# IntuitionMachines/volta

Hardware: AMD Instinct MI355X
Metric: image-text pairs/sec, ctrl_vilbert_base pretrain step (higher is better)
Workload: dtype bf16

## Files before the change

include/volta_hip.h:

```cpp
#ifndef VOLTA_HIP_H
#define VOLTA_HIP_H
#include <stddef.h>
#include <stdint.h>

#ifdef __cplusplus
extern "C" {
#endif

typedef void* vk_stream_t;

int vk_version(void);
const char* vk_device_arch(void);
const char* vk_last_error(void);

typedef struct vk_dropout {
    const uint64_t* seed;
    uint32_t site;
    uint32_t threshold;
    float scale;
} vk_dropout;

int vk_set_seed(uint64_t* seed_dev, uint64_t seed, vk_stream_t s);

int vk_cast_f32_bf16(const float* src, void* dst, int64_t n, vk_stream_t s);
// ... 262 lines not shown
    const void* target;
    const int64_t* mask;
    void* work;
    float* out;
    int32_t* row_argmax;
    int32_t kind, groups, n, ld;
} vk_task_loss_args;
int64_t vk_task_loss_work_bytes(int groups);
int vk_task_loss_fwd(const vk_task_loss_args* a, vk_stream_t s);
int vk_task_loss_bwd(const vk_task_loss_args* a, const float* gscale, void* dlogits, vk_stream_t s);

int vk_mask_prep(const int64_t* mask, float* out, int n, vk_stream_t s);

#define VK_CHUNK_SKIP 255
int vk_grad_norm_workspace_floats(void);
int vk_grad_norm_clip(const float* g, int64_t n, float pre_scale, float max_norm, float* partial, float* out, vk_stream_t s);
int vk_grad_norm_clip_masked(const float* g, int64_t n, const uint8_t* chunk_class, float pre_scale, float max_norm, float* partial, float* out, vk_stream_t s);
int vk_grad_sqnorm_chunks(const float* g, int64_t chunk0, int64_t nchunks, const uint8_t* chunk_class, float* sums, vk_stream_t s);
int vk_grad_norm_from_chunks(float* sums, int64_t total_chunks, float pre_scale, float max_norm, float* out, vk_stream_t s);
typedef struct vk_adamw_args {
    float* p;
    const float* g;
    float* m;
    float* v;
    void* shadow;
    const uint8_t* chunk_class;
    const float* clip;
    int64_t n;
    float cls_lr_mult[8];
    float cls_wd[8];
    float lr, beta1, beta2, eps, step_mult, grad_scale;
} vk_adamw_args;
int vk_adamw_step(const vk_adamw_args* a, vk_stream_t s);
int vk_adamw_step_on(const vk_adamw_args* a, int ncus, vk_stream_t s);
typedef struct vk_adamw_tensor {
    float* p;
    const float* g;
    float* m;
    float* v;
    int64_t numel;
    int32_t cls;
    int32_t reserved_;
} vk_adamw_tensor;
int vk_adamw_step_list(const vk_adamw_args* a, const vk_adamw_tensor* list, int n, int64_t max_numel, vk_stream_t s);
int vk_grad_sqnorm_list(const vk_adamw_tensor* list, int n, int64_t max_numel, float* work, float* sums, vk_stream_t s);
int vk_grad_sqnorm_list_work_floats(void);
#define VK_RADAM_CLASSES 64
typedef struct vk_radam_args {
    float* p;
    const float* g;
    float* m;
    float* v;
    void* shadow;
    const uint8_t* chunk_class;
    const float* clip;
    int64_t n;
    float cls_decay[VK_RADAM_CLASSES];
    float cls_step[VK_RADAM_CLASSES];
    int32_t cls_rect[VK_RADAM_CLASSES];
    float beta1, beta2;
    float one_minus_beta1, one_minus_beta2;
    float eps, grad_scale;
} vk_radam_args;
int vk_radam_step(const vk_radam_args* a, vk_stream_t s);
int vk_radam_step_list(const vk_radam_args* a, const vk_adamw_tensor* list, int n, int64_t max_numel, vk_stream_t s);
int vk_axpy_f32(float* y, const float* x, float alpha, int64_t n, vk_stream_t s);
// ... 314 lines not shown
```

volta_amd/_lib.py:

```python
import ctypes as C
import os

import torch

_HERE = os.path.dirname(os.path.abspath(__file__))
LIB_PATH = os.path.join(_HERE, "libvolta_hip_%s.so" % os.environ["VK_LIB"] if os.environ.get("VK_LIB") else "libvolta_hip.so")
GEMM_PERSISTENT, GEMM_ONE_TILE_PER_WG, GEMM_SOFT_START = 0x1000, 0x2000, 0x4000


class VoltaHipError(RuntimeError):
    pass


if not os.path.exists(LIB_PATH):
    raise ImportError(
        "volta_amd: %s not found. The HIP kernels are the product; there is no fallback path. "
        "Build with `make -C volta_amd/csrc` (hipcc --offload-arch=gfx950)." % LIB_PATH)

lib = C.CDLL(LIB_PATH)

c_p = C.c_void_p
i32 = C.c_int32
CHUNK_SKIP = 255

# ... 286 lines not shown
_sig("vk_text_end_rows", C.c_int, c_p, C.c_int, C.c_int, c_p, c_p, c_p)
_sig("vk_vlbert_obj_ids", C.c_int, c_p, c_p, C.c_int, C.c_int, c_p)
_sig("vk_lmdb_open", C.c_int, C.c_char_p, C.POINTER(c_p))
_sig("vk_lmdb_close", None, c_p)
_sig("vk_lmdb_entries", C.c_int64, c_p)
_sig("vk_lmdb_first", C.c_int, c_p)
_sig("vk_lmdb_next", C.c_int, c_p, C.POINTER(c_p), C.POINTER(C.c_size_t), C.POINTER(c_p), C.POINTER(C.c_size_t))
_sig("vk_lmdb_get", C.c_int, c_p, C.c_char_p, C.c_size_t, C.POINTER(c_p), C.POINTER(C.c_size_t))
_sig("vk_concap_record_decode", C.c_int, c_p, C.c_size_t, C.POINTER(ConcapRecord))
_sig("vk_concap_records_decode", C.c_int, C.POINTER(c_p), C.POINTER(C.c_size_t), C.POINTER(ConcapRecord), C.c_int, C.c_int, C.POINTER(C.c_int))
_sig("vk_wordpiece_open", C.c_int, C.c_char_p, C.c_int, C.POINTER(c_p))
_sig("vk_wordpiece_close", None, c_p)
_sig("vk_wordpiece_vocab_size", C.c_int, c_p)
_sig("vk_wordpiece_token_id", C.c_int, c_p, C.c_char_p)
_sig("vk_wordpiece_encode", C.c_int, c_p, C.c_char_p, C.c_size_t, c_p, C.c_int)
_sig("vk_wordpiece_encode_batch", C.c_int, c_p, C.POINTER(C.c_char_p), C.POINTER(C.c_size_t), C.c_int, c_p, C.c_int, c_p, C.c_int)
_sig("vk_b64_decode", C.c_int, C.c_char_p, C.c_size_t, c_p, C.c_size_t, C.POINTER(C.c_size_t))
_sig("vk_task_batch", C.c_int, C.POINTER(TaskBatchArgs), c_p)
_sig("vk_task_images_stage", C.c_int, C.POINTER(TaskImage), C.c_int, C.c_int, C.POINTER(C.c_int))
_sig("vk_vlbert_positions", C.c_int, c_p, C.c_int, C.c_int, C.c_int, c_p, c_p, c_p)
_sig("vk_vis_loss_fwd", C.c_int, C.POINTER(VisLossArgs), c_p)
_sig("vk_vis_loss_bwd", C.c_int, C.POINTER(VisLossArgs), c_p, C.c_int, c_p, c_p)
_sig("vk_task_loss_work_bytes", C.c_int64, C.c_int)
_sig("vk_task_loss_fwd", C.c_int, C.POINTER(TaskLossArgs), c_p)
_sig("vk_task_loss_bwd", C.c_int, C.POINTER(TaskLossArgs), c_p, c_p, c_p)
_sig("vk_nce_negatives", C.c_int, Dropout, C.c_int, C.c_int, c_p, c_p)
_sig("vk_pool_mul_bwd", C.c_int, c_p, C.c_int, c_p, c_p, c_p, c_p, C.c_int, C.c_int, Dropout, c_p)
_sig("vk_mask_prep", C.c_int, c_p, c_p, C.c_int, c_p)
_sig("vk_mul_bf16", C.c_int, c_p, c_p, c_p, C.c_int64, c_p, C.c_int, c_p)
_sig("vk_grad_norm_workspace_floats", C.c_int)
_sig("vk_grad_norm_clip", C.c_int, c_p, C.c_int64, C.c_float, C.c_float, c_p, c_p, c_p)
_sig("vk_adamw_step", C.c_int, C.POINTER(AdamwArgs), c_p)
_sig("vk_adamw_step_on", C.c_int, C.POINTER(AdamwArgs), C.c_int, c_p)
_sig("vk_grad_norm_clip_masked", C.c_int, c_p, C.c_int64, c_p, C.c_float, C.c_float, c_p, c_p, c_p)
_sig("vk_adamw_step_list", C.c_int, C.POINTER(AdamwArgs), c_p, C.c_int, C.c_int64, c_p)
_sig("vk_grad_sqnorm_list", C.c_int, c_p, C.c_int, C.c_int64, c_p, c_p, c_p)
_sig("vk_grad_sqnorm_list_work_floats", C.c_int)
_sig("vk_grad_seed", C.c_int, C.POINTER(GradSeedArgs), c_p)
_sig("vk_pair_gather", C.c_int, C.POINTER(PairGatherArgs), c_p)
_sig("vk_retrieval_ranks", C.c_int, C.POINTER(RetrievalRanksArgs), c_p)
_sig("vk_retrieval_ranks_shard_rows", C.c_int, C.POINTER(RetrievalRanksShardArgs), c_p)
_sig("vk_retrieval_ranks_shard_cols", C.c_int, C.POINTER(RetrievalRanksShardArgs), c_p)
_sig("vk_retrieval_ranks_finish", C.c_int, C.POINTER(RetrievalRanksShardArgs), c_p)
_sig("vk_image_means", C.c_int, C.POINTER(ImageMeansArgs), c_p)
_sig("vk_knn_pool_work_bytes", C.c_int64, C.c_int, C.c_int, C.c_int, C.c_int)
_sig("vk_knn_pool", C.c_int, C.POINTER(KnnPoolArgs), c_p)
_sig("vk_radam_step", C.c_int, C.POINTER(RadamArgs), c_p)
_sig("vk_radam_step_list", C.c_int, C.POINTER(RadamArgs), c_p, C.c_int, C.c_int64, c_p)
_sig("vk_grad_sqnorm_chunks", C.c_int, c_p, C.c_int64, C.c_int64, c_p, c_p, c_p)
_sig("vk_grad_norm_from_chunks", C.c_int, c_p, C.c_int64, C.c_float, C.c_float, c_p, c_p)
_sig("vk_axpy_f32", C.c_int, c_p, c_p, C.c_float, C.c_int64, c_p)
_sig("vk_sum_slabs_f32", C.c_int, c_p, c_p, C.c_int64, C.c_int, C.c_int64, c_p)
_sig("vk_sum_slabs_bf16", C.c_int, c_p, c_p, C.c_int64, C.c_int, C.c_int64, c_p, C.c_int, c_p)
_sig("vk_memset_async", C.c_int, c_p, C.c_int, C.c_int64, c_p)
_sig("vk_hold_cus", C.c_int, C.c_int, C.c_int, C.c_int, c_p)
_sig("vk_gate_wait", C.c_int, c_p, c_p, C.c_int, c_p, c_p)
_sig("vk_bump_u64", C.c_int, c_p, c_p)
_sig("vk_store_u64", C.c_int, c_p, C.c_uint64, c_p)
_sig("vk_gate_value", C.c_int, c_p, C.c_uint64, C.c_int, c_p, c_p)
_sig("vk_comm_standin", C.c_int, c_p, c_p, C.c_int64, C.c_int, C.c_int, c_p, c_p)
_sig("vk_gemm_reserve_cus", C.c_int, C.c_int)
_sig("vk_side_tail", C.c_int, C.POINTER(TailJob), C.c_int, c_p)
_sig("vk_lora_fwd", C.c_int, C.POINTER(LoraProblem), C.c_int, c_p)
_sig("vk_lora_bwd", C.c_int, C.POINTER(LoraBwdProblem), C.c_int, c_p, c_p)
_sig("vk_lora_bwd_work_bytes", C.c_int64, C.POINTER(LoraBwdProblem), C.c_int)
_sig("vk_lora_proj_fwd", C.c_int, C.POINTER(LoraProjProblem), C.c_int, c_p)
_sig("vk_lora_proj_bwd", C.c_int, C.POINTER(LoraProjBwdProblem), C.c_int, c_p, c_p)
_sig("vk_lora_proj_bwd_work_bytes", C.c_int64, C.POINTER(LoraProjBwdProblem), C.c_int)
_sig("vk_lora_fwd_drop", C.c_int, C.POINTER(LoraProblem), C.POINTER(Dropout), C.c_int, c_p)
_sig("vk_lora_bwd_drop", C.c_int, C.POINTER(LoraBwdProblem), C.POINTER(Dropout), C.c_int, c_p, c_p)
_sig("vk_lora_proj_fwd_drop", C.c_int, C.POINTER(LoraProjProblem), C.POINTER(Dropout), C.c_int, c_p)
_sig("vk_lora_proj_bwd_drop", C.c_int, C.POINTER(LoraProjBwdProblem), C.POINTER(Dropout), C.c_int, c_p, c_p)
_sig("vk_run_ops", C.c_int, C.POINTER(Op), C.c_int, c_p)
_sig("vk_run_ops_timed", C.c_int, C.POINTER(Op), C.c_int, c_p, C.POINTER(C.c_float))
_sig("vk_ln_bwd_finalize", C.c_int, C.POINTER(LnBwdArgs), c_p)
_sig("vk_ln_fwd_pair", C.c_int, C.POINTER(LnArgs), C.POINTER(LnArgs), c_p)
_sig("vk_ln_bwd_pair", C.c_int, C.POINTER(LnBwdArgs), C.POINTER(LnBwdArgs), c_p)
_sig("vk_concap_batch", C.c_int, C.POINTER(ConcapArgs), c_p)
_sig("vk_side_join", C.c_int, c_p)
_sig("vk_side_join_from", C.c_int, c_p, c_p)
_sig("vk_side_enable", None, C.c_int)
_sig("vk_side_stream", c_p, c_p)

EXPORTS = ["vk_version", "vk_device_arch", "vk_last_error", "vk_set_seed", "vk_cast_f32_bf16", "vk_gemm_grouped", "vk_gemm_grouped_ex", "vk_gemm_geometry", "vk_gemm_chain", "vk_gemm_split_workspace_bytes", "vk_gemm_fp8_grouped", "vk_quant_rows_fp8", "vk_cast_bf16_fp8",
           "vk_ln_fwd", "vk_ln_fwd_pair", "vk_ln_bwd_partial_rows", "vk_ln_bwd", "vk_ln_bwd_pair", "vk_ln_bwd_finalize", "vk_gated_attn_fwd", "vk_gated_attn_bwd", "vk_gated_attn_lds_bytes",
           "vk_embed_sum_fwd", "vk_embed_sum_bwd", "vk_embed_bwd_workspace_bytes", "vk_rows32", "vk_loc_linear_fwd", "vk_loc_linear_bwd",
           "vk_add_dropout", "vk_colsum_bf16", "vk_vlbert_prep_fwd", "vk_vlbert_maskgrad", "vk_rowgroup_sum_bf16",
           "vk_relu_bwd_bf16", "vk_copy_async", "vk_select_rows", "vk_gather_rows", "vk_scatter_rows_add", "vk_xent_fwd",
           "vk_xent_bwd", "vk_kl_fwd", "vk_kl_bwd", "vk_loss_finalize", "vk_pool_mul_fwd", "vk_pool_mul_bwd",
           "vk_pool_fuse_fwd", "vk_pool_fuse_bwd", "vk_text_end_rows", "vk_vlbert_obj_ids", "vk_vlbert_positions", "vk_vis_loss_fwd", "vk_vis_loss_bwd", "vk_nce_negatives", "vk_task_loss_work_bytes", "vk_task_loss_fwd", "vk_task_loss_bwd",
           "vk_mask_prep", "vk_mul_bf16", "vk_grad_norm_workspace_floats", "vk_grad_norm_clip", "vk_grad_norm_clip_masked", "vk_grad_sqnorm_chunks", "vk_grad_norm_from_chunks", "vk_adamw_step", "vk_adamw_step_on", "vk_adamw_step_list", "vk_grad_sqnorm_list", "vk_grad_sqnorm_list_work_floats", "vk_grad_seed", "vk_pair_gather", "vk_radam_step", "vk_radam_step_list",
           "vk_axpy_f32", "vk_sum_slabs_f32", "vk_sum_slabs_bf16", "vk_memset_async", "vk_hold_cus", "vk_gate_wait", "vk_bump_u64", "vk_store_u64", "vk_gate_value", "vk_comm_standin", "vk_gemm_reserve_cus", "vk_side_tail", "vk_run_ops", "vk_run_ops_timed", "vk_side_join", "vk_side_join_from", "vk_side_stream", "vk_side_enable", "vk_concap_batch",
           "vk_lmdb_open", "vk_lmdb_close", "vk_lmdb_entries", "vk_lmdb_first", "vk_lmdb_next", "vk_lmdb_get", "vk_concap_record_decode", "vk_concap_records_decode", "vk_b64_decode",
           "vk_wordpiece_open", "vk_wordpiece_close", "vk_wordpiece_vocab_size", "vk_wordpiece_token_id", "vk_wordpiece_encode", "vk_wordpiece_encode_batch",
           "vk_lora_fwd", "vk_lora_bwd", "vk_lora_bwd_work_bytes", "vk_lora_proj_fwd", "vk_lora_proj_bwd", "vk_lora_proj_bwd_work_bytes",
           "vk_lora_fwd_drop", "vk_lora_bwd_drop", "vk_lora_proj_fwd_drop", "vk_lora_proj_bwd_drop",
           "vk_task_batch", "vk_task_images_stage", "vk_retrieval_ranks", "vk_retrieval_ranks_shard_rows", "vk_retrieval_ranks_shard_cols", "vk_retrieval_ranks_finish", "vk_image_means", "vk_knn_pool_work_bytes", "vk_knn_pool"]


def check(rc):
    if rc != 0:
        raise VoltaHipError(lib.vk_last_error().decode())


def stream_ptr():
    return C.c_void_p(torch.cuda.current_stream().cuda_stream)


def ptr(t):
    return C.c_void_p(t.data_ptr()) if t is not None else None
```

volta_amd/csrc/attention.hip:

```cpp
#include "common.h"
#include "../../include/volta_hip.h"
#include "util.h"

namespace vk {



template <int DHT>
__device__ __forceinline__ uint32_t img_off(int row, int col) {
    return (uint32_t)(row * (2 * DHT) + ((((col >> 4) ^ ((row >> 1) & 3)) << 5) | ((col & 15) << 1)));
}
template <int DHT>
__device__ __forceinline__ bf16x8 img_row_frag(uint32_t img, int row0, int ks, int lane) {
    const int row = row0 + (lane & 15);
    return *(const bf16x8 VK_LDS*)(uintptr_t)(img + img_off<DHT>(row, ks * 32 + (lane >> 4) * 8));
}
template <int DHT>
__device__ __forceinline__ bf16x8 img_tr_frag(uint32_t img, int rbase, int d0, int lane) {
    const int g = lane >> 4, q = (lane & 15) >> 2, p = lane & 3;
    const int r0 = rbase + 4 * g + q, r1 = r0 + 16;
    bf16x4 lo = lds_read_tr16(img + img_off<DHT>(r0, d0 + 4 * p));
    bf16x4 hi = lds_read_tr16(img + img_off<DHT>(r1, d0 + 4 * p));
    bf16x8 r;
    r[0] = lo[0]; r[1] = lo[1]; r[2] = lo[2]; r[3] = lo[3];
// ... 440 lines not shown
static int fill(AttnK& k, const vk_attn_args* a, const vk_attn_bwd_args* bw) {
    for (int m = 0; m < 2; ++m) {
        k.q[m] = (const uint16_t*)a->q[m]; k.k[m] = (const uint16_t*)a->k[m]; k.v[m] = (const uint16_t*)a->v[m];
        k.ld[m] = a->ld[m]; k.L[m] = a->L[m]; k.mask[m] = a->mask[m];
        k.ctx[m] = (uint16_t*)a->ctx[m]; k.ldo[m] = a->ldo[m]; k.lse[m] = a->lse[m];
        for (int n = 0; n < 2; ++n) { k.gate[m][n] = a->gate[m][n]; k.drop[m][n] = a->drop[m][n]; }
        k.dctx[m] = bw ? (const uint16_t*)bw->dctx[m] : nullptr;
        k.dq[m] = bw ? (uint16_t*)bw->dq[m] : nullptr; k.dk[m] = bw ? (uint16_t*)bw->dk[m] : nullptr;
        k.dv[m] = bw ? (uint16_t*)bw->dv[m] : nullptr; k.ldg[m] = bw ? bw->ldg[m] : 0;
    }
    k.B = a->B; k.nh = a->nh; k.scale = a->scale;
    for (int m = 0; m < 2; ++m) {
        const bool qa = a->gate[m][0] || a->gate[m][1], ka = a->gate[0][m] || a->gate[1][m];
        if (!qa && !ka) continue;
        if (a->L[m] <= 0) return set_error("vk_gated_attn: modality %d is gated on but has length %d", m, a->L[m]);
        if (a->L[m] > (m == 0 ? 64 : 128)) return set_error("vk_gated_attn: lengths (%d, %d) exceed the (64, 128) tile budget", a->L[0], a->L[1]);
        if ((a->ld[m] & 7) || (a->ldo[m] & 7)) return set_error("vk_gated_attn: row strides must be multiples of 8");
        if (ka && (!a->k[m] || !a->v[m] || !a->mask[m])) return set_error("vk_gated_attn: K/V/mask of modality %d missing", m);
        if (qa && (!a->q[m] || !a->ctx[m] || !a->lse[m])) return set_error("vk_gated_attn: Q/ctx/lse of modality %d missing", m);
        if (bw && qa && (!bw->dctx[m] || !bw->dq[m])) return set_error("vk_gated_attn_bwd: dctx/dq of modality %d missing", m);
        if (bw && ka && (!bw->dk[m] || !bw->dv[m])) return set_error("vk_gated_attn_bwd: dk/dv of modality %d missing", m);
    }
    return 0;
}

VK_ATTN_TUNABLE g_attn_fwd_waves = 4;
VK_ATTN_TUNABLE g_attn_fwd_occ = 4;
template <int TP, int RP, int DHT>
static int launch_fwd(const AttnK& k, int nq_tiles, hipStream_t s) {
    const int lds = 3 * (TP + RP) * 2 * DHT + (TP + RP) * 4 + 16;
    int waves = nq_tiles < 4 ? 4 : (nq_tiles > 8 ? 8 : nq_tiles);
    if (g_attn_fwd_waves >= 4 && g_attn_fwd_waves < waves && 4 * lds <= 160 * 1024) waves = g_attn_fwd_waves;
    if (DHT == 64 && g_attn_fwd_occ == 5) {
        hipLaunchKernelGGL((attn_fwd_kernel<TP, RP, 5, DHT>), dim3(k.B * k.nh), dim3(64 * waves), lds, s, k);
    } else {
        auto kern = attn_fwd_kernel<TP, RP, (DHT == 64 ? 4 : 3), DHT>;
        static const hipError_t attr = hipFuncSetAttribute((const void*)kern, hipFuncAttributeMaxDynamicSharedMemorySize, lds); (void)attr;
        hipLaunchKernelGGL(kern, dim3(k.B * k.nh), dim3(64 * waves), lds, s, k);
    }
    return check_launch("vk_gated_attn_fwd");
}
VK_ATTN_TUNABLE g_attn_bwd_waves = 4;
VK_ATTN_TUNABLE g_attn_bwd_occ = 3;

template <int TP, int RP, int DHT>
static int launch_bwd(const AttnK& k, int ntasks, hipStream_t s) {
    const int lds = 4 * (TP + RP) * 2 * DHT + 3 * (TP + RP) * 4 + 16;
    if (DHT == 64 && g_attn_bwd_occ == 3 && 3 * lds <= 160 * 1024) {
        auto kern = attn_bwd_kernel<TP, RP, 3, DHT>;
        static const hipError_t attr = hipFuncSetAttribute((const void*)kern, hipFuncAttributeMaxDynamicSharedMemorySize, lds); (void)attr;
        int waves = g_attn_bwd_waves < 4 ? 4 : (ntasks > g_attn_bwd_waves ? g_attn_bwd_waves : (ntasks < 4 ? 4 : ntasks));
        hipLaunchKernelGGL(kern, dim3(k.B * k.nh), dim3(64 * waves), lds, s, k);
    } else {
        auto kern = attn_bwd_kernel<TP, RP, 2, DHT>;
        static const hipError_t attr = hipFuncSetAttribute((const void*)kern, hipFuncAttributeMaxDynamicSharedMemorySize, lds); (void)attr;
        int waves = g_attn_bwd_waves < 4 ? 4 : (ntasks > g_attn_bwd_waves ? g_attn_bwd_waves : (ntasks < 4 ? 4 : ntasks));
        if (2 * lds > 160 * 1024) waves = ntasks >= 8 ? 8 : (ntasks < 4 ? 4 : ntasks);
        hipLaunchKernelGGL(kern, dim3(k.B * k.nh), dim3(64 * waves), lds, s, k);
    }
    return check_launch("vk_gated_attn_bwd");
}

static bool bwd_fits(int TP, int RP, int dht) { return 4 * (TP + RP) * 2 * dht + 3 * (TP + RP) * 4 + 16 <= 160 * 1024; }

}

namespace vk { int attn_generic(const vk_attn_args* a, const vk_attn_bwd_args* bw, vk_stream_t stream); }

#ifdef VK_STUDY
static int g_attn_force_generic = 0;
extern "C" void vk_attn_set_force_generic(int v) { g_attn_force_generic = v; }
#else
static constexpr int g_attn_force_generic = 0;
#endif
static bool attn_mfma_ok(const vk_attn_args* a) {
    if (a->probs[0][0] || a->probs[0][1] || a->probs[1][0] || a->probs[1][1]) return false;
    for (int m = 0; m < 2; ++m) {
        const bool on = a->gate[m][0] || a->gate[m][1] || a->gate[0][m] || a->gate[1][m];
        if (on && a->L[m] > (m == 0 ? 64 : 128)) return false;
    }
    if (a->dh == 0 || a->dh == 64) return true;
    if (a->dh != 128 || g_attn_force_generic) return false;
    const int TP = a->L[0] > 32 ? 64 : 32, RP = a->L[1] > 64 ? 128 : 64;
    return vk::bwd_fits(TP, RP, 128);
}

namespace vk { size_t attn_generic_lds(const vk_attn_args* a, bool bwd); }

extern "C" size_t vk_gated_attn_lds_bytes(const vk_attn_args* a, int backward) {
    if (!a || attn_mfma_ok(a)) return 0;
    return vk::attn_generic_lds(a, backward != 0);
// ... 51 lines not shown
```

volta_amd/csrc/attention_generic.hip:

```cpp
#include "common.h"
#include "../../include/volta_hip.h"
#include "util.h"

namespace vk {

struct AttnG {
    const uint16_t* q[2]; const uint16_t* k[2]; const uint16_t* v[2];
    int32_t ld[2], L[2];
    const float* mask[2];
    uint16_t* ctx[2]; int32_t ldo[2];
    float* lse[2];
    int32_t B, nh;
    int32_t gate[2][2];
    vk_dropout drop[2][2];
    float scale;
    const uint16_t* dctx[2];
    uint16_t* dq[2]; uint16_t* dk[2]; uint16_t* dv[2];
    int32_t ldg[2];
    float* probs[2][2];
};

constexpr int GW = 4;
constexpr int GMAXNS = 8;

// ... 227 lines not shown
                    const uint32_t wq = *(const uint32_t*)(imgA[mq] + q * RS + 4 * lane), wg = *(const uint32_t*)(imgB[mq] + q * RS + 4 * lane);
                    const float ds = pb0[j], pd = pb1[j];
                    k0 += ds * bf2f(wq & 0xFFFF); k1 += ds * bf2f(wq >> 16);
                    v0 += pd * bf2f(wg & 0xFFFF); v1 += pd * bf2f(wg >> 16);
                }
                *(uint32_t*)(a.dk[mk] + ((size_t)b * Lk + k) * a.ldg[mk] + h * D + 2 * lane) = pack2bf(k0, k1);
                *(uint32_t*)(a.dv[mk] + ((size_t)b * Lk + k) * a.ldg[mk] + h * D + 2 * lane) = pack2bf(v0, v1);
            }
        }
    }
}

static size_t g_lds_bytes(const AttnG& k, int D, int NS, bool bwd) {
    const size_t RS = (size_t)D * 2 + 16;
    size_t n = 0;
    if (bwd) {
        const size_t Lsum = (size_t)k.L[0] + (size_t)k.L[1];
        n = 2 * Lsum * RS + 2 * ((Lsum * 4 + 15) & ~(size_t)15);
    } else {
        for (int m = 0; m < 2; ++m)
            if (k.gate[0][m] || k.gate[1][m]) n += 2 * (size_t)k.L[m] * RS;
    }
    n += (size_t)GW * D * 4 * (bwd ? 2 : 1) + (size_t)GW * NS * 64 * 4 * (bwd ? 2 : 1);
    return (n + 15) & ~(size_t)15;
}

template <int D, int NS>
static int g_launch_ns(const AttnG& k, bool bwd, hipStream_t s) {
    const size_t lds = g_lds_bytes(k, D, NS, bwd);
    if (lds > 160 * 1024) return set_error("vk_gated_attn: head size %d with lengths (%d, %d) needs %zu bytes of LDS (> 160 KiB)", D, k.L[0], k.L[1], lds);
    if (bwd) {
        auto kern = attn_generic_bwd_kernel<D, NS>;
        if (hipFuncSetAttribute((const void*)kern, hipFuncAttributeMaxDynamicSharedMemorySize, (int)lds) != hipSuccess) return set_error("vk_gated_attn_bwd: cannot reserve %zu bytes of LDS", lds);
        hipLaunchKernelGGL(kern, dim3(k.B * k.nh), dim3(64 * GW), lds, s, k);
        return check_launch("vk_gated_attn_bwd (generic kernel)");
    }
    auto kern = attn_generic_fwd_kernel<D, NS>;
    if (hipFuncSetAttribute((const void*)kern, hipFuncAttributeMaxDynamicSharedMemorySize, (int)lds) != hipSuccess) return set_error("vk_gated_attn_fwd: cannot reserve %zu bytes of LDS", lds);
    hipLaunchKernelGGL(kern, dim3(k.B * k.nh), dim3(64 * GW), lds, s, k);
    return check_launch("vk_gated_attn_fwd (generic kernel)");
}

template <int D>
static int g_launch(const AttnG& k, bool bwd, hipStream_t s) {
    int need = 0;
    for (int m = 0; m < 2; ++m) {
        const int nq = (k.gate[m][0] ? k.L[0] : 0) + (k.gate[m][1] ? k.L[1] : 0), nk = (k.gate[0][m] ? k.L[0] : 0) + (k.gate[1][m] ? k.L[1] : 0);
        need = need > nq ? need : nq;
        need = need > nk ? need : nk;
    }
    if (need > GMAXNS * 64) return set_error("vk_gated_attn: %d keys per query row (at most %d on the generic kernels)", need, GMAXNS * 64);
    if (need <= 192) return g_launch_ns<D, 3>(k, bwd, s);
    if (need <= 320) return g_launch_ns<D, 5>(k, bwd, s);
    return g_launch_ns<D, 8>(k, bwd, s);
}

size_t attn_generic_lds(const vk_attn_args* a, bool bwd) {
    AttnG k;
    for (int m = 0; m < 2; ++m) {
        const bool qa = a->gate[m][0] || a->gate[m][1], ka = a->gate[0][m] || a->gate[1][m];
        k.L[m] = (qa || ka) ? a->L[m] : 0;
        for (int j = 0; j < 2; ++j) k.gate[m][j] = a->gate[m][j];
    }
    int need = 0;
    for (int m = 0; m < 2; ++m) {
        const int nq = (k.gate[m][0] ? k.L[0] : 0) + (k.gate[m][1] ? k.L[1] : 0), nk = (k.gate[0][m] ? k.L[0] : 0) + (k.gate[1][m] ? k.L[1] : 0);
        need = need > nq ? need : nq;
        need = need > nk ? need : nk;
    }
    const int NS = need <= 192 ? 3 : need <= 320 ? 5 : 8;
    return g_lds_bytes(k, a->dh ? a->dh : 64, NS, bwd);
}
// ... 37 lines not shown
```

volta_amd/csrc/backbone.hip:

```cpp
#include "common.h"
#include "../../include/volta_hip.h"
#include "util.h"

namespace vk {

__global__ __launch_bounds__(256) void grad_seed_kernel(const vk_grad_seed_args a) {
    const int64_t per_row = a.H / 8, total = (int64_t)a.B * a.L * per_row;
    for (int64_t i = (int64_t)blockIdx.x * 256 + threadIdx.x; i < total; i += (int64_t)gridDim.x * 256) {
        const int64_t r = i / per_row;
        const int h = (int)(i - r * per_row) * 8;
        const int64_t b = r / a.L, l = r - b * a.L;
        float x[8];
        if (a.src) {
            const float* s = a.src + b * a.stride_b + l * a.stride_l + h;
            const f32x4 lo = *(const f32x4*)s, hi = *(const f32x4*)(s + 4);
#pragma unroll
            for (int k = 0; k < 4; ++k) { x[k] = lo[k]; x[k + 4] = hi[k]; }
        } else {
#pragma unroll
            for (int k = 0; k < 8; ++k) x[k] = 0.f;
        }
        if (a.y) {
            const u32x4 yv = *(const u32x4*)((const uint16_t*)a.y + r * a.ldy + h);
#pragma unroll
            for (int k = 0; k < 4; ++k) {
                if (!(bf2f((uint16_t)(yv[k] & 0xFFFFu)) > 0.f)) x[2 * k] = 0.f;
                if (!(bf2f((uint16_t)(yv[k] >> 16)) > 0.f)) x[2 * k + 1] = 0.f;
            }
        }
        uint16_t* d = (uint16_t*)a.dst + (a.row0 + r) * a.ld + h;
        if (a.accumulate) {
            const u32x4 dv = *(const u32x4*)d;
#pragma unroll
            for (int k = 0; k < 4; ++k) {
                x[2 * k] += bf2f((uint16_t)(dv[k] & 0xFFFFu));
                x[2 * k + 1] += bf2f((uint16_t)(dv[k] >> 16));
            }
        }
        *(u32x4*)d = u32x4{pack2bf(x[0], x[1]), pack2bf(x[2], x[3]), pack2bf(x[4], x[5]), pack2bf(x[6], x[7])};
    }
}

}

using namespace vk;

extern "C" int vk_grad_seed(const vk_grad_seed_args* a, vk_stream_t s) {
    if (a->B <= 0 || a->L <= 0 || a->H <= 0) return set_error("vk_grad_seed: empty shape %d x %d x %d", a->B, a->L, a->H);
    if (a->H % 8 || a->ld % 8 || a->row0 < 0 || a->ld < a->H || (a->y && (a->ldy % 8 || a->ldy < a->H)))
        return set_error("vk_grad_seed: H, ld and ldy must be multiples of 8 (H %d, ld %d, ldy %d)", a->H, a->ld, a->ldy);
    if (!a->dst || ((uintptr_t)a->dst & 15) || ((uintptr_t)a->y & 15)) return set_error("vk_grad_seed: dst and y need 16-byte alignment");
    if (!a->src && a->accumulate) return 0;
    if (a->src && (((uintptr_t)a->src & 15) || (a->stride_b & 3) || (a->stride_l & 3)))
        return set_error("vk_grad_seed: src needs 16-byte alignment and strides that are multiples of 4 (copy it contiguous)");
    const int64_t total = (int64_t)a->B * a->L * (a->H / 8);
    int64_t blocks = (total + 255) / 256;
    if (blocks > 2048) blocks = 2048;
    hipLaunchKernelGGL(grad_seed_kernel, dim3((unsigned)blocks), dim3(256), 0, (hipStream_t)s, *a);
    return check_launch("vk_grad_seed");
}
```

volta_amd/csrc/capi.cpp:

```cpp
#include "util.h"
#include "../../include/volta_hip.h"

namespace vk {
static thread_local char g_err[512] = {0};
char* error_buffer() { return g_err; }
int set_error(const char* fmt, ...) {
    va_list ap;
    va_start(ap, fmt);
    vsnprintf(g_err, sizeof(g_err), fmt, ap);
    va_end(ap);
    return -1;
}
int check_launch(const char* what) {
    hipError_t e = hipGetLastError();
    if (e != hipSuccess) return set_error("%s: %s", what, hipGetErrorString(e));
    return 0;
}
}

extern "C" int vk_version(void) { return 1; }
extern "C" const char* vk_device_arch(void) { return "gfx950"; }
extern "C" const char* vk_last_error(void) { return vk::error_buffer(); }
```

volta_amd/csrc/embed.hip:

```cpp
#include "common.h"
#include "../../include/volta_hip.h"
#include "util.h"
#include <climits>

namespace vk {

__device__ __forceinline__ void ld4(const uint16_t* p, float (&v)[4]) {
    u32x2 r = *(const u32x2*)p;
    v[0] = bf2f(r[0] & 0xFFFF); v[1] = bf2f(r[0] >> 16); v[2] = bf2f(r[1] & 0xFFFF); v[3] = bf2f(r[1] >> 16);
}
__device__ __forceinline__ void st4(uint16_t* p, const float (&v)[4]) {
    *(u32x2*)p = u32x2{pack2bf(v[0], v[1]), pack2bf(v[2], v[3])};
}

__device__ __forceinline__ int64_t clampi(int64_t v, int n) { return v < 0 ? 0 : (v >= n ? n - 1 : v); }

__global__ __launch_bounds__(256) void embed_sum_fwd_kernel(vk_embed_args a) {
    const int lane = threadIdx.x & 63, row = blockIdx.x * 4 + (threadIdx.x >> 6);
    if (row >= a.M) return;
    const int64_t id = clampi(a.ids[row], a.V);
    const int64_t ty = a.type_ids ? clampi(a.type_ids[row], a.n_types) : 0;
    const int64_t ps = clampi(a.pos_ids ? a.pos_ids[row] : (row % a.T), a.P);
    const float* w = a.word + (size_t)id * a.H;
    const float* p = a.pos + (size_t)ps * a.H;
// ... 521 lines not shown
    const int b = blockIdx.x, c = blockIdx.y * 256 + threadIdx.x * 4;
    if (c >= H) return;
    float s[4] = {0.f, 0.f, 0.f, 0.f};
    for (int t = 0; t < T; ++t) {
        float v[4];
        ld4(in + ((size_t)b * T + t) * H + c, v);
#pragma unroll
        for (int r = 0; r < 4; ++r) s[r] += v[r];
    }
    st4(out + (size_t)b * H + c, s);
}

__global__ void relu_bwd_kernel(const uint16_t* dy, const uint16_t* y, uint16_t* out, size_t n8) {
    for (size_t i = (size_t)blockIdx.x * blockDim.x + threadIdx.x; i < n8; i += (size_t)gridDim.x * blockDim.x) {
        const u32x4 g = *(const u32x4*)(dy + i * 8), v = *(const u32x4*)(y + i * 8);
        u32x4 o;
#pragma unroll
        for (int k = 0; k < 4; ++k) {
            const uint32_t lo = (bf2f(v[k] & 0xFFFF) > 0.f) ? (g[k] & 0xFFFFu) : 0u, hi = (bf2f(v[k] >> 16) > 0.f) ? (g[k] & 0xFFFF0000u) : 0u;
            o[k] = lo | hi;
        }
        *(u32x4*)(out + i * 8) = o;
    }
}

}

using namespace vk;

extern "C" int vk_vlbert_prep_fwd(const float* loc, int nloc, const float* feat, const float* mask_emb, void* out, int32_t* zero_flag,
                                  int M, int F, int dim, vk_dropout drop, vk_stream_t s) {
    if (F % 4 || (8 * dim) % 4 || nloc < 4) return set_error("vk_vlbert_prep_fwd: F and 8*dim must be multiples of 4, nloc >= 4");
    if (M <= 0) return 0;
    hipLaunchKernelGGL(vlbert_prep_kernel, dim3((M + 3) / 4), dim3(256), 0, (hipStream_t)s, loc, nloc, feat, mask_emb, (uint16_t*)out, zero_flag, M, F, dim, drop);
    return check_launch("vk_vlbert_prep_fwd");
}

extern "C" int vk_vlbert_maskgrad(const void* dx, int ldx, int col0, const int32_t* zero_flag, float* partial, float* out, int M, int F,
                                  vk_dropout drop, vk_stream_t s) {
    if (F % 4 || F > 2048 || col0 % 4) return set_error("vk_vlbert_maskgrad: F must be a multiple of 4, <= 2048");
    if (M <= 0) return 0;
    const int nblk = (M + 31) / 32, nch = (F + 255) / 256;
    hipStream_t st = (hipStream_t)s;
    if (nch <= 4) hipLaunchKernelGGL(vlbert_maskgrad_kernel<4>, dim3(nblk), dim3(256), 0, st, (const uint16_t*)dx, ldx, col0, zero_flag, partial, M, F, drop);
    else hipLaunchKernelGGL(vlbert_maskgrad_kernel<8>, dim3(nblk), dim3(256), 0, st, (const uint16_t*)dx, ldx, col0, zero_flag, partial, M, F, drop);
    hipLaunchKernelGGL(colsum_finalize_kernel, dim3((F + 63) / 64), dim3(1024), 0, st, partial, nblk, F, out, 0);
    return check_launch("vk_vlbert_maskgrad");
}

extern "C" int vk_rowgroup_sum_bf16(const void* in, void* out, int B, int T, int H, vk_stream_t s) {
    if (H % 4) return set_error("vk_rowgroup_sum_bf16: H %% 4 != 0");
    if (B <= 0) return 0;
    hipLaunchKernelGGL(rowgroup_sum_kernel, dim3(B, (H + 255) / 256), dim3(64), 0, (hipStream_t)s, (const uint16_t*)in, (uint16_t*)out, T, H);
    return check_launch("vk_rowgroup_sum_bf16");
}

extern "C" int vk_relu_bwd_bf16(const void* dy, const void* y, void* out, int64_t n, vk_stream_t s) {
    if (n % 8) return set_error("vk_relu_bwd_bf16: n %% 8 != 0");
    if (n <= 0) return 0;
    int64_t blocks = (n / 8 + 255) / 256;
    if (blocks > 4096) blocks = 4096;
    hipLaunchKernelGGL(relu_bwd_kernel, dim3((unsigned)blocks), dim3(256), 0, (hipStream_t)s, (const uint16_t*)dy, (const uint16_t*)y, (uint16_t*)out, (size_t)(n / 8));
    return check_launch("vk_relu_bwd_bf16");
}

extern "C" int vk_copy_async(void* dst, const void* src, int64_t bytes, vk_stream_t s) {
    if (bytes <= 0) return 0;
    hipError_t e = hipMemcpyAsync(dst, src, (size_t)bytes, hipMemcpyDeviceToDevice, (hipStream_t)s);
    if (e != hipSuccess) return set_error("vk_copy_async: %s", hipGetErrorString(e));
    return 0;
}

extern "C" int vk_embed_sum_fwd(const vk_embed_args* a, vk_stream_t s) {
    if (a->H % 4) return set_error("vk_embed_sum_fwd: H %% 4 != 0");
    if (a->M <= 0) return 0;
    hipLaunchKernelGGL(embed_sum_fwd_kernel, dim3((a->M + 3) / 4), dim3(256), 0, (hipStream_t)s, *a);
    return check_launch("vk_embed_sum_fwd");
}

static size_t ws_align(size_t b) { return (b + 255) & ~(size_t)255; }

static size_t embed_ws_layout(int M, int H, int V, int P, int has_pos, char* base, EmbWs* w) {
    const size_t S = (size_t)((M + 31) / 32) * 32;
    size_t off = 0;
    auto take = [&](size_t bytes) { char* q = base ? base + off : nullptr; off += ws_align(bytes); return q; };
    EmbWs x;
    x.Pw = (float*)take(S * H * 4);
    x.Pp = has_pos ? (float*)take(S * H * 4) : nullptr;
    x.Q = (float*)take(S / 32 * 4 * H * 4);
    x.kw = (int*)take(S * 4);
    x.kp = has_pos ? (int*)take(S * 4) : nullptr;
    x.ow = (int*)take((size_t)V * 4);
    x.op = has_pos ? (int*)take((size_t)P * 4) : nullptr;
    if (w) *w = x;
    return off;
}

extern "C" int64_t vk_embed_bwd_workspace_bytes(int M, int H, int V, int P, int has_pos) {
    return M <= 0 ? 0 : (int64_t)embed_ws_layout(M, H, V, P, has_pos, nullptr, nullptr);
}

extern "C" int vk_embed_sum_bwd(const vk_embed_bwd_args* a, vk_stream_t s) {
    if (a->H % 4 || a->H > 1024) return set_error("vk_embed_sum_bwd: H must be a multiple of 4, <= 1024");
    if (a->n_types > 4) return set_error("vk_embed_sum_bwd: at most 4 token types");
    if (a->M <= 0) return 0;
    if (a->T <= 0 || a->M % a->T) return set_error("vk_embed_sum_bwd: M must be a multiple of T (rows are b * T + t)");
    if (!a->work) return set_error("vk_embed_sum_bwd: no workspace (vk_embed_bwd_workspace_bytes)");
    const int has_pos = a->pos_ids && a->dpos;
    EmbWs w;
    embed_ws_layout(a->M, a->H, a->V, a->P, has_pos, (char*)a->work, &w);
    const int nch = (a->H + 255) / 256, S = (a->M + 31) / 32 * 32;
    hipStream_t st = (hipStream_t)s;
    hipLaunchKernelGGL(fill_i32_kernel, dim3((a->V + 255) / 256), dim3(256), 0, st, w.ow, INT_MAX, a->V);
    if (has_pos) hipLaunchKernelGGL(fill_i32_kernel, dim3((a->P + 255) / 256), dim3(256), 0, st, w.op, INT_MAX, a->P);
    dim3 grid(S / 32), block(256);
    switch (nch) {
        case 1: hipLaunchKernelGGL(embed_scatter_kernel<1>, grid, block, 0, st, *a, w); break;
        case 2: hipLaunchKernelGGL(embed_scatter_kernel<2>, grid, block, 0, st, *a, w); break;
        case 3: hipLaunchKernelGGL(embed_scatter_kernel<3>, grid, block, 0, st, *a, w); break;
        default: hipLaunchKernelGGL(embed_scatter_kernel<4>, grid, block, 0, st, *a, w); break;
    }
    dim3 grid2(S + (a->dtype ? (a->H + 63) / 64 : 0), has_pos ? 2 : 1);
    switch (nch) {
        case 1: hipLaunchKernelGGL(embed_combine_kernel<1>, grid2, block, 0, st, *a, w, S); break;
        case 2: hipLaunchKernelGGL(embed_combine_kernel<2>, grid2, block, 0, st, *a, w, S); break;
        case 3: hipLaunchKernelGGL(embed_combine_kernel<3>, grid2, block, 0, st, *a, w, S); break;
        default: hipLaunchKernelGGL(embed_combine_kernel<4>, grid2, block, 0, st, *a, w, S); break;
    }
    if (!a->pos_ids && a->dpos) {
        hipLaunchKernelGGL(embed_pos_reduce_kernel, dim3(a->T, (a->H + 255) / 256), dim3(64), 0, st, (const uint16_t*)a->dz, a->dpos,
                           a->M / a->T, a->T, a->H);
    }
    return check_launch("vk_embed_sum_bwd");
}

extern "C" int vk_loc_linear_fwd(const float* loc, const float* W, const float* bias, void* out, int M, int H, int nloc, vk_stream_t s) {
    if (nloc > 8 || H % 4) return set_error("vk_loc_linear_fwd: nloc <= 8, H %% 4 == 0 required");
    if (M <= 0) return 0;
    if (H > 1024) return set_error("vk_loc_linear_fwd: H <= 1024 required");
    const dim3 grid((M + 4 * LOC_ROWS - 1) / (4 * LOC_ROWS)), block(256);
    hipStream_t st = (hipStream_t)s;
    switch ((H + 255) / 256) {
        case 1: hipLaunchKernelGGL(loc_linear_fwd_kernel<1>, grid, block, 0, st, loc, W, bias, (uint16_t*)out, M, H, nloc); break;
        case 2: hipLaunchKernelGGL(loc_linear_fwd_kernel<2>, grid, block, 0, st, loc, W, bias, (uint16_t*)out, M, H, nloc); break;
        case 3: hipLaunchKernelGGL(loc_linear_fwd_kernel<3>, grid, block, 0, st, loc, W, bias, (uint16_t*)out, M, H, nloc); break;
        default: hipLaunchKernelGGL(loc_linear_fwd_kernel<4>, grid, block, 0, st, loc, W, bias, (uint16_t*)out, M, H, nloc); break;
    }
    return check_launch("vk_loc_linear_fwd");
}

extern "C" int vk_rows32(int M) { return (M + 31) / 32; }

extern "C" int vk_loc_linear_bwd(const void* dz, const float* loc, float* partial, float* dW, float* db, int M, int H, int nloc, vk_stream_t s) {
    if (nloc > 8 || H % 4 || H > 1024) return set_error("vk_loc_linear_bwd: nloc <= 8, H %% 4 == 0, H <= 1024 required");
    if (M <= 0) return 0;
    const int nblk = (M + 31) / 32, nch = (H + 255) / 256;
    hipStream_t st = (hipStream_t)s;
    switch (nch) {
        case 1: hipLaunchKernelGGL(loc_linear_bwd_kernel<1>, dim3(nblk), dim3(256), 0, st, (const uint16_t*)dz, loc, partial, M, H, nloc); break;
        case 2: hipLaunchKernelGGL(loc_linear_bwd_kernel<2>, dim3(nblk), dim3(256), 0, st, (const uint16_t*)dz, loc, partial, M, H, nloc); break;
        case 3: hipLaunchKernelGGL(loc_linear_bwd_kernel<3>, dim3(nblk), dim3(256), 0, st, (const uint16_t*)dz, loc, partial, M, H, nloc); break;
        default: hipLaunchKernelGGL(loc_linear_bwd_kernel<4>, dim3(nblk), dim3(256), 0, st, (const uint16_t*)dz, loc, partial, M, H, nloc); break;
    }
    hipLaunchKernelGGL(loc_linear_bwd_finalize_kernel, dim3((9 * H + 63) / 64), dim3(1024), 0, st, partial, nblk, H, nloc, dW, db);
    return check_launch("vk_loc_linear_bwd");
}

extern "C" int vk_add_dropout(const void* a, const void* b, void* y, int M, int H, float scale, vk_dropout drop, int backward, vk_stream_t s) {
    if (H % 4) return set_error("vk_add_dropout: H %% 4 != 0");
    if (M <= 0) return 0;
    hipLaunchKernelGGL(add_dropout_kernel, dim3((M + 3) / 4), dim3(256), 0, (hipStream_t)s, (const uint16_t*)a, (const uint16_t*)b,
                       (uint16_t*)y, M, H, scale, drop, backward);
    return check_launch("vk_add_dropout");
}

extern "C" int vk_colsum_bf16(const void* src, float* partial, float* out, int M, int H, int accumulate, vk_stream_t s) {
    if (H % 4 || H > 1024) return set_error("vk_colsum_bf16: H must be a multiple of 4, <= 1024");
    if (M <= 0) return 0;
    const int nblk = (M + 31) / 32, nch = (H + 255) / 256;
    hipStream_t st = (hipStream_t)s;
    switch (nch) {
        case 1: hipLaunchKernelGGL(colsum_kernel<1>, dim3(nblk), dim3(256), 0, st, (const uint16_t*)src, partial, M, H); break;
        case 2: hipLaunchKernelGGL(colsum_kernel<2>, dim3(nblk), dim3(256), 0, st, (const uint16_t*)src, partial, M, H); break;
        case 3: hipLaunchKernelGGL(colsum_kernel<3>, dim3(nblk), dim3(256), 0, st, (const uint16_t*)src, partial, M, H); break;
        default: hipLaunchKernelGGL(colsum_kernel<4>, dim3(nblk), dim3(256), 0, st, (const uint16_t*)src, partial, M, H); break;
    }
    hipLaunchKernelGGL(colsum_finalize_kernel, dim3((H + 63) / 64), dim3(1024), 0, st, partial, nblk, H, out, accumulate);
    return check_launch("vk_colsum_bf16");
}
```

volta_amd/csrc/executor.cpp:

```cpp
#include "util.h"
#include <vector>
#include "../../include/volta_hip.h"

static int run_one(const vk_op& o, int i, vk_stream_t s);

#include <cstdlib>
#include <mutex>
#include <unordered_map>
namespace {
constexpr int N_SIDE_EVENTS = 16;
struct Side {
    hipStream_t stream = nullptr;
    hipEvent_t fork = nullptr, join = nullptr;
    hipEvent_t done[N_SIDE_EVENTS] = {};
    bool recorded[N_SIDE_EVENTS] = {};
    bool ok = false;
};
std::mutex g_side_mutex;
std::unordered_map<void*, Side*> g_sides;
int g_side_enabled = 1;

Side* side_lookup(vk_stream_t caller) {
    std::lock_guard<std::mutex> lock(g_side_mutex);
    auto it = g_sides.find((void*)caller);
// ... 15 lines not shown
        if (e != hipSuccess) { vk::set_error("side stream: hipStreamCreate failed"); return nullptr; }
    }
    if (hipEventCreateWithFlags(&g.fork, hipEventDisableTiming) != hipSuccess || hipEventCreateWithFlags(&g.join, hipEventDisableTiming) != hipSuccess) {
        vk::set_error("side stream: hipEventCreate failed");
        return nullptr;
    }
    for (int i = 0; i < N_SIDE_EVENTS; ++i)
        if (hipEventCreateWithFlags(&g.done[i], hipEventDisableTiming) != hipSuccess) { vk::set_error("side stream: hipEventCreate failed"); return nullptr; }
    g.ok = true;
    return sp;
}
}

extern "C" void vk_side_enable(int on) { g_side_enabled = on; }

extern "C" int vk_side_join_from(vk_stream_t owner, vk_stream_t waiter) {
    Side* g = side_lookup(owner);
    if (!g || !g->ok) return 0;
    if (hipEventRecord(g->join, g->stream) != hipSuccess) return vk::set_error("vk_side_join: hipEventRecord failed");
    if (hipStreamWaitEvent((hipStream_t)waiter, g->join, 0) != hipSuccess) return vk::set_error("vk_side_join: hipStreamWaitEvent failed");
    return 0;
}

extern "C" int vk_side_join(vk_stream_t s) { return vk_side_join_from(s, s); }

extern "C" vk_stream_t vk_side_stream(vk_stream_t owner) {
    Side* g = side_for(owner);
    return g ? (vk_stream_t)g->stream : nullptr;
}

extern "C" int vk_run_ops(const vk_op* ops, int n, vk_stream_t s) {
    vk_stream_t cur = s;
    Side* g = nullptr;
    for (int i = 0; i < n; ++i) {
        const vk_op& o = ops[i];
        if (o.kind >= VK_OP_SIDE_BEGIN && o.kind <= VK_OP_JOIN) {
            if (!g_side_enabled) continue;
            if (!g && !(g = side_for(s))) return -1;
            hipError_t e = hipSuccess;
            switch (o.kind) {
                case VK_OP_SIDE_BEGIN:
                    if (o.i0 != 1) {
                        e = hipEventRecord(g->fork, (hipStream_t)s);
                        if (e == hipSuccess) e = hipStreamWaitEvent(g->stream, g->fork, 0);
                    }
                    cur = (vk_stream_t)g->stream;
                    break;
                case VK_OP_SIDE_END:
                    if (o.i0 < 0 || o.i0 >= N_SIDE_EVENTS) return vk::set_error("vk_run_ops: side event %d out of range", o.i0);
                    e = hipEventRecord(g->done[o.i0], g->stream);
                    g->recorded[o.i0] = true;
                    cur = s;
                    break;
                case VK_OP_WAIT_SIDE:
                    if (o.i0 < 0 || o.i0 >= N_SIDE_EVENTS) return vk::set_error("vk_run_ops: side event %d out of range", o.i0);
                    if (g->recorded[o.i0]) e = hipStreamWaitEvent((hipStream_t)s, g->done[o.i0], 0);
                    break;
                default:
                    if (vk_side_join(s) != 0) return -1;
            }
            if (e != hipSuccess) return vk::set_error("vk_run_ops: side-stream control op %d failed at index %d: %s", o.kind, i, hipGetErrorString(e));
            continue;
        }
        if (o.kind == VK_OP_GENERIC && o.a && ((const vk_generic_args*)o.a)->fn == VK_FN_GATE && cur == s) continue;
        int rc = run_one(o, i, cur);
        if (rc != 0) return rc;
    }
    if (cur != s) return vk::set_error("vk_run_ops: op list ends inside a side-stream block");
    return 0;
}

extern "C" int vk_run_ops_timed(const vk_op* ops, int n, vk_stream_t s, float* ms) {
    static thread_local std::vector<hipEvent_t> ev;
    while ((int)ev.size() < n + 1) {
        hipEvent_t e;
        if (hipEventCreate(&e) != hipSuccess) return vk::set_error("vk_run_ops_timed: hipEventCreate failed");
        ev.push_back(e);
    }
    hipStream_t st = (hipStream_t)s;
    (void)hipEventRecord(ev[0], st);
    for (int i = 0; i < n; ++i) {
        const bool gate = ops[i].kind == VK_OP_GENERIC && ops[i].a && ((const vk_generic_args*)ops[i].a)->fn == VK_FN_GATE;
        if (!(ops[i].kind >= VK_OP_SIDE_BEGIN && ops[i].kind <= VK_OP_JOIN) && !gate) {
            int rc = run_one(ops[i], i, s);
            if (rc != 0) return rc;
        }
        (void)hipEventRecord(ev[i + 1], st);
    }
    if (hipStreamSynchronize(st) != hipSuccess) return vk::set_error("vk_run_ops_timed: stream sync failed");
    for (int i = 0; i < n; ++i) {
        float t = 0.f;
        (void)hipEventElapsedTime(&t, ev[i], ev[i + 1]);
        ms[i] += t;
    }
    return 0;
}

static int run_one(const vk_op& o, int i, vk_stream_t s) {
// ... 78 lines not shown
```

volta_amd/csrc/fp8.hip:

```cpp
#include "gemm_common.h"

namespace vk {

typedef __attribute__((ext_vector_type(8))) int i32x8;
constexpr float FP8_MAX = 448.0f;

struct KProb8 { KProb b; const float* sa; const float* sb; };
struct KGroup8 { int32_t nprob; int32_t plain_order; KProb8 p[VK_GEMM_FP8_MAX_GROUP]; };

template <typename SRC>
__global__ __launch_bounds__(256) void quant_rows_fp8_kernel(const SRC* __restrict__ src, int64_t ld, uint8_t* __restrict__ dst, int64_t ldq, float* __restrict__ scale,
                                                             int M, int K, const int32_t* dyn) {
    const int lane = threadIdx.x & 63, row = blockIdx.x * 4 + (threadIdx.x >> 6);
    const int Mr = dyn ? min(*dyn, M) : M;
    if (row >= Mr) return;
    const SRC* x = src + (size_t)row * ld;
    constexpr int MAXCH = 8;
    float v[MAXCH][8];
    float amax = 0.f;
#pragma unroll
    for (int j = 0; j < MAXCH; ++j) {
        const int c = (j * 64 + lane) * 8;
#pragma unroll
        for (int r = 0; r < 8; ++r) v[j][r] = 0.f;
// ... 115 lines not shown
        }
    }
    {
        const int gq = lane >> 4, lr = lane & 15;
        const __amdgpu_buffer_rsrc_t ra = make_rsrc(Q.sa, Q.sa ? (uint32_t)M * 4u : 0u), rb = make_rsrc(Q.sb, Q.sb ? (uint32_t)P.N * 4u : 0u);
        f32x4 sb4[4];
#pragma unroll
        for (int j = 0; j < 4; ++j) {
            sb4[j] = __builtin_bit_cast(f32x4, __builtin_amdgcn_raw_buffer_load_b128(rb, (uint32_t)(n0 + wn * 64 + j * 16 + gq * 4) * 4u, 0, 0));
            if (!Q.sb) sb4[j] = f32x4{1.f, 1.f, 1.f, 1.f};
        }
#pragma unroll
        for (int i = 0; i < TI; ++i) {
            float sa = __builtin_bit_cast(float, __builtin_amdgcn_raw_buffer_load_b32(ra, (uint32_t)(m0 + wm * 64 * TM + i * 16 + lr) * 4u, 0, 0));
            if (!Q.sa) sa = 1.f;
#pragma unroll
            for (int j = 0; j < 4; ++j)
#pragma unroll
                for (int r = 0; r < 4; ++r) acc[i][j][r] *= sa * sb4[j][r];
        }
    }
    f32x4 accb[TI];
    __builtin_amdgcn_s_barrier();
    gemm_epilogue<false, EPI, TI, 4>(P, acc, accb, false, m0 + wm * 64 * TM, n0 + wn * 64, M, lane, lds0 + (uint32_t)wave * 16384u);
}

template <int WM, int WN, int TM>
static int launch8(int epi, const KGroup8& g, int total, hipStream_t s) {
    constexpr int LDS = 2 * (64 * TM * WM + 64 * WN) * 128;
#define VK_CASE(E)                                                                                        \
    case E: {                                                                                             \
        auto k = gemm_fp8_kernel<E, WM, WN, TM>;                                                          \
        static const hipError_t attr = hipFuncSetAttribute((const void*)k, hipFuncAttributeMaxDynamicSharedMemorySize, LDS); (void)attr; \
        hipLaunchKernelGGL(k, dim3(total), dim3(64 * WM * WN), LDS, s, g);                                \
        break;                                                                                            \
    }
    switch (epi) {
        VK_CASE(VK_EPI_BF16) VK_CASE(VK_EPI_GELU) VK_CASE(VK_EPI_F32) VK_CASE(VK_EPI_RELU)
        default: return set_error("vk_gemm_fp8_grouped: epilogue %d is not available on the fp8 path", epi);
    }
#undef VK_CASE
    return check_launch("vk_gemm_fp8_grouped");
}

}

using namespace vk;

extern "C" int vk_gemm_fp8_grouped(int epilogue, const vk_gemm_fp8_problem* probs, int nprob, int geometry, vk_stream_t stream) {
    if (nprob < 1 || nprob > VK_GEMM_FP8_MAX_GROUP) return set_error("vk_gemm_fp8_grouped: nprob %d out of range", nprob);
    const bool f32out = epilogue == VK_EPI_F32;
    bool any_dyn = false;
    for (int i = 0; i < nprob; ++i) {
        const vk_gemm_problem& q = probs[i].p;
        if (q.M < 0 || q.N <= 0 || q.K < 0) return set_error("vk_gemm_fp8_grouped: bad shape %d %d %d", q.M, q.N, q.K);
        if ((q.lda & 15) || (q.ldb & 15)) return set_error("vk_gemm_fp8_grouped: lda/ldb must be multiples of 16 bytes (got %d %d)", q.lda, q.ldb);
        if (((uintptr_t)q.A & 15) || ((uintptr_t)q.B & 15) || ((uintptr_t)q.C & 15)) return set_error("vk_gemm_fp8_grouped: operands must be 16-byte aligned");
        if (!f32out && (q.ldc & 3)) return set_error("vk_gemm_fp8_grouped: ldc must be a multiple of 4");
        if ((q.K % 128) != 0 && q.lda < ((q.K + 127) / 128) * 128) return set_error("vk_gemm_fp8_grouped: K=%d needs lda padded to a multiple of 128", q.K);
        if (q.bias_grad || q.R) return set_error("vk_gemm_fp8_grouped: forward epilogues only");
        if (epilogue == VK_EPI_GELU && !q.C2) return set_error("vk_gemm_fp8_grouped: C2 missing");
        if (probs[i].c8 && (epilogue != VK_EPI_GELU || (probs[i].ldc8 & 3) || ((uintptr_t)probs[i].c8 & 3))) return set_error("vk_gemm_fp8_grouped: c8 is a GELU-epilogue output with a 4-byte aligned leading dimension");
        if ((uint64_t)q.M * q.lda >= 0x7FFFFFF0ull || (uint64_t)q.N * q.ldb >= 0x7FFFFFF0ull) return set_error("vk_gemm_fp8_grouped: operands must stay below 2 GiB");
        any_dyn |= q.dyn != nullptr;
    }
    int t256 = 0;
    for (int i = 0; i < nprob; ++i) t256 += ((probs[i].p.M + 255) / 256) * ((probs[i].p.N + 255) / 256);
    int edge = geometry ? geometry : (t256 >= 160 ? 256 : 128);
    if (edge != 128 && edge != 256) return set_error("vk_gemm_fp8_grouped: geometry %d (128 or 256)", geometry);
    KGroup8 g{};
    g.nprob = nprob;
    g.plain_order = any_dyn ? 1 : 0;
    int total = 0;
    for (int i = 0; i < nprob; ++i) {
        const vk_gemm_problem& q = probs[i].p;
        KProb& k = g.p[i].b;
        k.A = (const char*)q.A; k.B = (const char*)q.B; k.C = (char*)q.C; k.C2 = (char*)q.C2; k.bias = q.bias;
        k.R = nullptr; k.bias_grad = nullptr; k.dyn = q.dyn;
        k.M = q.M; k.N = q.N; k.K = q.K; k.lda = q.lda; k.ldb = q.ldb; k.ldc = q.ldc; k.ldr = 0; k.n_store = q.n_store;
        const int ncols = (f32out && q.n_store > q.N) ? q.n_store : q.N;
        k.tiles_n = (ncols + edge - 1) / edge;
        k.tile_start = total;
        total += ((q.M + edge - 1) / edge) * k.tiles_n;
        k.C8 = (char*)probs[i].c8; k.c8_mul = probs[i].c8_mul; k.ldc8 = probs[i].ldc8;
        g.p[i].sa = probs[i].scale_a; g.p[i].sb = probs[i].scale_b;
    }
    if (total == 0) return 0;
    hipStream_t s = (hipStream_t)stream;
    return edge == 256 ? launch8<2, 4, 2>(epilogue, g, total, s) : launch8<2, 2, 1>(epilogue, g, total, s);
}

extern "C" int vk_quant_rows_fp8(const void* src, int src_is_f32, int64_t ld, void* dst, int64_t ldq, float* scale, int M, int K, const int32_t* dyn, vk_stream_t stream) {
    if (M <= 0) return 0;
    if (K <= 0 || K > 4096 || (K & 7) || (ld & 7) || (ldq & 7)) return set_error("vk_quant_rows_fp8: K=%d (multiple of 8, <= 4096), ld / ldq multiples of 8", K);
    if (((uintptr_t)src & 15) || ((uintptr_t)dst & 7)) return set_error("vk_quant_rows_fp8: alignment");
    hipStream_t s = (hipStream_t)stream;
    if (src_is_f32) hipLaunchKernelGGL(quant_rows_fp8_kernel<float>, dim3((M + 3) / 4), dim3(256), 0, s, (const float*)src, ld, (uint8_t*)dst, ldq, scale, M, K, dyn);
    else hipLaunchKernelGGL(quant_rows_fp8_kernel<uint16_t>, dim3((M + 3) / 4), dim3(256), 0, s, (const uint16_t*)src, ld, (uint8_t*)dst, ldq, scale, M, K, dyn);
    return check_launch("vk_quant_rows_fp8");
}

extern "C" int vk_cast_bf16_fp8(const void* src, void* dst, int64_t n, float mul, vk_stream_t stream) {
    if (n <= 0) return 0;
    if ((n & 7) || ((uintptr_t)src & 15) || ((uintptr_t)dst & 7)) return set_error("vk_cast_bf16_fp8: n %% 8 == 0 and aligned buffers required");
    int64_t blocks = (n / 8 + 255) / 256;
    if (blocks > 8192) blocks = 8192;
    hipLaunchKernelGGL(cast_bf16_fp8_kernel, dim3((unsigned)blocks), dim3(256), 0, (hipStream_t)stream, (const uint16_t*)src, (uint8_t*)dst, (size_t)n, mul);
    return check_launch("vk_cast_bf16_fp8");
}
```

volta_amd/csrc/gemm.hip:

```cpp
#include "gemm_common.h"
#include <cstdlib>

namespace vk {

template <int WM, int WN, int TM = 1> struct Geo {
    static constexpr int THREADS = 64 * WM * WN, BM = 64 * TM * WM, BN = 64 * WN;
    static constexpr int A_BYTES = BM * BK * 2, B_BYTES = BN * BK * 2, STAGE = A_BYTES + B_BYTES;
};

template <bool T, int EXT, int THREADS>
__device__ __forceinline__ void stage_tile(__amdgpu_buffer_rsrc_t rs, uint32_t lds_tile, int ld, int row0, int col0, int tid) {
    constexpr int NP = EXT * 8 / THREADS;
    constexpr int CPR = T ? EXT / 8 : 8;
    const int wave = tid >> 6;
#pragma unroll
    for (int i = 0; i < NP; ++i) {
        const int lin = i * THREADS + tid;
        const int r = lin / CPR, cp = lin % CPR;
        const int cl = T ? (cp ^ tswz(r)) : (cp ^ (r & 7));
        const uint32_t voff = ((uint32_t)(row0 + r) * (uint32_t)ld + (uint32_t)(col0 + cl * 8)) * 2u;
        const uint32_t dst = lds_tile + (i * THREADS + wave * 64) * 16;
        __builtin_amdgcn_raw_ptr_buffer_load_lds(rs, (VK_LDS void*)(uintptr_t)dst, 16, voff, 0, 0, 0);
    }
}
// ... 121 lines not shown
#undef VK_LSTORE
    } else {
        auto stage = [&](int buf, int kt) {
            const uint32_t ta = lds0 + buf * G::STAGE, tb = ta + G::A_BYTES;
            if (AT) stage_tile<true, BM, THREADS>(rsA, ta, P.lda, kt * BK, m0, tid);
            else    stage_tile<false, BM, THREADS>(rsA, ta, P.lda, m0, kt * BK, tid);
            if (BT) stage_tile<true, BN, THREADS>(rsB, tb, P.ldb, kt * BK, n0, tid);
            else    stage_tile<false, BN, THREADS>(rsB, tb, P.ldb, n0, kt * BK, tid);
        };
        if (nk > 0) stage(0, 0);
        const bool late = (g.stagger & 0xFF) && (WM * WN > 4) && ((__builtin_amdgcn_readfirstlane(wave) >> 2) & 1);
        for (int kt = 0; kt < nk; ++kt) {
            asm volatile("s_waitcnt vmcnt(0)" ::: "memory");
            __builtin_amdgcn_s_barrier();
            if (!late && kt + 1 < nk) stage((kt + 1) & 1, kt + 1);
            compute_ks(kt & 1, 0);
            if (late && kt + 1 < nk) stage((kt + 1) & 1, kt + 1);
            compute_ks(kt & 1, 1);
        }
    }

    gemm_epilogue<AT, EPI, TI, 4>(P, acc, accb, do_bias_grad, m0 + wm * 64 * TM, n0 + wn * 64, M, lane);
    retire_mark(g);
}

template <bool AT, bool BT, int WM, int WN, bool REGSTAGE, int TM = 1>
static int launch_cfg(int epi, const KGroup& g, int total, hipStream_t s) {
    using G = Geo<WM, WN, TM>;
    constexpr int LDS = 2 * G::STAGE;
#define VK_CASE(E)                                                                                        \
    case E: {                                                                                             \
        auto k = gemm_kernel<AT, BT, E, WM, WN, REGSTAGE, TM>;                                                \
        static const hipError_t attr = hipFuncSetAttribute((const void*)k, hipFuncAttributeMaxDynamicSharedMemorySize, LDS); (void)attr;  \
        hipLaunchKernelGGL(k, dim3(total), dim3(G::THREADS), LDS, s, g);                                  \
        break;                                                                                            \
    }
    switch (epi) {
        VK_CASE(VK_EPI_BF16) VK_CASE(VK_EPI_GELU) VK_CASE(VK_EPI_MULR) VK_CASE(VK_EPI_ADDR) VK_CASE(VK_EPI_F32) VK_CASE(VK_EPI_RELU) VK_CASE(VK_EPI_F32_ACC)
        default: return set_error("vk_gemm_grouped: unknown epilogue %d", epi);
    }
#undef VK_CASE
    return check_launch("vk_gemm_grouped");
}

#ifdef VK_STUDY
#define VK_TUNABLE static int
#else
#define VK_TUNABLE static constexpr int
#endif
VK_TUNABLE g_stagger = 1;
VK_TUNABLE g_min_tiles256_tn = 50;
VK_TUNABLE g_min_tiles256 = 160;
VK_TUNABLE g_debug = 0;
VK_TUNABLE g_regstage_override = -1;
VK_TUNABLE g_persistent = 1;
#ifdef VK_STUDY
static int g_tile_override = 0;
#endif

static int total_tiles(const vk_gemm_problem* probs, int nprob, int epilogue, int bm, int bn) {
    int total = 0;
    for (int i = 0; i < nprob; ++i) {
        const vk_gemm_problem& q = probs[i];
        const bool f32 = epilogue == VK_EPI_F32 || epilogue == VK_EPI_F32_ACC;
        const int ncols = (f32 && q.n_store > q.N) ? q.n_store : q.N;
        total += ((q.M + bm - 1) / bm) * ((ncols + bn - 1) / bn);
    }
// ... 228 lines not shown
```

volta_amd/csrc/gemm256.hip:

```cpp
#include "gemm_common.h"
#include <hip/hip_ext.h>
#include <type_traits>
#include <atomic>

namespace vk {

constexpr uint32_t HT = 16384;
constexpr uint32_t OOB = 0x80000000u;

template <bool T, bool IS_A>
__device__ __forceinline__ void stage_offsets(uint32_t (&off)[2], int ld, int ext0, int tid) {
#pragma unroll
    for (int i = 0; i < 2; ++i) {
        const int lin = i * 512 + tid;
        if (!T) {
            const int hr = lin >> 3, cp = lin & 7;
            const int row = IS_A ? ((hr >> 6) * 128 + (hr & 63)) : ((hr >> 5) * 64 + (hr & 31));
            off[i] = ((uint32_t)(ext0 + row) * (uint32_t)ld + (uint32_t)((cp ^ (hr & 7)) * 8)) * 2u;
        } else {
            const int kr = lin >> 4, cp = lin & 15;
            const int c = cp ^ tswz(kr);
            const int col = IS_A ? ((c >> 3) * 128 + (c & 7) * 8) : ((c >> 2) * 64 + (c & 3) * 8);
            off[i] = ((uint32_t)kr * (uint32_t)ld + (uint32_t)(ext0 + col)) * 2u;
        }
// ... 472 lines not shown
}

#ifdef VK_STUDY
static unsigned long long* g_stamps = nullptr;
#else
static constexpr unsigned long long* g_stamps = nullptr;
#endif

static std::atomic<int> g_reserved_cus{0};

static int persistent_grid(int total) {
    const int ncu = NUM_CU - g_reserved_cus.load(std::memory_order_relaxed);
    if (total <= ncu) return total;
    const int rounds = (total + ncu - 1) / ncu;
    const int even = ((total + rounds - 1) / rounds + 7) & ~7;
    return even < ncu ? even : ncu;
}

template <bool AT, bool BT, int KSPLIT>
static int launch_layout(int epi, const KGroup& g, int total, hipStream_t s, bool persistent, bool soft) {
    const int flags = soft ? hipExtAnyOrderLaunch : 0;
    constexpr int LDS = (KSPLIT ? 10 : 8) * HT;
#ifdef VK_STUDY
#define VK_KERNEL_OF(E) (KSPLIT == 2 ? gemm256k_kernel<AT, BT, E, 2> : KSPLIT == 3 ? gemm256k_kernel<AT, BT, E, 3> : KSPLIT == 4 ? gemm256k_kernel<AT, BT, E, 4> : gemm256_kernel<AT, BT, E>)
#else
#define VK_KERNEL_OF(E) (KSPLIT == 2 ? gemm256k_kernel<AT, BT, E, 2> : KSPLIT == 3 ? gemm256k_kernel<AT, BT, E, 3> : gemm256k_kernel<AT, BT, E, 4>)
#endif
#define VK_CASE(E)                                                                                        \
    case E: {                                                                                             \
        if constexpr (!(AT && BT) && (KSPLIT == 3 || KSPLIT == 4)) {                                      \
            if (persistent) {                                                                             \
                auto kp = gemm256p_kernel<AT, BT, E, KSPLIT>;                                             \
                static const hipError_t attr_p = hipFuncSetAttribute((const void*)kp, hipFuncAttributeMaxDynamicSharedMemorySize, LDS); (void)attr_p; \
                hipExtLaunchKernelGGL(kp, dim3(persistent_grid(total)), dim3(512), LDS, s, nullptr, nullptr, flags, g, total, g_stamps); \
                break;                                                                                    \
            }                                                                                             \
        }                                                                                                 \
        auto k = VK_KERNEL_OF(E);                                                                         \
        static const hipError_t attr = hipFuncSetAttribute((const void*)k, hipFuncAttributeMaxDynamicSharedMemorySize, LDS); (void)attr;  \
        hipExtLaunchKernelGGL(k, dim3(total), dim3(512), LDS, s, nullptr, nullptr, flags, g);             \
        break;                                                                                            \
    }
    switch (epi) {
        VK_CASE(VK_EPI_BF16) VK_CASE(VK_EPI_GELU) VK_CASE(VK_EPI_MULR) VK_CASE(VK_EPI_ADDR) VK_CASE(VK_EPI_F32) VK_CASE(VK_EPI_RELU) VK_CASE(VK_EPI_F32_ACC)
        default: return set_error("vk_gemm_grouped: unknown epilogue %d", epi);
    }
#undef VK_CASE
#undef VK_KERNEL_OF
    return check_launch("vk_gemm_grouped");
}

int launch_gemm256_chain(int layout, int epi_p, int epi_c, const KGroup& g, int nprod, int ncons, hipStream_t s) {
    constexpr int LDS = 10 * HT;
    const int ncu = (NUM_CU - g_reserved_cus.load(std::memory_order_relaxed)) & ~7;
#define VK_CHAIN_CASE(BT_, P_, C_)                                                                                  \
    if (layout == ((BT_) ? VK_NN : VK_NT) && epi_p == (P_) && epi_c == (C_)) {                                        \
        auto k = gemm256c_kernel<BT_, P_, C_>;                                                                        \
        static const hipError_t attr = hipFuncSetAttribute((const void*)k, hipFuncAttributeMaxDynamicSharedMemorySize, LDS); (void)attr; \
        hipLaunchKernelGGL(k, dim3(ncu), dim3(512), LDS, s, g, nprod, ncons, g_stamps);                               \
        return check_launch("vk_gemm_chain");                                                                         \
    }
    VK_CHAIN_CASE(false, VK_EPI_GELU, VK_EPI_BF16)
    VK_CHAIN_CASE(true, VK_EPI_MULR, VK_EPI_ADDR)
#undef VK_CHAIN_CASE
    return set_error("vk_gemm_chain: layout %d with epilogues %d -> %d is not built (NT: GELU -> BF16, NN: MULR -> ADDR)", layout, epi_p, epi_c);
}

template <int KSPLIT>
static int launch_variant(int layout, int epilogue, const KGroup& g, int total, hipStream_t s, bool persistent, bool soft) {
    if (layout == VK_NT) return launch_layout<false, false, KSPLIT>(epilogue, g, total, s, persistent, soft);
    if (layout == VK_NN) return launch_layout<false, true, KSPLIT>(epilogue, g, total, s, persistent, soft);
    if (layout == VK_TN) return launch_layout<true, true, KSPLIT>(epilogue, g, total, s, false, false);
    return set_error("vk_gemm_grouped: unknown layout %d", layout);
}

int launch_gemm256(int layout, int epilogue, const KGroup& g, int total, hipStream_t s, int variant, bool persistent, bool soft) {
    if (variant == 2) return launch_variant<2>(layout, epilogue, g, total, s, false, soft);
    if (variant == 3) return launch_variant<3>(layout, epilogue, g, total, s, persistent, soft);
    if (variant == 4) return launch_variant<4>(layout, epilogue, g, total, s, persistent, soft);
#ifdef VK_STUDY
    return launch_variant<0>(layout, epilogue, g, total, s, false, false);
#else
    return set_error("vk_gemm_grouped: geometry variant %d is not part of this build", variant);
#endif
}

}

extern "C" int vk_gemm_reserve_cus(int n) {
    const int prev = vk::g_reserved_cus.load(std::memory_order_relaxed);
    if (n >= 0) vk::g_reserved_cus.store(n > 128 ? 128 : (n + 7) & ~7, std::memory_order_relaxed);
    return prev;
// ... 8 lines not shown
```

volta_amd/csrc/gemm4w.hip:

```cpp
#include "gemm_common.h"

namespace vk {

constexpr uint32_t W4_OOB = 0x80000000u;

__device__ __forceinline__ int kswz4(int r) { return (-(r >> 2)) & 3; }

template <bool T, int EXT, int NMAX>
__device__ __forceinline__ void strip_offsets4(uint32_t (&off)[NMAX], int ld, int ext0, int tid) {
    static_assert(EXT / 64 <= NMAX, "offset array too small");
#pragma unroll
    for (int i = 0; i < EXT / 64; ++i) {
        const int lin = i * 256 + tid;
        if (!T) {
            const int r = lin >> 2, cp = lin & 3;
            off[i] = ((uint32_t)(ext0 + r) * (uint32_t)ld + (uint32_t)((cp ^ kswz4(r)) * 8)) * 2u;
        } else {
            constexpr int CPR = EXT / 8;
            const int kr = lin / CPR, cp = lin % CPR;
            const int c = cp ^ tswz(kr);
            off[i] = ((uint32_t)kr * (uint32_t)ld + (uint32_t)(ext0 + c * 8)) * 2u;
        }
    }
}
// ... 102 lines not shown
        asm volatile("s_waitcnt lgkmcnt(0)" ::: "memory");
        __builtin_amdgcn_sched_barrier(0);
        __builtin_amdgcn_s_setprio(1);
#pragma unroll
        for (int i = 0; i < TI; ++i)
#pragma unroll
            for (int j = 0; j < 4; ++j)
                acc[i][j] = __builtin_amdgcn_mfma_f32_16x16x32_bf16(b[j], a[i], acc[i][j], 0, 0, 0);
        if (BG && do_bias_grad) {
#pragma unroll
            for (int i = 0; i < TI; ++i) accb[i] = __builtin_amdgcn_mfma_f32_16x16x32_bf16(ones, a[i], accb[i], 0, 0, 0);
        }
        __builtin_amdgcn_s_setprio(0);
        W4_BARRIER();
        rd = rd == RING - 1 ? 0 : rd + 1;
        wrs = wrs == RING - 1 ? 0 : wrs + 1;
    }
    asm volatile("s_waitcnt vmcnt(0)" ::: "memory");
    W4_BARRIER();

#undef W4_WAIT_STAGE
    gemm_epilogue<AT, EPI, TI, 4>(P, acc, accb, do_bias_grad, m0 + wr * (BM / 2), n0 + wc * 64, M, lane, lds0 + (uint32_t)wave * 16384u);
    retire_mark(g);
}

template <bool AT, bool BT, int TI, int RING>
static int launch_layout4(int epi, const KGroup& g, int total, hipStream_t s) {
    constexpr int LDS = RING * (32 * TI * 64 + 8192);
    static_assert(LDS >= 4 * 16384, "the epilogue stages 16 KiB per wave in the ring");
#define VK_CASE(E)                                                                                        \
    case E: {                                                                                             \
        auto k = gemm4w_kernel<AT, BT, E, TI, RING>;                                                      \
        static const hipError_t attr = hipFuncSetAttribute((const void*)k, hipFuncAttributeMaxDynamicSharedMemorySize, LDS); (void)attr; \
        hipLaunchKernelGGL(k, dim3(total), dim3(256), LDS, s, g);                                         \
        break;                                                                                            \
    }
    switch (epi) {
        VK_CASE(VK_EPI_BF16) VK_CASE(VK_EPI_GELU) VK_CASE(VK_EPI_MULR) VK_CASE(VK_EPI_ADDR) VK_CASE(VK_EPI_F32) VK_CASE(VK_EPI_RELU) VK_CASE(VK_EPI_F32_ACC)
        default: return set_error("vk_gemm_grouped: unknown epilogue %d", epi);
    }
#undef VK_CASE
    return check_launch("vk_gemm_grouped");
}

int launch_gemm4w(int layout, int epilogue, const KGroup& g, int total, hipStream_t s, int bm) {
    if (bm == 128) {
        if (layout == VK_NT) return launch_layout4<false, false, 4, 6>(epilogue, g, total, s);
        if (layout == VK_NN) return launch_layout4<false, true, 4, 6>(epilogue, g, total, s);
        if (layout == VK_TN) return launch_layout4<true, true, 4, 6>(epilogue, g, total, s);
    } else {
        if (layout == VK_NT) return launch_layout4<false, false, 8, 3>(epilogue, g, total, s);
        if (layout == VK_NN) return launch_layout4<false, true, 8, 3>(epilogue, g, total, s);
        if (layout == VK_TN) return launch_layout4<true, true, 8, 3>(epilogue, g, total, s);
    }
    return set_error("vk_gemm_grouped: unknown layout %d", layout);
}

}
```

volta_amd/csrc/heads.hip:

```cpp
#include "common.h"
#include "../../include/volta_hip.h"
#include "util.h"

namespace vk {

__global__ __launch_bounds__(1024) void select_rows_kernel(const int64_t* labels, int N, int mode, int inner, int outer, int off,
                                                           int32_t* rows, int32_t* pos, int32_t* count) {
    __shared__ int wave_tot[16];
    __shared__ int base_s;
    const int tid = threadIdx.x, lane = tid & 63, wave = tid >> 6;
    if (tid == 0) base_s = 0;
    __syncthreads();
    for (int start = 0; start < N; start += 1024) {
        const int i = start + tid;
        bool f = false;
        if (i < N) { const int64_t l = labels[i]; f = mode ? (l == 1) : (l != -1); }
        const unsigned long long bal = __ballot(f);
        const int before = __popcll(bal & ((1ull << lane) - 1ull));
        if (lane == 0) wave_tot[wave] = __popcll(bal);
        __syncthreads();
        int wbase = base_s;
        for (int w = 0; w < wave; ++w) wbase += wave_tot[w];
        if (f) {
            const int j = wbase + before;
// ... 160 lines not shown
        const u32x4 w = philox4((uint32_t)(c >> 2), (uint32_t)row, dc.site, 0u, (uint32_t)seed, (uint32_t)(seed >> 32));
        keep = (w[c & 3] >= dc.threshold) ? dc.scale : 0.f;
    }
    out[i] = f2bf(bf2f(pt[i]) * bf2f(pv[i]) * keep);
}
__global__ __launch_bounds__(256) void pool_mul_bwd_kernel(const uint16_t* dp, int ldp, const uint16_t* pt, const uint16_t* pv, uint16_t* dyt, uint16_t* dyv,
                                                           int B, int P, vk_dropout dc) {
    const int i = blockIdx.x * 256 + threadIdx.x;
    if (i >= B * P) return;
    const int row = i / P, c = i - row * P;
    float keep = 1.f;
    if (dc.threshold) {
        const uint64_t seed = *dc.seed;
        const u32x4 w = philox4((uint32_t)(c >> 2), (uint32_t)row, dc.site, 0u, (uint32_t)seed, (uint32_t)(seed >> 32));
        keep = (w[c & 3] >= dc.threshold) ? dc.scale : 0.f;
    }
    const float g = bf2f(dp[(size_t)row * ldp + c]) * keep, a = bf2f(pt[i]), b = bf2f(pv[i]);
    dyt[i] = f2bf(a > 0.f ? g * b : 0.f);
    dyv[i] = f2bf(b > 0.f ? g * a : 0.f);
}

__global__ void mask_prep_kernel(const int64_t* m, float* out, int n) {
    const int i = blockIdx.x * 256 + threadIdx.x;
    if (i < n) out[i] = (1.0f - (float)m[i]) * -10000.0f;
}

}

using namespace vk;

extern "C" int vk_select_rows(const int64_t* labels, int N, int mode, int inner, int outer, int off, int32_t* rows, int32_t* pos,
                              int32_t* count, vk_stream_t s) {
    if (N < 0 || inner <= 0) return set_error("vk_select_rows: bad arguments");
    hipLaunchKernelGGL(select_rows_kernel, dim3(1), dim3(1024), 0, (hipStream_t)s, labels, N, mode, inner, outer, off, rows, pos, count);
    return check_launch("vk_select_rows");
}
extern "C" int vk_gather_rows(const void* src, const int32_t* rows, const int32_t* count, void* dst, int H, int max_rows, vk_stream_t s) {
    if (H % 8) return set_error("vk_gather_rows: H %% 8 != 0");
    if (max_rows <= 0) return 0;
    hipLaunchKernelGGL(gather_rows_kernel, dim3((max_rows + 3) / 4), dim3(256), 0, (hipStream_t)s, (const uint16_t*)src, rows, count, (uint16_t*)dst, H, max_rows);
    return check_launch("vk_gather_rows");
}
extern "C" int vk_scatter_rows_add(const void* src, const int32_t* rows, const int32_t* count, void* dst, int H, int max_rows, vk_stream_t s) {
    if (H % 4) return set_error("vk_scatter_rows_add: H %% 4 != 0");
    if (max_rows <= 0) return 0;
    hipLaunchKernelGGL(scatter_rows_add_kernel, dim3((max_rows + 3) / 4), dim3(256), 0, (hipStream_t)s, (const uint16_t*)src, rows, count, (uint16_t*)dst, H, max_rows);
    return check_launch("vk_scatter_rows_add");
}
extern "C" int vk_xent_fwd(const vk_xent_args* a, vk_stream_t s) {
    if (a->max_rows <= 0) return 0;
    hipLaunchKernelGGL(xent_fwd_kernel, dim3(a->max_rows), dim3(256), 0, (hipStream_t)s, *a);
    return check_launch("vk_xent_fwd");
}
extern "C" int vk_xent_bwd(const vk_xent_args* a, void* dlogits, int ldd, const float* gscale, vk_stream_t s) {
    if (a->max_rows <= 0) return 0;
    if (ldd < a->V) return set_error("vk_xent_bwd: ldd < V");
    hipLaunchKernelGGL(xent_bwd_kernel, dim3(a->max_rows), dim3(256), 0, (hipStream_t)s, *a, (uint16_t*)dlogits, ldd, gscale);
    return check_launch("vk_xent_bwd");
}
extern "C" int vk_kl_fwd(const vk_kl_args* a, vk_stream_t s) {
    if (a->max_rows <= 0) return 0;
    hipLaunchKernelGGL(kl_fwd_kernel, dim3(a->max_rows), dim3(256), 0, (hipStream_t)s, *a);
    return check_launch("vk_kl_fwd");
}
extern "C" int vk_kl_bwd(const vk_kl_args* a, void* dlogits, int ldd, const float* gscale, vk_stream_t s) {
    if (a->max_rows <= 0) return 0;
    if (ldd < a->V) return set_error("vk_kl_bwd: ldd < V");
    hipLaunchKernelGGL(kl_bwd_kernel, dim3(a->max_rows), dim3(256), 0, (hipStream_t)s, *a, (uint16_t*)dlogits, ldd, gscale);
    return check_launch("vk_kl_bwd");
}
extern "C" int vk_loss_finalize(const float* sums, const int32_t* n_t, const int32_t* n_v, int B, float kl_weight, float* losses, vk_stream_t s) {
    hipLaunchKernelGGL(loss_finalize_kernel, dim3(1), dim3(64), 0, (hipStream_t)s, sums, n_t, n_v, B, kl_weight, losses);
    return check_launch("vk_loss_finalize");
}
extern "C" int vk_pool_mul_fwd(const void* pt, const void* pv, void* out, int B, int P, vk_dropout drop, vk_stream_t s) {
    hipLaunchKernelGGL(pool_mul_fwd_kernel, dim3((B * P + 255) / 256), dim3(256), 0, (hipStream_t)s, (const uint16_t*)pt, (const uint16_t*)pv, (uint16_t*)out, B, P, drop);
    return check_launch("vk_pool_mul_fwd");
}
extern "C" int vk_pool_mul_bwd(const void* dp, int ldp, const void* pt, const void* pv, void* dyt, void* dyv, int B, int P, vk_dropout drop, vk_stream_t s) {
    hipLaunchKernelGGL(pool_mul_bwd_kernel, dim3((B * P + 255) / 256), dim3(256), 0, (hipStream_t)s, (const uint16_t*)dp, ldp, (const uint16_t*)pt,
                       (const uint16_t*)pv, (uint16_t*)dyt, (uint16_t*)dyv, B, P, drop);
    return check_launch("vk_pool_mul_bwd");
}
extern "C" int vk_mask_prep(const int64_t* mask, float* out, int n, vk_stream_t s) {
    if (n <= 0) return 0;
    hipLaunchKernelGGL(mask_prep_kernel, dim3((n + 255) / 256), dim3(256), 0, (hipStream_t)s, mask, out, n);
    return check_launch("vk_mask_prep");
}
```

volta_amd/csrc/layernorm.hip:

```cpp
#include "common.h"
#include "../../include/volta_hip.h"
#include "util.h"

namespace vk {

constexpr float LN_EPS = 1e-12f;
constexpr int LN_THREADS = 256;
constexpr int LN_BWD_ROWS = 16;

__device__ __forceinline__ uint32_t drop_row(const vk_drop_rows (&seg)[2], int split, int row, uint32_t& site) {
    const int si = row >= split ? 1 : 0;
    const int r = si ? row - split : row;
    site = seg[si].site;
    if (seg[si].div <= 0) return (uint32_t)r;
    return (uint32_t)((r / seg[si].div) * seg[si].mul + (r % seg[si].div) + seg[si].off);
}

__device__ __forceinline__ void load4(const uint16_t* p, float (&v)[4]) {
    u32x2 r = *(const u32x2*)p;
    v[0] = bf2f(r[0] & 0xFFFF); v[1] = bf2f(r[0] >> 16); v[2] = bf2f(r[1] & 0xFFFF); v[3] = bf2f(r[1] >> 16);
}
__device__ __forceinline__ void store4(uint16_t* p, const float (&v)[4]) {
    *(u32x2*)p = u32x2{pack2bf(v[0], v[1]), pack2bf(v[2], v[3])};
}
// ... 290 lines not shown
        for (int b = ty; b < nblk; b += 16) s += partial[(size_t)b * 2 * H + i];
    red[ty][tx] = s;
    __syncthreads();
    if (ty == 0 && i < 2 * H) {
#pragma unroll
        for (int k = 1; k < 16; ++k) s += red[k][tx];
        float* o = i < H ? dgamma + i : dbeta + (i - H);
        *o = accumulate ? *o + s : s;
    }
}

}

static int ln_check(int H, int maxH, const char* who) {
    if (H % 4 || H > maxH || H <= 0) return vk::set_error("%s: H=%d must be a multiple of 4, <= %d", who, H, maxH);
    return 0;
}

extern "C" int vk_ln_fwd_pair(const vk_ln_args* a, const vk_ln_args* b, vk_stream_t stream) {
    using namespace vk;
    if (ln_check(a->H, 2048, "vk_ln_fwd")) return -1;
    if (b && (b->H != a->H || a->dyn || b->dyn)) return set_error("vk_ln_fwd_pair: both jobs need the same H and static row counts");
    const int nb0 = a->M > 0 ? (a->M + 3) / 4 : 0, nb1 = (b && b->M > 0) ? (b->M + 3) / 4 : 0;
    if (nb0 + nb1 == 0) return 0;
    const int nch = (a->H + 255) / 256;
    dim3 grid(nb0 + nb1), block(LN_THREADS);
    hipStream_t s = (hipStream_t)stream;
    JobPair<vk_ln_args> jp;
    jp.job[0] = *a;
    jp.job[1] = b ? *b : *a;
    jp.nb0 = nb0;
    jp.stagger = jp.stagger_mod = 0;
    switch (nch) {
        case 1: hipLaunchKernelGGL(ln_fwd_kernel<1>, grid, block, 0, s, jp); break;
        case 2: hipLaunchKernelGGL(ln_fwd_kernel<2>, grid, block, 0, s, jp); break;
        case 3: hipLaunchKernelGGL(ln_fwd_kernel<3>, grid, block, 0, s, jp); break;
        case 4: hipLaunchKernelGGL(ln_fwd_kernel<4>, grid, block, 0, s, jp); break;
        default: hipLaunchKernelGGL(ln_fwd_kernel<8>, grid, block, 0, s, jp); break;
    }
    return check_launch("vk_ln_fwd");
}

extern "C" int vk_ln_fwd(const vk_ln_args* a, vk_stream_t stream) { return vk_ln_fwd_pair(a, nullptr, stream); }

extern "C" int vk_ln_bwd_partial_rows(int M) { return (M + vk::LN_BWD_ROWS - 1) / vk::LN_BWD_ROWS; }

#ifdef VK_STUDY
static unsigned long long* g_ln_stamps = nullptr;
static int g_ln_stagger = 0, g_ln_stagger_mod = 0;
extern "C" void vk_ln_set_stamp_buffer(unsigned long long* p) { g_ln_stamps = p; }
extern "C" void vk_ln_set_stagger(int ticks, int mod) { g_ln_stagger = ticks; g_ln_stagger_mod = mod; }
#else
static constexpr unsigned long long* g_ln_stamps = nullptr;
static constexpr int g_ln_stagger = 0, g_ln_stagger_mod = 0;
#endif

static void ln_finalize_launch(const vk_ln_bwd_args* a, hipStream_t s) {
    hipLaunchKernelGGL(vk::ln_bwd_finalize_kernel, dim3((2 * a->H + 63) / 64), dim3(1024), 0, s, a->partial, vk_ln_bwd_partial_rows(a->M), a->H,
                       a->dgamma, a->dbeta, a->accumulate & 1);
}

extern "C" int vk_ln_bwd_pair(const vk_ln_bwd_args* a, const vk_ln_bwd_args* b, vk_stream_t stream) {
    using namespace vk;
    if (ln_check(a->H, 2048, "vk_ln_bwd")) return -1;
    if (b && (b->H != a->H || a->dyn || b->dyn)) return set_error("vk_ln_bwd_pair: both jobs need the same H and static row counts");
    if (b && !a->partial != !b->partial) {
        if (vk_ln_bwd_pair(a, nullptr, stream)) return -1;
        return vk_ln_bwd_pair(b, nullptr, stream);
    }
    const bool params = a->partial != nullptr;
    if (!params && !a->dz && !a->dd && (!b || (!b->dz && !b->dd))) return 0;
    const int nb0 = a->M > 0 ? vk_ln_bwd_partial_rows(a->M) : 0, nb1 = (b && b->M > 0) ? vk_ln_bwd_partial_rows(b->M) : 0;
    const int nch = (a->H + 255) / 256;
    dim3 grid(nb0 + nb1), block(LN_THREADS);
    hipStream_t s = (hipStream_t)stream;
    JobPair<vk_ln_bwd_args> jp;
    jp.job[0] = *a;
    jp.job[1] = b ? *b : *a;
    jp.nb0 = nb0;
    jp.stagger = g_ln_stagger; jp.stagger_mod = g_ln_stagger_mod;
    if (nb0 + nb1 && params) switch (nch) {
        case 1: hipLaunchKernelGGL(ln_bwd_kernel<1>, grid, block, 0, s, jp, g_ln_stamps); break;
        case 2: hipLaunchKernelGGL(ln_bwd_kernel<2>, grid, block, 0, s, jp, g_ln_stamps); break;
        case 3: hipLaunchKernelGGL(ln_bwd_kernel<3>, grid, block, 0, s, jp, g_ln_stamps); break;
        case 4: hipLaunchKernelGGL(ln_bwd_kernel<4>, grid, block, 0, s, jp, g_ln_stamps); break;
        case 5: case 6: hipLaunchKernelGGL(ln_bwd_kernel<6>, grid, block, 0, s, jp, g_ln_stamps); break;
        default: hipLaunchKernelGGL(ln_bwd_kernel<8>, grid, block, 0, s, jp, g_ln_stamps); break;
    }
    if (nb0 + nb1 && !params) switch (nch) {
        case 1: hipLaunchKernelGGL(ln_bwd_dx_kernel<1>, grid, block, 0, s, jp, g_ln_stamps); break;
        case 2: hipLaunchKernelGGL(ln_bwd_dx_kernel<2>, grid, block, 0, s, jp, g_ln_stamps); break;
        case 3: hipLaunchKernelGGL(ln_bwd_dx_kernel<3>, grid, block, 0, s, jp, g_ln_stamps); break;
        case 4: hipLaunchKernelGGL(ln_bwd_dx_kernel<4>, grid, block, 0, s, jp, g_ln_stamps); break;
        case 5: case 6: hipLaunchKernelGGL(ln_bwd_dx_kernel<6>, grid, block, 0, s, jp, g_ln_stamps); break;
        default: hipLaunchKernelGGL(ln_bwd_dx_kernel<8>, grid, block, 0, s, jp, g_ln_stamps); break;
    }
    if (!params) return check_launch("vk_ln_bwd");
    if ((nb0 || !(a->accumulate & 1)) && !(a->accumulate & 2)) ln_finalize_launch(a, s);
    if (b && (nb1 || !(b->accumulate & 1)) && !(b->accumulate & 2)) ln_finalize_launch(b, s);
    return check_launch("vk_ln_bwd");
}

extern "C" int vk_ln_bwd(const vk_ln_bwd_args* a, vk_stream_t stream) { return vk_ln_bwd_pair(a, nullptr, stream); }

extern "C" int vk_ln_bwd_finalize(const vk_ln_bwd_args* a, vk_stream_t stream) {
    if (!a->partial) return vk::set_error("vk_ln_bwd_finalize: the job has no partial records (partial NULL: gamma and beta frozen)");
    if (a->M <= 0 && (a->accumulate & 1)) return 0;
    ln_finalize_launch(a, (hipStream_t)stream);
    return vk::check_launch("vk_ln_bwd_finalize");
}
```

volta_amd/csrc/misc.hip:

```cpp
#include "common.h"
#include "../../include/volta_hip.h"
#include "util.h"

namespace vk {

__global__ void set_seed_kernel(uint64_t* p, uint64_t v) { *p = v; }

__global__ void cast_f32_bf16_kernel(const float* __restrict__ src, uint16_t* __restrict__ dst, size_t n) {
    const size_t n8 = n >> 3;
    for (size_t i = (size_t)blockIdx.x * blockDim.x + threadIdx.x; i < n8; i += (size_t)gridDim.x * blockDim.x) {
        const f32x4 a = __builtin_nontemporal_load((const f32x4*)(src + i * 8)), b = __builtin_nontemporal_load((const f32x4*)(src + i * 8 + 4));
        *(u32x4*)(dst + i * 8) = u32x4{pack2bf(a[0], a[1]), pack2bf(a[2], a[3]), pack2bf(b[0], b[1]), pack2bf(b[2], b[3])};
    }
    if (blockIdx.x == 0 && threadIdx.x < (n & 7)) dst[n8 * 8 + threadIdx.x] = f2bf(src[n8 * 8 + threadIdx.x]);
}

__global__ void mul_bf16_kernel(const uint16_t* a, const uint16_t* b, uint16_t* out, size_t n, const int32_t* dyn_rows, int row_len) {
    if (dyn_rows) { const size_t lim = (size_t)(*dyn_rows) * row_len; if (lim < n) n = lim; }
    const size_t n8 = n >> 3;
    for (size_t i = (size_t)blockIdx.x * blockDim.x + threadIdx.x; i < n8; i += (size_t)gridDim.x * blockDim.x) {
        const u32x4 x = *(const u32x4*)(a + i * 8), y = *(const u32x4*)(b + i * 8);
        u32x4 o;
#pragma unroll
        for (int k = 0; k < 4; ++k) o[k] = pack2bf(bf2f(x[k] & 0xFFFF) * bf2f(y[k] & 0xFFFF), bf2f(x[k] >> 16) * bf2f(y[k] >> 16));
        *(u32x4*)(out + i * 8) = o;
    }
}

}

extern "C" int vk_mul_bf16(const void* a, const void* b, void* out, int64_t n, const int32_t* dyn_rows, int row_len, vk_stream_t s) {
    if (n <= 0) return 0;
    if (n % 8 || row_len % 8) return vk::set_error("vk_mul_bf16: n and row_len must be multiples of 8");
    if (((uintptr_t)a & 15) || ((uintptr_t)b & 15) || ((uintptr_t)out & 15)) return vk::set_error("vk_mul_bf16: 16-byte alignment required");
    int64_t blocks = (n / 8 + 255) / 256;
    if (blocks > 4096) blocks = 4096;
    hipLaunchKernelGGL(vk::mul_bf16_kernel, dim3((unsigned)blocks), dim3(256), 0, (hipStream_t)s, (const uint16_t*)a, (const uint16_t*)b,
                       (uint16_t*)out, (size_t)n, dyn_rows, row_len);
    return vk::check_launch("vk_mul_bf16");
}

extern "C" int vk_set_seed(uint64_t* seed_dev, uint64_t seed, vk_stream_t s) {
    hipLaunchKernelGGL(vk::set_seed_kernel, dim3(1), dim3(1), 0, (hipStream_t)s, seed_dev, seed);
    return vk::check_launch("vk_set_seed");
}

extern "C" int vk_cast_f32_bf16(const float* src, void* dst, int64_t n, vk_stream_t s) {
    if (n <= 0) return 0;
    if (((uintptr_t)src & 15) || ((uintptr_t)dst & 15)) return vk::set_error("vk_cast_f32_bf16: 16-byte alignment required");
    int64_t blocks = (n / 8 + 255) / 256;
    if (blocks > 4096) blocks = 4096;
    if (blocks < 1) blocks = 1;
    hipLaunchKernelGGL(vk::cast_f32_bf16_kernel, dim3((unsigned)blocks), dim3(256), 0, (hipStream_t)s, src, (uint16_t*)dst, (size_t)n);
    return vk::check_launch("vk_cast_f32_bf16");
}

namespace vk {
__global__ __launch_bounds__(512) void mfma_peak_kernel(const uint32_t* seed, float* out, int iters) {
    typedef __attribute__((ext_vector_type(8))) short v8;
    typedef __attribute__((ext_vector_type(4))) float v4;
    v8 a[4], b[4];
    const uint32_t s = seed[threadIdx.x & 63] + blockIdx.x;
#pragma unroll
    for (int i = 0; i < 4; ++i)
#pragma unroll
        for (int k = 0; k < 8; ++k) {
            a[i][k] = (short)(0x3C00 + ((s * (i * 8 + k + 1) * 2654435761u) >> 22));
            b[i][k] = (short)(0xBC00 + ((s * (i * 8 + k + 77) * 40503u) >> 22));
        }
    v4 acc[4][4];
#pragma unroll
    for (int i = 0; i < 4; ++i)
#pragma unroll
        for (int j = 0; j < 4; ++j) acc[i][j] = v4{0.f, 0.f, 0.f, 0.f};
    for (int it = 0; it < iters; ++it) {
#pragma unroll
        for (int i = 0; i < 4; ++i)
#pragma unroll
            for (int j = 0; j < 4; ++j) acc[i][j] = __builtin_amdgcn_mfma_f32_16x16x32_bf16(a[i], b[j], acc[i][j], 0, 0, 0);
    }
    float t = 0.f;
#pragma unroll
    for (int i = 0; i < 4; ++i)
#pragma unroll
        for (int j = 0; j < 4; ++j) t += acc[i][j][0] + acc[i][j][1] + acc[i][j][2] + acc[i][j][3];
    if (t == 12345.678f) out[0] = t;
}
}

extern "C" int vk_mfma_peak(const uint32_t* seed64, float* out, int iters, int blocks, vk_stream_t stream) {
    hipLaunchKernelGGL(vk::mfma_peak_kernel, dim3(blocks), dim3(512), 0, (hipStream_t)stream, seed64, out, iters);
    return vk::check_launch("vk_mfma_peak");
}

namespace vk {
__global__ void hold_cus_kernel(unsigned ticks) {
    extern __shared__ char smem[];
    if (threadIdx.x == 0) {
        smem[0] = 1;
        const unsigned long long t0 = __builtin_amdgcn_s_memrealtime();
        while (__builtin_amdgcn_s_memrealtime() - t0 < ticks) __builtin_amdgcn_s_sleep(16);
    }
}
}

extern "C" int vk_hold_cus(int nwg, int usec, int whole_cu, vk_stream_t stream) {
    if (nwg <= 0 || usec <= 0) return 0;
    if (nwg > 256 || usec > 100000) return vk::set_error("vk_hold_cus: at most 256 workgroups for at most 0.1 s (got %d, %d us)", nwg, usec);
    constexpr int LDS = 160 * 1024;
    static const hipError_t attr = hipFuncSetAttribute((const void*)vk::hold_cus_kernel, hipFuncAttributeMaxDynamicSharedMemorySize, LDS); (void)attr;
    hipLaunchKernelGGL(vk::hold_cus_kernel, dim3(nwg), dim3(64), whole_cu ? LDS : 64, (hipStream_t)stream, (unsigned)usec * 100u);
    return vk::check_launch("vk_hold_cus");
}

namespace vk {
__global__ __launch_bounds__(256) void comm_standin_kernel(const u32x4* __restrict__ src, u32x4* __restrict__ dst, size_t n16, unsigned min_ticks,
                                                           unsigned long long* stamps) {
    const unsigned long long t0 = __builtin_amdgcn_s_memrealtime();
    if (stamps && threadIdx.x == 0) atomicMin(stamps, t0);
    const size_t per = (n16 + gridDim.x - 1) / gridDim.x, lo = per * blockIdx.x, hi = lo + per < n16 ? lo + per : n16;
    for (size_t i = lo + threadIdx.x; i < hi; i += 256) __builtin_nontemporal_store(__builtin_nontemporal_load(src + i), dst + i);
    if (threadIdx.x == 0) {
        const unsigned long long first = stamps ? __hip_atomic_load(stamps, __ATOMIC_RELAXED, __HIP_MEMORY_SCOPE_AGENT) : t0;
        while (__builtin_amdgcn_s_memrealtime() - first < min_ticks) __builtin_amdgcn_s_sleep(32);
        if (stamps) atomicMax(stamps + 1, __builtin_amdgcn_s_memrealtime());
    }
}
}

extern "C" int vk_comm_standin(const void* src, void* dst, int64_t bytes, int nwg, int min_usec, uint64_t* stamps, vk_stream_t stream) {
    if (bytes <= 0 || nwg <= 0) return 0;
    if ((bytes & 15) || ((uintptr_t)src & 15) || ((uintptr_t)dst & 15)) return vk::set_error("vk_comm_standin: 16-byte granularity");
    if (nwg > 1024 || min_usec < 0 || min_usec > 100000) return vk::set_error("vk_comm_standin: at most 1024 workgroups, at most 0.1 s");
    hipLaunchKernelGGL(vk::comm_standin_kernel, dim3(nwg), dim3(256), 0, (hipStream_t)stream, (const vk::u32x4*)src, (vk::u32x4*)dst, (size_t)(bytes / 16),
                       (unsigned)min_usec * 100u, (unsigned long long*)stamps);
    return vk::check_launch("vk_comm_standin");
}

namespace vk {
__global__ void gate_wait_kernel(const unsigned long long* flag, const unsigned long long* stamp, unsigned timeout_ticks, int32_t* err) {
    if (threadIdx.x != 0) return;
    const unsigned long long want = __hip_atomic_load(stamp, __ATOMIC_RELAXED, __HIP_MEMORY_SCOPE_AGENT);
    const unsigned long long t0 = __builtin_amdgcn_s_memrealtime();
    while (__hip_atomic_load(flag, __ATOMIC_RELAXED, __HIP_MEMORY_SCOPE_AGENT) != want) {
        __builtin_amdgcn_s_sleep(16);
        if (__builtin_amdgcn_s_memrealtime() - t0 > timeout_ticks) {
            if (err) __hip_atomic_store(err, 2, __ATOMIC_RELAXED, __HIP_MEMORY_SCOPE_AGENT);
            break;
        }
    }
}
__global__ void bump_u64_kernel(unsigned long long* w) { *w += 1ull; }
__global__ void store_u64_kernel(unsigned long long* w, unsigned long long v) { __hip_atomic_store(w, v, __ATOMIC_RELAXED, __HIP_MEMORY_SCOPE_AGENT); }
__global__ void gate_value_kernel(const unsigned long long* flag, unsigned long long want, unsigned timeout_ticks, int32_t* err) {
    if (threadIdx.x != 0) return;
    const unsigned long long t0 = __builtin_amdgcn_s_memrealtime();
    while (__hip_atomic_load(flag, __ATOMIC_RELAXED, __HIP_MEMORY_SCOPE_AGENT) != want) {
        __builtin_amdgcn_s_sleep(16);
        if (__builtin_amdgcn_s_memrealtime() - t0 > timeout_ticks) {
            if (err) __hip_atomic_store(err, 2, __ATOMIC_RELAXED, __HIP_MEMORY_SCOPE_AGENT);
            break;
        }
    }
}
}

extern "C" int vk_store_u64(uint64_t* word, uint64_t value, vk_stream_t stream) {
    if (!word) return vk::set_error("vk_store_u64: NULL");
    hipLaunchKernelGGL(vk::store_u64_kernel, dim3(1), dim3(1), 0, (hipStream_t)stream, (unsigned long long*)word, (unsigned long long)value);
    return vk::check_launch("vk_store_u64");
}

extern "C" int vk_gate_value(const uint64_t* flag, uint64_t want, int timeout_us, int32_t* err, vk_stream_t stream) {
    if (!flag || timeout_us <= 0 || timeout_us > 10000000) return vk::set_error("vk_gate_value: flag and 0 < timeout_us <= 10000000");
    hipLaunchKernelGGL(vk::gate_value_kernel, dim3(1), dim3(64), 0, (hipStream_t)stream, (const unsigned long long*)flag, (unsigned long long)want,
                       (unsigned)(timeout_us > 40000000 ? 4000000000u : (unsigned)timeout_us * 100u), err);
    return vk::check_launch("vk_gate_value");
}

extern "C" int vk_gate_wait(const uint64_t* flag, const uint64_t* stamp, int timeout_us, int32_t* err, vk_stream_t stream) {
    if (!flag || !stamp || timeout_us <= 0 || timeout_us > 1000000) return vk::set_error("vk_gate_wait: flag, stamp and 0 < timeout_us <= 1000000");
    hipLaunchKernelGGL(vk::gate_wait_kernel, dim3(1), dim3(64), 0, (hipStream_t)stream, (const unsigned long long*)flag, (const unsigned long long*)stamp,
                       (unsigned)timeout_us * 100u, err);
    return vk::check_launch("vk_gate_wait");
}

extern "C" int vk_bump_u64(uint64_t* word, vk_stream_t stream) {
    if (!word) return vk::set_error("vk_bump_u64: NULL");
    hipLaunchKernelGGL(vk::bump_u64_kernel, dim3(1), dim3(1), 0, (hipStream_t)stream, (unsigned long long*)word);
    return vk::check_launch("vk_bump_u64");
}
```

volta_amd/csrc/optim.hip:

```cpp
#include "common.h"
#include "../../include/volta_hip.h"
#include "util.h"

namespace vk {

constexpr int NORM_BLOCKS = 1024;

__global__ __launch_bounds__(256) void sqnorm_partial_kernel(const float* g, size_t n4, float* partial, const uint8_t* chunk_class) {
    __shared__ float sh[4];
    float s = 0.f;
    for (size_t i = (size_t)blockIdx.x * 256 + threadIdx.x; i < n4; i += (size_t)gridDim.x * 256) {
        if (chunk_class && chunk_class[i >> 8] == VK_CHUNK_SKIP) continue;
        const f32x4 v = *(const f32x4*)(g + i * 4);
        s += v[0] * v[0] + v[1] * v[1] + v[2] * v[2] + v[3] * v[3];
    }
    s = wave_sum(s);
    if ((threadIdx.x & 63) == 0) sh[threadIdx.x >> 6] = s;
    __syncthreads();
    if (threadIdx.x == 0) partial[blockIdx.x] = sh[0] + sh[1] + sh[2] + sh[3];
}
__global__ __launch_bounds__(256) void sqnorm_final_kernel(const float* partial, int nblk, float pre_scale, float max_norm, float* out) {
    __shared__ double sh[4];
    double s = 0.0;
    for (int i = threadIdx.x; i < nblk; i += 256) s += (double)partial[i];
// ... 263 lines not shown
            for (int k = 1; k < 16; ++k) s += red[k][tx];
            float* o = i < H ? J.dst + i : J.dst2 + (i - H);
            *o = J.accumulate ? *o + s : s;
        }
    }
}

}

using namespace vk;

extern "C" int vk_side_tail(const vk_tail_job* jobs, int njobs, vk_stream_t s) {
    if (njobs <= 0) return 0;
    if (njobs > VK_TAIL_MAX_JOBS) return set_error("vk_side_tail: %d jobs (max %d)", njobs, VK_TAIL_MAX_JOBS);
    TailJobs t;
    t.njobs = njobs;
    int total = 0;
    for (int i = 0; i < njobs; ++i) {
        t.j[i] = jobs[i];
        vk_tail_job& J = t.j[i];
        int nb;
        if (J.kind == 0) {
            if ((J.stride & 3) || ((uintptr_t)J.dst & 15) || ((uintptr_t)J.src & 15)) return set_error("vk_side_tail: slab job %d needs 16-byte alignment", i);
            nb = (int)((J.n / 4 + 255) / 256);
            if (nb < 1) nb = 1;
        } else if (J.kind == 1) {
            nb = (int)((2 * J.n + 15) / 16);
        } else return set_error("vk_side_tail: unknown job kind %d", J.kind);
        if (J.n <= 0 || J.count <= 0) nb = 0;
        J.block_start = total;
        total += nb;
    }
    if (total == 0) return 0;
    hipLaunchKernelGGL(side_tail_kernel, dim3((unsigned)total), dim3(256), 0, (hipStream_t)s, t);
    return check_launch("vk_side_tail");
}

extern "C" int vk_sum_slabs_bf16(void* dst, const float* src, int64_t slab_stride, int nslabs, int64_t n, const int32_t* dyn_rows, int row_len, vk_stream_t s) {
    if (n <= 0 || nslabs <= 0) return 0;
    if ((slab_stride & 3) || (n & 3) || (row_len & 3)) return set_error("vk_sum_slabs_bf16: lengths must be multiples of 4");
    if (((uintptr_t)src & 15) || ((uintptr_t)dst & 7)) return set_error("vk_sum_slabs_bf16: src needs 16-byte, dst 8-byte alignment");
    int64_t blocks = (n / 4 + 255) / 256;
    if (blocks > 2048) blocks = 2048;
    hipLaunchKernelGGL(sum_slabs_bf16_kernel, dim3((unsigned)blocks), dim3(256), 0, (hipStream_t)s, (uint16_t*)dst, src, (size_t)slab_stride, nslabs, (size_t)n, dyn_rows, row_len);
    return check_launch("vk_sum_slabs_bf16");
}

extern "C" int vk_sum_slabs_f32(float* dst, const float* src, int64_t slab_stride, int nslabs, int64_t n, vk_stream_t s) {
    if (n <= 0 || nslabs <= 0) return 0;
    if ((slab_stride & 3) || ((uintptr_t)dst & 15) || ((uintptr_t)src & 15)) return set_error("vk_sum_slabs_f32: 16-byte alignment required");
    int64_t blocks = (n / 4 + 255) / 256;
    if (blocks > 2048) blocks = 2048;
    if (blocks < 1) blocks = 1;
    hipLaunchKernelGGL(sum_slabs_kernel, dim3((unsigned)blocks), dim3(256), 0, (hipStream_t)s, dst, src, (size_t)slab_stride, nslabs, (size_t)n);
    return check_launch("vk_sum_slabs_f32");
}

extern "C" int vk_grad_norm_workspace_floats(void) { return NORM_BLOCKS; }

extern "C" int vk_grad_norm_clip_masked(const float* g, int64_t n, const uint8_t* chunk_class, float pre_scale, float max_norm, float* partial, float* out, vk_stream_t s) {
    if (n % 4 || ((uintptr_t)g & 15)) return set_error("vk_grad_norm_clip: n %% 4 == 0 and 16-byte alignment required");
    if (chunk_class && (n % 1024)) return set_error("vk_grad_norm_clip_masked: a chunk mask needs an arena of whole 1024-element chunks");
    hipStream_t st = (hipStream_t)s;
    hipLaunchKernelGGL(sqnorm_partial_kernel, dim3(NORM_BLOCKS), dim3(256), 0, st, g, (size_t)(n / 4), partial, chunk_class);
    hipLaunchKernelGGL(sqnorm_final_kernel, dim3(1), dim3(256), 0, st, partial, NORM_BLOCKS, pre_scale, max_norm, out);
    return check_launch("vk_grad_norm_clip");
}

extern "C" int vk_grad_sqnorm_chunks(const float* g, int64_t chunk0, int64_t nchunks, const uint8_t* chunk_class, float* sums, vk_stream_t s) {
    if (chunk0 < 0 || nchunks < 0 || ((uintptr_t)g & 15)) return set_error("vk_grad_sqnorm_chunks: bad range or alignment");
    if (nchunks == 0) return 0;
    hipLaunchKernelGGL(sqnorm_chunks_kernel, dim3((unsigned)((nchunks + 3) / 4)), dim3(256), 0, (hipStream_t)s, g, (size_t)chunk0, (size_t)nchunks, chunk_class, sums);
    return check_launch("vk_grad_sqnorm_chunks");
}

extern "C" int vk_grad_norm_from_chunks(float* sums, int64_t total_chunks, float pre_scale, float max_norm, float* out, vk_stream_t s) {
    if (total_chunks <= 0) return set_error("vk_grad_norm_from_chunks: no chunks");
    if (((uintptr_t)(sums + total_chunks)) & 7) return set_error("vk_grad_norm_from_chunks: total_chunks must be even (the group sums follow the chunk sums as doubles)");
    double* group = (double*)(sums + total_chunks);
    hipLaunchKernelGGL(sqnorm_groups_kernel, dim3(SQ_GROUPS), dim3(256), 0, (hipStream_t)s, sums, (size_t)total_chunks, group);
    hipLaunchKernelGGL(sqnorm_from_groups_kernel, dim3(1), dim3(64), 0, (hipStream_t)s, (const double*)group, pre_scale, max_norm, out);
    return check_launch("vk_grad_norm_from_chunks");
}

extern "C" int vk_grad_norm_clip(const float* g, int64_t n, float pre_scale, float max_norm, float* partial, float* out, vk_stream_t s) {
    return vk_grad_norm_clip_masked(g, n, nullptr, pre_scale, max_norm, partial, out, s);
}

extern "C" int vk_adamw_step(const vk_adamw_args* a, vk_stream_t s) {
    if (a->n % 1024) return set_error("vk_adamw_step: arena length must be a multiple of 1024 elements");
    if (a->n == 0) return 0;
    hipLaunchKernelGGL(adamw_kernel, dim3((unsigned)(a->n / 1024)), dim3(256), 0, (hipStream_t)s, *a);
    return check_launch("vk_adamw_step");
}

extern "C" int vk_adamw_step_on(const vk_adamw_args* a, int ncus, vk_stream_t s) {
    if (a->n % 1024) return set_error("vk_adamw_step_on: arena length must be a multiple of 1024 elements");
    if (ncus < 1 || ncus > 256) return set_error("vk_adamw_step_on: %d compute units", ncus);
    if (a->n == 0) return 0;
    constexpr int FOOTPRINT = 96 * 1024;
    static const hipError_t attr = hipFuncSetAttribute((const void*)adamw_narrow_kernel, hipFuncAttributeMaxDynamicSharedMemorySize, FOOTPRINT); (void)attr;
    hipLaunchKernelGGL(adamw_narrow_kernel, dim3((unsigned)ncus), dim3(512), FOOTPRINT, (hipStream_t)s, *a);
    return check_launch("vk_adamw_step_on");
}

static int list_blocks(int64_t max_numel, int cap) {
    int64_t b = (max_numel + 1023) / 1024;
    return (int)(b < 1 ? 1 : b > cap ? cap : b);
}

extern "C" int vk_adamw_step_list(const vk_adamw_args* a, const vk_adamw_tensor* list, int n, int64_t max_numel, vk_stream_t s) {
    if (n < 0 || n > 65535 || max_numel < 0) return set_error("vk_adamw_step_list: %d tensors, max numel %lld", n, (long long)max_numel);
    if (n == 0 || max_numel == 0) return 0;
    hipLaunchKernelGGL(adamw_list_kernel, dim3((unsigned)list_blocks(max_numel, 1024), (unsigned)n), dim3(256), 0, (hipStream_t)s, *a, list);
    return check_launch("vk_adamw_step_list");
}

extern "C" int vk_grad_sqnorm_list_work_floats(void) { return 2 * SQ_LIST_BLOCKS; }

extern "C" int vk_grad_sqnorm_list(const vk_adamw_tensor* list, int n, int64_t max_numel, float* work, float* sums, vk_stream_t s) {
    if (n < 0 || n > 65535 || max_numel < 0) return set_error("vk_grad_sqnorm_list: %d tensors, max numel %lld", n, (long long)max_numel);
    if (n == 0) return 0;
    if ((uintptr_t)work & 7) return set_error("vk_grad_sqnorm_list: work needs 8-byte alignment");
    hipLaunchKernelGGL(sqnorm_list_partial_kernel, dim3(SQ_LIST_BLOCKS, (unsigned)n), dim3(256), 0, (hipStream_t)s, list, (double*)work);
    hipLaunchKernelGGL(sqnorm_list_final_kernel, dim3((unsigned)n), dim3(64), 0, (hipStream_t)s, (const double*)work, sums);
    return check_launch("vk_grad_sqnorm_list");
// ... 17 lines not shown
```

volta_amd/csrc/pairs.hip:

```cpp
#include "common.h"
#include "../../include/volta_hip.h"
#include "util.h"

namespace vk {

__global__ __launch_bounds__(256) void pair_gather_kernel(const vk_pair_gather_args a) {
    const int p = blockIdx.x, k = blockIdx.y, t = threadIdx.x;
    const int side = a.side[k];
    int64_t item;
    if (a.cap_idx) item = side ? a.img_idx[p] : a.cap_idx[p];
    else item = side ? (int64_t)a.i0 + p % a.ni : (int64_t)a.c0 + p / a.ni;
    const bool ok = item >= 0 && item < a.n_items[side];
    const int64_t nb = a.bytes[k];
    const char* __restrict__ src = (const char*)a.src[k] + (ok ? item : 0) * nb;
    char* __restrict__ dst = (char*)a.dst[k] + (int64_t)p * nb;
    int64_t done = 0;
    if ((((uintptr_t)src | (uintptr_t)dst) & 15) == 0) {
        const u32x4* __restrict__ s4 = (const u32x4*)src;
        u32x4* __restrict__ d4 = (u32x4*)dst;
        const int64_t n16 = nb >> 4;
        const u32x4 z = {0u, 0u, 0u, 0u};
        int64_t j = t;
        for (; j + 3 * 256 < n16; j += 4 * 256) {
            const u32x4 v0 = ok ? s4[j] : z, v1 = ok ? s4[j + 256] : z, v2 = ok ? s4[j + 512] : z, v3 = ok ? s4[j + 768] : z;
// ... 2 lines not shown
            d4[j + 512] = v2;
            d4[j + 768] = v3;
        }
        for (; j < n16; j += 256) d4[j] = ok ? s4[j] : z;
        done = n16 << 2;
    }
    const uint32_t* __restrict__ s1 = (const uint32_t*)src;
    uint32_t* __restrict__ d1 = (uint32_t*)dst;
    for (int64_t j = done + t; j < (nb >> 2); j += 256) d1[j] = ok ? s1[j] : 0u;
}

}

using namespace vk;

extern "C" int vk_pair_gather(const vk_pair_gather_args* a, vk_stream_t s) {
    if (a->nseg < 1 || a->nseg > VK_PAIR_MAX_SEGS || a->npairs < 0) return set_error("vk_pair_gather: %d segments (1..%d), %d pairs", a->nseg, VK_PAIR_MAX_SEGS, a->npairs);
    if (!a->cap_idx != !a->img_idx) return set_error("vk_pair_gather: cap_idx and img_idx are given together or not at all");
    if (a->n_items[0] < 0 || a->n_items[1] < 0) return set_error("vk_pair_gather: negative item count");
    if (!a->cap_idx && a->npairs > 0) {
        if (a->nc <= 0 || a->ni <= 0 || (int64_t)a->nc * a->ni != a->npairs || a->c0 < 0 || a->i0 < 0 ||
            (int64_t)a->c0 + a->nc > a->n_items[0] || (int64_t)a->i0 + a->ni > a->n_items[1])
            return set_error("vk_pair_gather: cross product captions [%d, +%d) x images [%d, +%d) does not fit %d pairs of %lld x %lld items", a->c0, a->nc,
                             a->i0, a->ni, a->npairs, (long long)a->n_items[0], (long long)a->n_items[1]);
    }
    for (int k = 0; k < a->nseg; ++k) {
        if (!a->src[k] || !a->dst[k] || a->bytes[k] <= 0 || (a->bytes[k] & 3) || (a->side[k] != 0 && a->side[k] != 1) ||
            ((uintptr_t)a->src[k] & 3) || ((uintptr_t)a->dst[k] & 3))
            return set_error("vk_pair_gather: segment %d (bytes %lld, side %d): buffers 4-byte aligned, bytes a positive multiple of 4, side 0 | 1", k,
                             (long long)a->bytes[k], a->side[k]);
        if (a->n_items[a->side[k]] <= 0) return set_error("vk_pair_gather: segment %d reads side %d, which has no items", k, a->side[k]);
    }
    if (a->npairs == 0) return 0;
    hipLaunchKernelGGL(pair_gather_kernel, dim3((unsigned)a->npairs, (unsigned)a->nseg), dim3(256), 0, (hipStream_t)s, *a);
    return check_launch("vk_pair_gather");
}
```

volta_amd/csrc/util.h:

```cpp
#pragma once
#include <hip/hip_runtime.h>
#include <cstdarg>
#include <cstdio>

namespace vk {
char* error_buffer();
int set_error(const char* fmt, ...);
int check_launch(const char* what);
}
```

volta_amd/csrc/vislosses.hip:

```cpp
#include "common.h"
#include "../../include/volta_hip.h"
#include "util.h"

namespace vk {

__device__ __forceinline__ float vl_block_sum(float v, float* sh) {
    v = wave_sum(v);
    const int lane = threadIdx.x & 63, wave = threadIdx.x >> 6;
    __syncthreads();
    if (lane == 0) sh[wave] = v;
    __syncthreads();
    return sh[0] + sh[1] + sh[2] + sh[3];
}
__device__ __forceinline__ float vl_block_max(float v, float* sh) {
    v = wave_max(v);
    const int lane = threadIdx.x & 63, wave = threadIdx.x >> 6;
    __syncthreads();
    if (lane == 0) sh[wave] = v;
    __syncthreads();
    return fmaxf(fmaxf(sh[0], sh[1]), fmaxf(sh[2], sh[3]));
}

template <bool HUBER>
__global__ __launch_bounds__(256) void vis_reg_fwd_kernel(vk_vis_loss_args a) {
// ... 201 lines not shown
        for (int k = 0; k < K; ++k) opos[(size_t)b * K + k] = c + (k == K - 1);
    }
    for (int o = 32; o; o >>= 1) lo = min(lo, __shfl_xor(lo, o));
    if ((tid & 63) == 0) s_min[tid >> 6] = lo;
    __syncthreads();
    lo = s_min[0];
    for (int w = 1; w < 16; ++w) lo = min(lo, s_min[w]);
    for (int i = tid; i < B * T; i += 1024) {
        const int t = i % T;
        tpos[i] = t + (t >= lo ? K : 0);
    }
}

}

using namespace vk;

static int check_vis(const vk_vis_loss_args* a, const char* who) {
    if (a->kind != VK_VIS_MSE && a->kind != VK_VIS_NCE && a->kind != VK_VIS_XENT && a->kind != VK_VIS_HUBER) return set_error("%s: unknown kind %d", who, a->kind);
    if (!a->logits || !a->pos || !a->count || !a->loss_sum || a->ld < a->V) return set_error("%s: missing logits / pos / count / loss_sum, or ld < V", who);
    if (a->kind == VK_VIS_XENT && (!a->labels || !a->lse)) return set_error("%s: xent needs labels and lse", who);
    if ((a->kind == VK_VIS_MSE || a->kind == VK_VIS_HUBER || a->kind == VK_VIS_NCE) && !a->target) return set_error("%s: regression / nce need the feature matrix", who);
    if (a->kind == VK_VIS_NCE && (!a->neg_index || !a->aux || !a->lse || a->n_neg < 1 || a->n_neg + 1 > VK_NCE_MAX_SAMPLES || a->V % 4 || a->ld % 4))
        return set_error("%s: nce needs neg_index, aux, lse, 1 <= n_neg < %d and V, ld multiples of 4", who, VK_NCE_MAX_SAMPLES);
    return 0;
}

extern "C" int vk_vis_loss_fwd(const vk_vis_loss_args* a, vk_stream_t s) {
    if (check_vis(a, "vk_vis_loss_fwd")) return -1;
    if (a->max_rows <= 0) return 0;
    const dim3 grid(a->max_rows), block(256);
    hipStream_t st = (hipStream_t)s;
    switch (a->kind) {
        case VK_VIS_MSE: hipLaunchKernelGGL(vis_reg_fwd_kernel<false>, grid, block, 0, st, *a); break;
        case VK_VIS_HUBER: hipLaunchKernelGGL(vis_reg_fwd_kernel<true>, grid, block, 0, st, *a); break;
        case VK_VIS_XENT: hipLaunchKernelGGL(vis_xent_fwd_kernel, grid, block, 0, st, *a); break;
        default: hipLaunchKernelGGL(vis_nce_fwd_kernel, grid, block, 0, st, *a); break;
    }
    return check_launch("vk_vis_loss_fwd");
}

extern "C" int vk_vis_loss_bwd(const vk_vis_loss_args* a, void* dlogits, int ldd, const float* gscale, vk_stream_t s) {
    if (check_vis(a, "vk_vis_loss_bwd")) return -1;
    if (ldd < a->V) return set_error("vk_vis_loss_bwd: ldd < V");
    if (a->max_rows <= 0) return 0;
    const dim3 grid(a->max_rows), block(256);
    hipStream_t st = (hipStream_t)s;
    uint16_t* d = (uint16_t*)dlogits;
    switch (a->kind) {
        case VK_VIS_MSE: hipLaunchKernelGGL(vis_reg_bwd_kernel<false>, grid, block, 0, st, *a, d, ldd, gscale); break;
        case VK_VIS_HUBER: hipLaunchKernelGGL(vis_reg_bwd_kernel<true>, grid, block, 0, st, *a, d, ldd, gscale); break;
        case VK_VIS_XENT: hipLaunchKernelGGL(vis_xent_bwd_kernel, grid, block, 0, st, *a, d, ldd, gscale); break;
        default: hipLaunchKernelGGL(vis_nce_bwd_kernel, grid, block, 0, st, *a, d, ldd, gscale); break;
    }
    return check_launch("vk_vis_loss_bwd");
}

extern "C" int vk_nce_negatives(vk_dropout rng, int B, int R, int32_t* out, vk_stream_t s) {
    if (!rng.seed || B < 2 || R < 2) return set_error("vk_nce_negatives: needs a seed word, B >= 2 and R >= 2 (losses.py:50,59 draw from [0, B-1) and [0, R-1))");
    hipLaunchKernelGGL(nce_negatives_kernel, dim3(B * R), dim3(128), 0, (hipStream_t)s, rng, B, R, out);
    return check_launch("vk_nce_negatives");
}

extern "C" int vk_pool_fuse_fwd(const void* pt, const void* pv, void* out, int B, int P, int mode, vk_dropout drop, vk_stream_t s) {
    if (mode < VK_FUSE_MUL || mode > VK_FUSE_TEXT || (mode != VK_FUSE_TEXT && !pv)) return set_error("vk_pool_fuse_fwd: mode %d (mul 0 | sum 1 | text 2; pv required unless text)", mode);
    hipLaunchKernelGGL(pool_fuse_fwd_kernel, dim3((B * P + 255) / 256), dim3(256), 0, (hipStream_t)s, (const uint16_t*)pt, (const uint16_t*)pv, (uint16_t*)out, B, P, mode, drop);
    return check_launch("vk_pool_fuse_fwd");
}
extern "C" int vk_pool_fuse_bwd(const void* dp, int ldp, const void* pt, const void* pv, void* dyt, void* dyv, int B, int P, int mode, vk_dropout drop, vk_stream_t s) {
    if (mode < VK_FUSE_MUL || mode > VK_FUSE_TEXT || (mode != VK_FUSE_TEXT && (!pv || !dyv))) return set_error("vk_pool_fuse_bwd: mode %d (mul 0 | sum 1 | text 2; pv, dyv required unless text)", mode);
    hipLaunchKernelGGL(pool_fuse_bwd_kernel, dim3((B * P + 255) / 256), dim3(256), 0, (hipStream_t)s, (const uint16_t*)dp, ldp, (const uint16_t*)pt,
                       (const uint16_t*)pv, (uint16_t*)dyt, (uint16_t*)dyv, B, P, mode, drop);
    return check_launch("vk_pool_fuse_bwd");
}

extern "C" int vk_text_end_rows(const int64_t* ids, int B, int T, int32_t* rows, int32_t* count, vk_stream_t s) {
    if (B <= 0 || T <= 0) return set_error("vk_text_end_rows: bad arguments");
    hipLaunchKernelGGL(text_end_rows_kernel, dim3(B), dim3(64), 0, (hipStream_t)s, ids, B, T, rows, count);
    return check_launch("vk_text_end_rows");
}

extern "C" int vk_vlbert_obj_ids(const int32_t* zero_flag, int64_t* ids, int M, int K, vk_stream_t s) {
    if (M <= 0 || K <= 0) return set_error("vk_vlbert_obj_ids: bad arguments");
    hipLaunchKernelGGL(vlbert_obj_ids_kernel, dim3((M + 255) / 256), dim3(256), 0, (hipStream_t)s, zero_flag, ids, M, K);
    return check_launch("vk_vlbert_obj_ids");
}

extern "C" int vk_vlbert_positions(const int64_t* ids, int B, int T, int K, int64_t* tpos, int64_t* opos, vk_stream_t s) {
    if (B <= 0 || T <= 0 || K <= 0 || !ids || !tpos || !opos) return set_error("vk_vlbert_positions: bad arguments");
    hipLaunchKernelGGL(vlbert_positions_kernel, dim3(1), dim3(1024), 0, (hipStream_t)s, ids, B, T, K, tpos, opos);
    return check_launch("vk_vlbert_positions");
}
```

volta_amd/engine/arena.py:

```python
import math

import torch

from .. import _lib as L
from .._lib import check, ptr
from .plan import _round_up

CHUNK = 1024
NO_DECAY = ("bias", "LayerNorm.bias", "LayerNorm.weight")


class ParamArena:

    def __init__(self, model, device, prefix=""):
        named = [(prefix + n, p) for n, p in model.named_parameters()]
        byname = dict(named)
        slots, seen = [], set()
        for name, p in named:
            if name in seen:
                continue
            group = [name]
            for q in ("query", "v_query"):
                tag = ".attention_self.%s." % q
                if tag in name and name.rsplit(".", 1)[1] in ("weight", "bias"):
# ... 74 lines not shown
        if force or self.shadow_version != v:
            self.sync_optimizer()
            check(L.lib.vk_cast_f32_bf16(ptr(self.master), ptr(self.shadow), self.total, L.stream_ptr()))
            self.shadow_version = v
            self.weights_epoch += 1

    def mark_shadow_fresh(self):
        self.shadow_version = self.param_version()
        self.weights_epoch += 1

    def fp8_weight(self, w):
        key = w.data_ptr()
        if key not in self.fp8_sites:
            N, K = w.shape
            Kp = _round_up(K, 128)
            self.fp8_sites[key] = (w, torch.zeros(N, Kp, dtype=torch.uint8, device=self.device), torch.ones(N, dtype=torch.float32, device=self.device))
            self.fp8_epoch = -1
        return self.fp8_sites[key][1:]

    def refresh_fp8(self):
        if self.fp8_epoch == self.weights_epoch:
            return
        for w, q, sc in self.fp8_sites.values():
            N, K = w.shape
            check(L.lib.vk_quant_rows_fp8(ptr(w), 1, w.stride(0), ptr(q), q.stride(0), ptr(sc), N, K, None, L.stream_ptr()))
        self.fp8_epoch = self.weights_epoch

    def invalidate_shadow(self):
        self.shadow_version = -1

    def sync_optimizer(self):
        pend = self.opt_pending
        if pend:
            cur = torch.cuda.current_stream()
            for ev in pend[1]:
                cur.wait_event(ev)
            self.opt_pending = None
```

volta_amd/engine/builder.py:

```python
import ctypes as C
import os
import re

import torch

from .. import _lib as L
from .._lib import check, ptr
from ..modules import sublayer_schedule
from .arena import CHUNK
from .embeddings import EmbeddingBuilders
from .heads import HeadBuilders
from .plan import (EV_DECODER_WGRAD, EV_IMAGE_EMB_BWD, EV_IMAGE_EMB_FWD, EV_WGRAD_RING, NODROP, Plan, _addr, _mk_segs, _round_up, op, side_begin, side_end, wait_side)
from .sublayers import SublayerBuilders


def frozen_blocks(arena, heads="pretrain"):
    blocks = {}
    if heads == "pretrain":
        blocks["decoder"] = ["bert.embeddings.word_embeddings.weight"]
    for name in arena.params:
        m = re.match(r"bert\.(v_)?embeddings\.", name)
        if m:
            key = m.group(0)
        elif heads == "pretrain" and name == "cls.predictions.bias":
# ... 549 lines not shown
        key = tuple(bounds)
        cache = self._fwd_segments
        if key in cache:
            return cache[key]

        def need(prefixes):
            hi = max((arena.offset[nm] + int(torch.tensor(arena.shape[nm]).prod()) for nm in arena.params if nm.startswith(tuple(prefixes))), default=0)
            hi_chunk = -(-hi // CHUNK)
            return next((i + 1 for i, b in enumerate(bounds) if b >= hi_chunk), len(bounds))

        nemb = len(self.stage_prefix) - len(self.fwd_sub_start)
        cuts = [(need(self.stage_prefix[0] if nemb else ["bert.embeddings."]), 0)]
        for k, start in enumerate(self.fwd_sub_start):
            cuts.append((need(self.stage_prefix[nemb + k]), start))
        cuts.append((len(bounds), self.fwd_heads_start))
        segs, cur_need = [], 0
        for i, (nd, start) in enumerate(cuts):
            end = cuts[i + 1][1] if i + 1 < len(cuts) else len(self.fwd.ops)
            nd = max(nd, cur_need)
            if segs and nd == cur_need:
                segs[-1] = (nd, segs[-1][1], end)
            else:
                segs.append((nd, start, end))
            cur_need = nd
        cache[key] = segs
        return segs

    def run_forward(self):
        pend = self.arena.opt_pending
        if not pend:
            self.fwd.run()
            return
        bounds, events = pend
        cur = torch.cuda.current_stream()
        waited = 0
        for nd, start, end in self.fwd_segments(bounds):
            for i in range(waited, nd):
                cur.wait_event(events[i])
            waited = max(waited, nd)
            self.fwd.run(start, end)
        self.arena.opt_pending = None

    def bind_inputs(self, tensors):
        for name, sites in self.inputs.items():
            t = tensors[name]
            addr = t.data_ptr()
            for struct, field, index in sites:
                if index is None:
                    setattr(struct, field, addr)
                else:
                    getattr(struct, field)[index] = addr

    def prepare_step(self, seed):
        if self.train or self.nce_site is not None:
            check(L.lib.vk_set_seed(ptr(self.seed), C.c_uint64(seed & 0xFFFFFFFFFFFFFFFF), L.stream_ptr()))
```

volta_amd/optimization.py:

```python
import ctypes as C
import math

import numpy as np
import torch
import weakref

from torch.optim import Optimizer
from torch.optim.lr_scheduler import LambdaLR

from . import _lib as L


def _split_params(params, labels=None):
    labels = labels or ["parameter %d" % i for i in range(len(params))]
    owners, foreign = {}, []
    for p, lab in zip(params, labels):
        o = getattr(p, "_vk_owner", None)
        if o is not None:
            owners.setdefault(id(o), (o, lab))
        else:
            foreign.append((p, lab))
    if len(owners) > 1:
        (_, a), (_, b) = list(owners.values())[:2]
        raise RuntimeError("volta_amd optimizers take the parameters of at most one volta_amd model: %s and %s belong to different models" % (a, b))
# ... 198 lines not shown
        red = getattr(ddp, "reducer", None)
        if red is None or red.mode != "zero1" or not (red.sharded or red.replicated):
            return None
        return red

    def _step_zero1(self, a, arena, red):
        f = self._fused
        layout = tuple(red.sharded)
        prev = f.get("zero1_layout")
        if prev is not None and prev != layout:
            red.gather(f["m"], prev)
            red.gather(f["v"], prev)
        f["zero1_layout"] = layout
        base = (a.p, a.g, a.m, a.v, a.shadow, a.chunk_class)
        for lo, hi in red.owned():
            assert lo % 1024 == 0 and hi % 1024 == 0 and hi > lo, (lo, hi)
            a.p, a.g, a.m, a.v = base[0] + 4 * lo, base[1] + 4 * lo, base[2] + 4 * lo, base[3] + 4 * lo
            a.shadow, a.chunk_class = base[4] + 2 * lo, base[5] + lo // 1024
            a.n = hi - lo
            L.check(L.lib.vk_adamw_step(C.byref(a), L.stream_ptr()))
        f["model"]._ddp.gather_params(arena)

    def _step_pipelined(self, a, arena, clip):
        f = self._fused
        if "stream" not in f:
            n = max(1, min(self._overlap[1], arena.total // 1024))
            nchunks = arena.total // 1024
            from .streams import independent_stream, engine_streams
            ddp = getattr(f["model"], "_ddp", None)
            comm = getattr(getattr(ddp, "reducer", None), "stream", None)
            with torch.cuda.device(arena.device):
                f["stream"] = independent_stream(engine_streams(), device=arena.device, soft_avoid=[comm] if comm is not None else [])
            f["bounds"] = [nchunks * (i + 1) // n for i in range(n)]
            f["events"] = [torch.cuda.Event() for _ in range(n)]
        side, bounds, events = f["stream"], f["bounds"], f["events"]
        side.wait_stream(torch.cuda.current_stream())
        if clip is not None:
            clip.record_stream(side)
        base = (a.p, a.g, a.m, a.v, a.shadow, a.chunk_class)
        with torch.cuda.stream(side):
            sp = C.c_void_p(side.cuda_stream)
            lo = 0
            for hi, ev in zip(bounds, events):
                if hi > lo:
                    off = lo * 1024
                    a.p, a.g, a.m, a.v = base[0] + 4 * off, base[1] + 4 * off, base[2] + 4 * off, base[3] + 4 * off
                    a.shadow, a.chunk_class = base[4] + 2 * off, base[5] + lo
                    a.n = (hi - lo) * 1024
                    L.check(L.lib.vk_adamw_step(C.byref(a), sp))
                ev.record(side)
                lo = hi
        arena.opt_pending = (bounds, events)

    def synchronize(self):
        if self._fused is not None and self._fused["arena"] is not None:
            self._fused["arena"].sync_optimizer()

    def _spans(self):
        arena = self._fused["arena"]
        byptr = {p.data_ptr(): n for n, p in arena.params.items()} if arena is not None else {}
        fmap = {id(t["p"]): t for t in self._fused.get("foreign", ())}
        out = []
        for g in self.param_groups:
            for p in g["params"]:
                if id(p) in fmap:
                    out.append(fmap[id(p)])
                    continue
                n = byptr[p.data_ptr()]
                numel = 1
                for d in arena.shape[n]:
                    numel *= d
                out.append((arena.offset[n], numel, tuple(arena.shape[n])))
        return out

    def consolidate_state_dict(self):
        self.synchronize()
        if self._fused is None:
            return
        f = self._fused
        red = self._zero1_reducer()
        if red is not None and f.get("zero1_layout"):
            red.gather(f["m"], f["zero1_layout"])
            red.gather(f["v"], f["zero1_layout"])
        f["zero1_consolidated_at"] = f["step"]
# ... 515 lines not shown
```

Measured before the change: 15670.

## Record events via launch macro and batch pipelined AdamW ranges in C

Replaces hipLaunchKernelGGL with a VK_LAUNCH macro that can attach an armed event to a launch. The op executor uses it to skip separate hipEventRecord calls at side-stream fork and join points. The pipelined AdamW step now runs all chunk ranges and records their events in one C call, and stream waits use raw HIP events instead of torch Event objects. The aim is to cut Python and HIP API overhead per step, at the cost of extra launch-macro complexity and thread-local event state.

```diff
diff --git a/include/volta_hip.h b/include/volta_hip.h
--- a/include/volta_hip.h
+++ b/include/volta_hip.h
@@ -318,6 +318,9 @@
     float lr, beta1, beta2, eps, step_mult, grad_scale;
 } vk_adamw_args;
 int vk_adamw_step(const vk_adamw_args* a, vk_stream_t s);
+void* vk_event_create(void);
+int vk_stream_wait_event(vk_stream_t s, void* event);
+int vk_adamw_step_ranges(const vk_adamw_args* a, const int64_t* bounds, int n, void* const* events, vk_stream_t s);
 int vk_adamw_step_on(const vk_adamw_args* a, int ncus, vk_stream_t s);
 typedef struct vk_adamw_tensor {
     float* p;
diff --git a/volta_amd/_lib.py b/volta_amd/_lib.py
--- a/volta_amd/_lib.py
+++ b/volta_amd/_lib.py
@@ -342,6 +342,9 @@
 _sig("vk_grad_norm_clip", C.c_int, c_p, C.c_int64, C.c_float, C.c_float, c_p, c_p, c_p)
 _sig("vk_adamw_step", C.c_int, C.POINTER(AdamwArgs), c_p)
 _sig("vk_adamw_step_on", C.c_int, C.POINTER(AdamwArgs), C.c_int, c_p)
+_sig("vk_event_create", c_p)
+_sig("vk_stream_wait_event", C.c_int, c_p, c_p)
+_sig("vk_adamw_step_ranges", C.c_int, C.POINTER(AdamwArgs), C.POINTER(C.c_int64), C.c_int, C.POINTER(c_p), c_p)
 _sig("vk_grad_norm_clip_masked", C.c_int, c_p, C.c_int64, c_p, C.c_float, C.c_float, c_p, c_p, c_p)
 _sig("vk_adamw_step_list", C.c_int, C.POINTER(AdamwArgs), c_p, C.c_int, C.c_int64, c_p)
 _sig("vk_grad_sqnorm_list", C.c_int, c_p, C.c_int, C.c_int64, c_p, c_p, c_p)
@@ -399,7 +402,7 @@
            "vk_relu_bwd_bf16", "vk_copy_async", "vk_select_rows", "vk_gather_rows", "vk_scatter_rows_add", "vk_xent_fwd",
            "vk_xent_bwd", "vk_kl_fwd", "vk_kl_bwd", "vk_loss_finalize", "vk_pool_mul_fwd", "vk_pool_mul_bwd",
            "vk_pool_fuse_fwd", "vk_pool_fuse_bwd", "vk_text_end_rows", "vk_vlbert_obj_ids", "vk_vlbert_positions", "vk_vis_loss_fwd", "vk_vis_loss_bwd", "vk_nce_negatives", "vk_task_loss_work_bytes", "vk_task_loss_fwd", "vk_task_loss_bwd",
-           "vk_mask_prep", "vk_mul_bf16", "vk_grad_norm_workspace_floats", "vk_grad_norm_clip", "vk_grad_norm_clip_masked", "vk_grad_sqnorm_chunks", "vk_grad_norm_from_chunks", "vk_adamw_step", "vk_adamw_step_on", "vk_adamw_step_list", "vk_grad_sqnorm_list", "vk_grad_sqnorm_list_work_floats", "vk_grad_seed", "vk_pair_gather", "vk_radam_step", "vk_radam_step_list",
+           "vk_mask_prep", "vk_mul_bf16", "vk_grad_norm_workspace_floats", "vk_grad_norm_clip", "vk_grad_norm_clip_masked", "vk_grad_sqnorm_chunks", "vk_grad_norm_from_chunks", "vk_adamw_step", "vk_adamw_step_on", "vk_adamw_step_ranges", "vk_event_create", "vk_stream_wait_event", "vk_adamw_step_list", "vk_grad_sqnorm_list", "vk_grad_sqnorm_list_work_floats", "vk_grad_seed", "vk_pair_gather", "vk_radam_step", "vk_radam_step_list",
            "vk_axpy_f32", "vk_sum_slabs_f32", "vk_sum_slabs_bf16", "vk_memset_async", "vk_hold_cus", "vk_gate_wait", "vk_bump_u64", "vk_store_u64", "vk_gate_value", "vk_comm_standin", "vk_gemm_reserve_cus", "vk_side_tail", "vk_run_ops", "vk_run_ops_timed", "vk_side_join", "vk_side_join_from", "vk_side_stream", "vk_side_enable", "vk_concap_batch",
            "vk_lmdb_open", "vk_lmdb_close", "vk_lmdb_entries", "vk_lmdb_first", "vk_lmdb_next", "vk_lmdb_get", "vk_concap_record_decode", "vk_concap_records_decode", "vk_b64_decode",
            "vk_wordpiece_open", "vk_wordpiece_close", "vk_wordpiece_vocab_size", "vk_wordpiece_token_id", "vk_wordpiece_encode", "vk_wordpiece_encode_batch",
diff --git a/volta_amd/csrc/attention.hip b/volta_amd/csrc/attention.hip
--- a/volta_amd/csrc/attention.hip
+++ b/volta_amd/csrc/attention.hip
@@ -496,11 +496,11 @@
     int waves = nq_tiles < 4 ? 4 : (nq_tiles > 8 ? 8 : nq_tiles);
     if (g_attn_fwd_waves >= 4 && g_attn_fwd_waves < waves && 4 * lds <= 160 * 1024) waves = g_attn_fwd_waves;
     if (DHT == 64 && g_attn_fwd_occ == 5) {
-        hipLaunchKernelGGL((attn_fwd_kernel<TP, RP, 5, DHT>), dim3(k.B * k.nh), dim3(64 * waves), lds, s, k);
+        VK_LAUNCH((attn_fwd_kernel<TP, RP, 5, DHT>), dim3(k.B * k.nh), dim3(64 * waves), lds, s, k);
     } else {
         auto kern = attn_fwd_kernel<TP, RP, (DHT == 64 ? 4 : 3), DHT>;
         static const hipError_t attr = hipFuncSetAttribute((const void*)kern, hipFuncAttributeMaxDynamicSharedMemorySize, lds); (void)attr;
-        hipLaunchKernelGGL(kern, dim3(k.B * k.nh), dim3(64 * waves), lds, s, k);
+        VK_LAUNCH(kern, dim3(k.B * k.nh), dim3(64 * waves), lds, s, k);
     }
     return check_launch("vk_gated_attn_fwd");
 }
@@ -514,13 +514,13 @@
         auto kern = attn_bwd_kernel<TP, RP, 3, DHT>;
         static const hipError_t attr = hipFuncSetAttribute((const void*)kern, hipFuncAttributeMaxDynamicSharedMemorySize, lds); (void)attr;
         int waves = g_attn_bwd_waves < 4 ? 4 : (ntasks > g_attn_bwd_waves ? g_attn_bwd_waves : (ntasks < 4 ? 4 : ntasks));
-        hipLaunchKernelGGL(kern, dim3(k.B * k.nh), dim3(64 * waves), lds, s, k);
+        VK_LAUNCH(kern, dim3(k.B * k.nh), dim3(64 * waves), lds, s, k);
     } else {
         auto kern = attn_bwd_kernel<TP, RP, 2, DHT>;
         static const hipError_t attr = hipFuncSetAttribute((const void*)kern, hipFuncAttributeMaxDynamicSharedMemorySize, lds); (void)attr;
         int waves = g_attn_bwd_waves < 4 ? 4 : (ntasks > g_attn_bwd_waves ? g_attn_bwd_waves : (ntasks < 4 ? 4 : ntasks));
         if (2 * lds > 160 * 1024) waves = ntasks >= 8 ? 8 : (ntasks < 4 ? 4 : ntasks);
-        hipLaunchKernelGGL(kern, dim3(k.B * k.nh), dim3(64 * waves), lds, s, k);
+        VK_LAUNCH(kern, dim3(k.B * k.nh), dim3(64 * waves), lds, s, k);
     }
     return check_launch("vk_gated_attn_bwd");
 }
diff --git a/volta_amd/csrc/attention_generic.hip b/volta_amd/csrc/attention_generic.hip
--- a/volta_amd/csrc/attention_generic.hip
+++ b/volta_amd/csrc/attention_generic.hip
@@ -283,12 +283,12 @@
     if (bwd) {
         auto kern = attn_generic_bwd_kernel<D, NS>;
         if (hipFuncSetAttribute((const void*)kern, hipFuncAttributeMaxDynamicSharedMemorySize, (int)lds) != hipSuccess) return set_error("vk_gated_attn_bwd: cannot reserve %zu bytes of LDS", lds);
-        hipLaunchKernelGGL(kern, dim3(k.B * k.nh), dim3(64 * GW), lds, s, k);
+        VK_LAUNCH(kern, dim3(k.B * k.nh), dim3(64 * GW), lds, s, k);
         return check_launch("vk_gated_attn_bwd (generic kernel)");
     }
     auto kern = attn_generic_fwd_kernel<D, NS>;
     if (hipFuncSetAttribute((const void*)kern, hipFuncAttributeMaxDynamicSharedMemorySize, (int)lds) != hipSuccess) return set_error("vk_gated_attn_fwd: cannot reserve %zu bytes of LDS", lds);
-    hipLaunchKernelGGL(kern, dim3(k.B * k.nh), dim3(64 * GW), lds, s, k);
+    VK_LAUNCH(kern, dim3(k.B * k.nh), dim3(64 * GW), lds, s, k);
     return check_launch("vk_gated_attn_fwd (generic kernel)");
 }
 
diff --git a/volta_amd/csrc/backbone.hip b/volta_amd/csrc/backbone.hip
--- a/volta_amd/csrc/backbone.hip
+++ b/volta_amd/csrc/backbone.hip
@@ -56,6 +56,6 @@
     const int64_t total = (int64_t)a->B * a->L * (a->H / 8);
     int64_t blocks = (total + 255) / 256;
     if (blocks > 2048) blocks = 2048;
-    hipLaunchKernelGGL(grad_seed_kernel, dim3((unsigned)blocks), dim3(256), 0, (hipStream_t)s, *a);
+    VK_LAUNCH(grad_seed_kernel, dim3((unsigned)blocks), dim3(256), 0, (hipStream_t)s, *a);
     return check_launch("vk_grad_seed");
 }
diff --git a/volta_amd/csrc/capi.cpp b/volta_amd/csrc/capi.cpp
--- a/volta_amd/csrc/capi.cpp
+++ b/volta_amd/csrc/capi.cpp
@@ -3,7 +3,9 @@
 
 namespace vk {
 static thread_local char g_err[512] = {0};
+static thread_local hipEvent_t g_launch_event = nullptr;
 char* error_buffer() { return g_err; }
+hipEvent_t& launch_event_slot() { return g_launch_event; }
 int set_error(const char* fmt, ...) {
     va_list ap;
     va_start(ap, fmt);
diff --git a/volta_amd/csrc/embed.hip b/volta_amd/csrc/embed.hip
--- a/volta_amd/csrc/embed.hip
+++ b/volta_amd/csrc/embed.hip
@@ -577,7 +577,7 @@
                                   int M, int F, int dim, vk_dropout drop, vk_stream_t s) {
     if (F % 4 || (8 * dim) % 4 || nloc < 4) return set_error("vk_vlbert_prep_fwd: F and 8*dim must be multiples of 4, nloc >= 4");
     if (M <= 0) return 0;
-    hipLaunchKernelGGL(vlbert_prep_kernel, dim3((M + 3) / 4), dim3(256), 0, (hipStream_t)s, loc, nloc, feat, mask_emb, (uint16_t*)out, zero_flag, M, F, dim, drop);
+    VK_LAUNCH(vlbert_prep_kernel, dim3((M + 3) / 4), dim3(256), 0, (hipStream_t)s, loc, nloc, feat, mask_emb, (uint16_t*)out, zero_flag, M, F, dim, drop);
     return check_launch("vk_vlbert_prep_fwd");
 }
 
@@ -589,14 +589,14 @@
     hipStream_t st = (hipStream_t)s;
     if (nch <= 4) hipLaunchKernelGGL(vlbert_maskgrad_kernel<4>, dim3(nblk), dim3(256), 0, st, (const uint16_t*)dx, ldx, col0, zero_flag, partial, M, F, drop);
     else hipLaunchKernelGGL(vlbert_maskgrad_kernel<8>, dim3(nblk), dim3(256), 0, st, (const uint16_t*)dx, ldx, col0, zero_flag, partial, M, F, drop);
-    hipLaunchKernelGGL(colsum_finalize_kernel, dim3((F + 63) / 64), dim3(1024), 0, st, partial, nblk, F, out, 0);
+    VK_LAUNCH(colsum_finalize_kernel, dim3((F + 63) / 64), dim3(1024), 0, st, partial, nblk, F, out, 0);
     return check_launch("vk_vlbert_maskgrad");
 }
 
 extern "C" int vk_rowgroup_sum_bf16(const void* in, void* out, int B, int T, int H, vk_stream_t s) {
     if (H % 4) return set_error("vk_rowgroup_sum_bf16: H %% 4 != 0");
     if (B <= 0) return 0;
-    hipLaunchKernelGGL(rowgroup_sum_kernel, dim3(B, (H + 255) / 256), dim3(64), 0, (hipStream_t)s, (const uint16_t*)in, (uint16_t*)out, T, H);
+    VK_LAUNCH(rowgroup_sum_kernel, dim3(B, (H + 255) / 256), dim3(64), 0, (hipStream_t)s, (const uint16_t*)in, (uint16_t*)out, T, H);
     return check_launch("vk_rowgroup_sum_bf16");
 }
 
@@ -605,7 +605,7 @@
     if (n <= 0) return 0;
     int64_t blocks = (n / 8 + 255) / 256;
     if (blocks > 4096) blocks = 4096;
-    hipLaunchKernelGGL(relu_bwd_kernel, dim3((unsigned)blocks), dim3(256), 0, (hipStream_t)s, (const uint16_t*)dy, (const uint16_t*)y, (uint16_t*)out, (size_t)(n / 8));
+    VK_LAUNCH(relu_bwd_kernel, dim3((unsigned)blocks), dim3(256), 0, (hipStream_t)s, (const uint16_t*)dy, (const uint16_t*)y, (uint16_t*)out, (size_t)(n / 8));
     return check_launch("vk_relu_bwd_bf16");
 }
 
@@ -619,7 +619,7 @@
 extern "C" int vk_embed_sum_fwd(const vk_embed_args* a, vk_stream_t s) {
     if (a->H % 4) return set_error("vk_embed_sum_fwd: H %% 4 != 0");
     if (a->M <= 0) return 0;
-    hipLaunchKernelGGL(embed_sum_fwd_kernel, dim3((a->M + 3) / 4), dim3(256), 0, (hipStream_t)s, *a);
+    VK_LAUNCH(embed_sum_fwd_kernel, dim3((a->M + 3) / 4), dim3(256), 0, (hipStream_t)s, *a);
     return check_launch("vk_embed_sum_fwd");
 }
 
@@ -686,10 +686,10 @@
     const dim3 grid((M + 4 * LOC_ROWS - 1) / (4 * LOC_ROWS)), block(256);
     hipStream_t st = (hipStream_t)s;
     switch ((H + 255) / 256) {
-        case 1: hipLaunchKernelGGL(loc_linear_fwd_kernel<1>, grid, block, 0, st, loc, W, bias, (uint16_t*)out, M, H, nloc); break;
-        case 2: hipLaunchKernelGGL(loc_linear_fwd_kernel<2>, grid, block, 0, st, loc, W, bias, (uint16_t*)out, M, H, nloc); break;
-        case 3: hipLaunchKernelGGL(loc_linear_fwd_kernel<3>, grid, block, 0, st, loc, W, bias, (uint16_t*)out, M, H, nloc); break;
-        default: hipLaunchKernelGGL(loc_linear_fwd_kernel<4>, grid, block, 0, st, loc, W, bias, (uint16_t*)out, M, H, nloc); break;
+        case 1: VK_LAUNCH(loc_linear_fwd_kernel<1>, grid, block, 0, st, loc, W, bias, (uint16_t*)out, M, H, nloc); break;
+        case 2: VK_LAUNCH(loc_linear_fwd_kernel<2>, grid, block, 0, st, loc, W, bias, (uint16_t*)out, M, H, nloc); break;
+        case 3: VK_LAUNCH(loc_linear_fwd_kernel<3>, grid, block, 0, st, loc, W, bias, (uint16_t*)out, M, H, nloc); break;
+        default: VK_LAUNCH(loc_linear_fwd_kernel<4>, grid, block, 0, st, loc, W, bias, (uint16_t*)out, M, H, nloc); break;
     }
     return check_launch("vk_loc_linear_fwd");
 }
@@ -707,15 +707,15 @@
         case 3: hipLaunchKernelGGL(loc_linear_bwd_kernel<3>, dim3(nblk), dim3(256), 0, st, (const uint16_t*)dz, loc, partial, M, H, nloc); break;
         default: hipLaunchKernelGGL(loc_linear_bwd_kernel<4>, dim3(nblk), dim3(256), 0, st, (const uint16_t*)dz, loc, partial, M, H, nloc); break;
     }
-    hipLaunchKernelGGL(loc_linear_bwd_finalize_kernel, dim3((9 * H + 63) / 64), dim3(1024), 0, st, partial, nblk, H, nloc, dW, db);
+    VK_LAUNCH(loc_linear_bwd_finalize_kernel, dim3((9 * H + 63) / 64), dim3(1024), 0, st, partial, nblk, H, nloc, dW, db);
     return check_launch("vk_loc_linear_bwd");
 }
 
 extern "C" int vk_add_dropout(const void* a, const void* b, void* y, int M, int H, float scale, vk_dropout drop, int backward, vk_stream_t s) {
     if (H % 4) return set_error("vk_add_dropout: H %% 4 != 0");
     if (M <= 0) return 0;
-    hipLaunchKernelGGL(add_dropout_kernel, dim3((M + 3) / 4), dim3(256), 0, (hipStream_t)s, (const uint16_t*)a, (const uint16_t*)b,
-                       (uint16_t*)y, M, H, scale, drop, backward);
+    VK_LAUNCH(add_dropout_kernel, dim3((M + 3) / 4), dim3(256), 0, (hipStream_t)s, (const uint16_t*)a, (const uint16_t*)b,
+              (uint16_t*)y, M, H, scale, drop, backward);
     return check_launch("vk_add_dropout");
 }
 
@@ -730,6 +730,6 @@
         case 3: hipLaunchKernelGGL(colsum_kernel<3>, dim3(nblk), dim3(256), 0, st, (const uint16_t*)src, partial, M, H); break;
         default: hipLaunchKernelGGL(colsum_kernel<4>, dim3(nblk), dim3(256), 0, st, (const uint16_t*)src, partial, M, H); break;
     }
-    hipLaunchKernelGGL(colsum_finalize_kernel, dim3((H + 63) / 64), dim3(1024), 0, st, partial, nblk, H, out, accumulate);
+    VK_LAUNCH(colsum_finalize_kernel, dim3((H + 63) / 64), dim3(1024), 0, st, partial, nblk, H, out, accumulate);
     return check_launch("vk_colsum_bf16");
 }
diff --git a/volta_amd/csrc/executor.cpp b/volta_amd/csrc/executor.cpp
--- a/volta_amd/csrc/executor.cpp
+++ b/volta_amd/csrc/executor.cpp
@@ -71,8 +71,11 @@
 extern "C" int vk_run_ops(const vk_op* ops, int n, vk_stream_t s) {
     vk_stream_t cur = s;
     Side* g = nullptr;
+    hipEvent_t rode = nullptr;
     for (int i = 0; i < n; ++i) {
         const vk_op& o = ops[i];
+        const hipEvent_t rode_here = rode;
+        rode = nullptr;
         if (o.kind >= VK_OP_SIDE_BEGIN && o.kind <= VK_OP_JOIN) {
             if (!g_side_enabled) continue;
             if (!g && !(g = side_for(s))) return -1;
@@ -80,14 +83,14 @@
             switch (o.kind) {
                 case VK_OP_SIDE_BEGIN:
                     if (o.i0 != 1) {
-                        e = hipEventRecord(g->fork, (hipStream_t)s);
+                        if (rode_here != g->fork) e = hipEventRecord(g->fork, (hipStream_t)s);
                         if (e == hipSuccess) e = hipStreamWaitEvent(g->stream, g->fork, 0);
                     }
                     cur = (vk_stream_t)g->stream;
                     break;
                 case VK_OP_SIDE_END:
                     if (o.i0 < 0 || o.i0 >= N_SIDE_EVENTS) return vk::set_error("vk_run_ops: side event %d out of range", o.i0);
-                    e = hipEventRecord(g->done[o.i0], g->stream);
+                    if (rode_here != g->done[o.i0]) e = hipEventRecord(g->done[o.i0], g->stream);
                     g->recorded[o.i0] = true;
                     cur = s;
                     break;
@@ -102,7 +105,19 @@
             continue;
         }
         if (o.kind == VK_OP_GENERIC && o.a && ((const vk_generic_args*)o.a)->fn == VK_FN_GATE && cur == s) continue;
+        hipEvent_t armed = nullptr;
+        if (g_side_enabled && i + 1 < n) {
+            const vk_op& nx = ops[i + 1];
+            const bool fork = nx.kind == VK_OP_SIDE_BEGIN && nx.i0 != 1 && cur == s;
+            const bool done = nx.kind == VK_OP_SIDE_END && cur != s && nx.i0 >= 0 && nx.i0 < N_SIDE_EVENTS;
+            if (fork || done) {
+                if (!g && !(g = side_for(s))) return -1;
+                armed = fork ? g->fork : g->done[nx.i0];
+                vk::arm_launch_event(armed);
+            }
+        }
         int rc = run_one(o, i, cur);
+        if (armed && vk::take_launch_event() == nullptr) rode = armed;
         if (rc != 0) return rc;
     }
     if (cur != s) return vk::set_error("vk_run_ops: op list ends inside a side-stream block");
diff --git a/volta_amd/csrc/fp8.hip b/volta_amd/csrc/fp8.hip
--- a/volta_amd/csrc/fp8.hip
+++ b/volta_amd/csrc/fp8.hip
@@ -171,7 +171,7 @@
     case E: {                                                                                             \
         auto k = gemm_fp8_kernel<E, WM, WN, TM>;                                                          \
         static const hipError_t attr = hipFuncSetAttribute((const void*)k, hipFuncAttributeMaxDynamicSharedMemorySize, LDS); (void)attr; \
-        hipLaunchKernelGGL(k, dim3(total), dim3(64 * WM * WN), LDS, s, g);                                \
+        VK_LAUNCH(k, dim3(total), dim3(64 * WM * WN), LDS, s, g);                                        \
         break;                                                                                            \
     }
     switch (epi) {
@@ -234,8 +234,8 @@
     if (K <= 0 || K > 4096 || (K & 7) || (ld & 7) || (ldq & 7)) return set_error("vk_quant_rows_fp8: K=%d (multiple of 8, <= 4096), ld / ldq multiples of 8", K);
     if (((uintptr_t)src & 15) || ((uintptr_t)dst & 7)) return set_error("vk_quant_rows_fp8: alignment");
     hipStream_t s = (hipStream_t)stream;
-    if (src_is_f32) hipLaunchKernelGGL(quant_rows_fp8_kernel<float>, dim3((M + 3) / 4), dim3(256), 0, s, (const float*)src, ld, (uint8_t*)dst, ldq, scale, M, K, dyn);
-    else hipLaunchKernelGGL(quant_rows_fp8_kernel<uint16_t>, dim3((M + 3) / 4), dim3(256), 0, s, (const uint16_t*)src, ld, (uint8_t*)dst, ldq, scale, M, K, dyn);
+    if (src_is_f32) VK_LAUNCH(quant_rows_fp8_kernel<float>, dim3((M + 3) / 4), dim3(256), 0, s, (const float*)src, ld, (uint8_t*)dst, ldq, scale, M, K, dyn);
+    else VK_LAUNCH(quant_rows_fp8_kernel<uint16_t>, dim3((M + 3) / 4), dim3(256), 0, s, (const uint16_t*)src, ld, (uint8_t*)dst, ldq, scale, M, K, dyn);
     return check_launch("vk_quant_rows_fp8");
 }
 
@@ -244,6 +244,6 @@
     if ((n & 7) || ((uintptr_t)src & 15) || ((uintptr_t)dst & 7)) return set_error("vk_cast_bf16_fp8: n %% 8 == 0 and aligned buffers required");
     int64_t blocks = (n / 8 + 255) / 256;
     if (blocks > 8192) blocks = 8192;
-    hipLaunchKernelGGL(cast_bf16_fp8_kernel, dim3((unsigned)blocks), dim3(256), 0, (hipStream_t)stream, (const uint16_t*)src, (uint8_t*)dst, (size_t)n, mul);
+    VK_LAUNCH(cast_bf16_fp8_kernel, dim3((unsigned)blocks), dim3(256), 0, (hipStream_t)stream, (const uint16_t*)src, (uint8_t*)dst, (size_t)n, mul);
     return check_launch("vk_cast_bf16_fp8");
 }
diff --git a/volta_amd/csrc/gemm.hip b/volta_amd/csrc/gemm.hip
--- a/volta_amd/csrc/gemm.hip
+++ b/volta_amd/csrc/gemm.hip
@@ -177,7 +177,7 @@
     case E: {                                                                                             \
         auto k = gemm_kernel<AT, BT, E, WM, WN, REGSTAGE, TM>;                                                \
         static const hipError_t attr = hipFuncSetAttribute((const void*)k, hipFuncAttributeMaxDynamicSharedMemorySize, LDS); (void)attr;  \
-        hipLaunchKernelGGL(k, dim3(total), dim3(G::THREADS), LDS, s, g);                                  \
+        VK_LAUNCH(k, dim3(total), dim3(G::THREADS), LDS, s, g);                                          \
         break;                                                                                            \
     }
     switch (epi) {
diff --git a/volta_amd/csrc/gemm256.hip b/volta_amd/csrc/gemm256.hip
--- a/volta_amd/csrc/gemm256.hip
+++ b/volta_amd/csrc/gemm256.hip
@@ -528,13 +528,13 @@
             if (persistent) {                                                                             \
                 auto kp = gemm256p_kernel<AT, BT, E, KSPLIT>;                                             \
                 static const hipError_t attr_p = hipFuncSetAttribute((const void*)kp, hipFuncAttributeMaxDynamicSharedMemorySize, LDS); (void)attr_p; \
-                hipExtLaunchKernelGGL(kp, dim3(persistent_grid(total)), dim3(512), LDS, s, nullptr, nullptr, flags, g, total, g_stamps); \
+                hipExtLaunchKernelGGL(kp, dim3(persistent_grid(total)), dim3(512), LDS, s, nullptr, vk::take_launch_event(), flags, g, total, g_stamps); \
                 break;                                                                                    \
             }                                                                                             \
         }                                                                                                 \
         auto k = VK_KERNEL_OF(E);                                                                         \
         static const hipError_t attr = hipFuncSetAttribute((const void*)k, hipFuncAttributeMaxDynamicSharedMemorySize, LDS); (void)attr;  \
-        hipExtLaunchKernelGGL(k, dim3(total), dim3(512), LDS, s, nullptr, nullptr, flags, g);             \
+        hipExtLaunchKernelGGL(k, dim3(total), dim3(512), LDS, s, nullptr, vk::take_launch_event(), flags, g); \
         break;                                                                                            \
     }
     switch (epi) {
@@ -553,7 +553,7 @@
     if (layout == ((BT_) ? VK_NN : VK_NT) && epi_p == (P_) && epi_c == (C_)) {                                        \
         auto k = gemm256c_kernel<BT_, P_, C_>;                                                                        \
         static const hipError_t attr = hipFuncSetAttribute((const void*)k, hipFuncAttributeMaxDynamicSharedMemorySize, LDS); (void)attr; \
-        hipLaunchKernelGGL(k, dim3(ncu), dim3(512), LDS, s, g, nprod, ncons, g_stamps);                               \
+        VK_LAUNCH(k, dim3(ncu), dim3(512), LDS, s, g, nprod, ncons, g_stamps);                                       \
         return check_launch("vk_gemm_chain");                                                                         \
     }
     VK_CHAIN_CASE(false, VK_EPI_GELU, VK_EPI_BF16)
diff --git a/volta_amd/csrc/gemm4w.hip b/volta_amd/csrc/gemm4w.hip
--- a/volta_amd/csrc/gemm4w.hip
+++ b/volta_amd/csrc/gemm4w.hip
@@ -158,7 +158,7 @@
     case E: {                                                                                             \
         auto k = gemm4w_kernel<AT, BT, E, TI, RING>;                                                      \
         static const hipError_t attr = hipFuncSetAttribute((const void*)k, hipFuncAttributeMaxDynamicSharedMemorySize, LDS); (void)attr; \
-        hipLaunchKernelGGL(k, dim3(total), dim3(256), LDS, s, g);                                         \
+        VK_LAUNCH(k, dim3(total), dim3(256), LDS, s, g);                                                 \
         break;                                                                                            \
     }
     switch (epi) {
diff --git a/volta_amd/csrc/heads.hip b/volta_amd/csrc/heads.hip
--- a/volta_amd/csrc/heads.hip
+++ b/volta_amd/csrc/heads.hip
@@ -216,58 +216,58 @@
 extern "C" int vk_select_rows(const int64_t* labels, int N, int mode, int inner, int outer, int off, int32_t* rows, int32_t* pos,
                               int32_t* count, vk_stream_t s) {
     if (N < 0 || inner <= 0) return set_error("vk_select_rows: bad arguments");
-    hipLaunchKernelGGL(select_rows_kernel, dim3(1), dim3(1024), 0, (hipStream_t)s, labels, N, mode, inner, outer, off, rows, pos, count);
+    VK_LAUNCH(select_rows_kernel, dim3(1), dim3(1024), 0, (hipStream_t)s, labels, N, mode, inner, outer, off, rows, pos, count);
     return check_launch("vk_select_rows");
 }
 extern "C" int vk_gather_rows(const void* src, const int32_t* rows, const int32_t* count, void* dst, int H, int max_rows, vk_stream_t s) {
     if (H % 8) return set_error("vk_gather_rows: H %% 8 != 0");
     if (max_rows <= 0) return 0;
-    hipLaunchKernelGGL(gather_rows_kernel, dim3((max_rows + 3) / 4), dim3(256), 0, (hipStream_t)s, (const uint16_t*)src, rows, count, (uint16_t*)dst, H, max_rows);
+    VK_LAUNCH(gather_rows_kernel, dim3((max_rows + 3) / 4), dim3(256), 0, (hipStream_t)s, (const uint16_t*)src, rows, count, (uint16_t*)dst, H, max_rows);
     return check_launch("vk_gather_rows");
 }
 extern "C" int vk_scatter_rows_add(const void* src, const int32_t* rows, const int32_t* count, void* dst, int H, int max_rows, vk_stream_t s) {
     if (H % 4) return set_error("vk_scatter_rows_add: H %% 4 != 0");
     if (max_rows <= 0) return 0;
-    hipLaunchKernelGGL(scatter_rows_add_kernel, dim3((max_rows + 3) / 4), dim3(256), 0, (hipStream_t)s, (const uint16_t*)src, rows, count, (uint16_t*)dst, H, max_rows);
+    VK_LAUNCH(scatter_rows_add_kernel, dim3((max_rows + 3) / 4), dim3(256), 0, (hipStream_t)s, (const uint16_t*)src, rows, count, (uint16_t*)dst, H, max_rows);
     return check_launch("vk_scatter_rows_add");
 }
 extern "C" int vk_xent_fwd(const vk_xent_args* a, vk_stream_t s) {
     if (a->max_rows <= 0) return 0;
-    hipLaunchKernelGGL(xent_fwd_kernel, dim3(a->max_rows), dim3(256), 0, (hipStream_t)s, *a);
+    VK_LAUNCH(xent_fwd_kernel, dim3(a->max_rows), dim3(256), 0, (hipStream_t)s, *a);
     return check_launch("vk_xent_fwd");
 }
 extern "C" int vk_xent_bwd(const vk_xent_args* a, void* dlogits, int ldd, const float* gscale, vk_stream_t s) {
     if (a->max_rows <= 0) return 0;
     if (ldd < a->V) return set_error("vk_xent_bwd: ldd < V");
-    hipLaunchKernelGGL(xent_bwd_kernel, dim3(a->max_rows), dim3(256), 0, (hipStream_t)s, *a, (uint16_t*)dlogits, ldd, gscale);
+    VK_LAUNCH(xent_bwd_kernel, dim3(a->max_rows), dim3(256), 0, (hipStream_t)s, *a, (uint16_t*)dlogits, ldd, gscale);
     return check_launch("vk_xent_bwd");
 }
 extern "C" int vk_kl_fwd(const vk_kl_args* a, vk_stream_t s) {
     if (a->max_rows <= 0) return 0;
-    hipLaunchKernelGGL(kl_fwd_kernel, dim3(a->max_rows), dim3(256), 0, (hipStream_t)s, *a);
+    VK_LAUNCH(kl_fwd_kernel, dim3(a->max_rows), dim3(256), 0, (hipStream_t)s, *a);
     return check_launch("vk_kl_fwd");
 }
 extern "C" int vk_kl_bwd(const vk_kl_args* a, void* dlogits, int ldd, const float* gscale, vk_stream_t s) {
     if (a->max_rows <= 0) return 0;
     if (ldd < a->V) return set_error("vk_kl_bwd: ldd < V");
-    hipLaunchKernelGGL(kl_bwd_kernel, dim3(a->max_rows), dim3(256), 0, (hipStream_t)s, *a, (uint16_t*)dlogits, ldd, gscale);
+    VK_LAUNCH(kl_bwd_kernel, dim3(a->max_rows), dim3(256), 0, (hipStream_t)s, *a, (uint16_t*)dlogits, ldd, gscale);
     return check_launch("vk_kl_bwd");
 }
 extern "C" int vk_loss_finalize(const float* sums, const int32_t* n_t, const int32_t* n_v, int B, float kl_weight, float* losses, vk_stream_t s) {
-    hipLaunchKernelGGL(loss_finalize_kernel, dim3(1), dim3(64), 0, (hipStream_t)s, sums, n_t, n_v, B, kl_weight, losses);
+    VK_LAUNCH(loss_finalize_kernel, dim3(1), dim3(64), 0, (hipStream_t)s, sums, n_t, n_v, B, kl_weight, losses);
     return check_launch("vk_loss_finalize");
 }
 extern "C" int vk_pool_mul_fwd(const void* pt, const void* pv, void* out, int B, int P, vk_dropout drop, vk_stream_t s) {
-    hipLaunchKernelGGL(pool_mul_fwd_kernel, dim3((B * P + 255) / 256), dim3(256), 0, (hipStream_t)s, (const uint16_t*)pt, (const uint16_t*)pv, (uint16_t*)out, B, P, drop);
+    VK_LAUNCH(pool_mul_fwd_kernel, dim3((B * P + 255) / 256), dim3(256), 0, (hipStream_t)s, (const uint16_t*)pt, (const uint16_t*)pv, (uint16_t*)out, B, P, drop);
     return check_launch("vk_pool_mul_fwd");
 }
 extern "C" int vk_pool_mul_bwd(const void* dp, int ldp, const void* pt, const void* pv, void* dyt, void* dyv, int B, int P, vk_dropout drop, vk_stream_t s) {
-    hipLaunchKernelGGL(pool_mul_bwd_kernel, dim3((B * P + 255) / 256), dim3(256), 0, (hipStream_t)s, (const uint16_t*)dp, ldp, (const uint16_t*)pt,
-                       (const uint16_t*)pv, (uint16_t*)dyt, (uint16_t*)dyv, B, P, drop);
+    VK_LAUNCH(pool_mul_bwd_kernel, dim3((B * P + 255) / 256), dim3(256), 0, (hipStream_t)s, (const uint16_t*)dp, ldp, (const uint16_t*)pt,
+              (const uint16_t*)pv, (uint16_t*)dyt, (uint16_t*)dyv, B, P, drop);
     return check_launch("vk_pool_mul_bwd");
 }
 extern "C" int vk_mask_prep(const int64_t* mask, float* out, int n, vk_stream_t s) {
     if (n <= 0) return 0;
-    hipLaunchKernelGGL(mask_prep_kernel, dim3((n + 255) / 256), dim3(256), 0, (hipStream_t)s, mask, out, n);
+    VK_LAUNCH(mask_prep_kernel, dim3((n + 255) / 256), dim3(256), 0, (hipStream_t)s, mask, out, n);
     return check_launch("vk_mask_prep");
 }
diff --git a/volta_amd/csrc/layernorm.hip b/volta_amd/csrc/layernorm.hip
--- a/volta_amd/csrc/layernorm.hip
+++ b/volta_amd/csrc/layernorm.hip
@@ -346,11 +346,11 @@
     jp.nb0 = nb0;
     jp.stagger = jp.stagger_mod = 0;
     switch (nch) {
-        case 1: hipLaunchKernelGGL(ln_fwd_kernel<1>, grid, block, 0, s, jp); break;
-        case 2: hipLaunchKernelGGL(ln_fwd_kernel<2>, grid, block, 0, s, jp); break;
-        case 3: hipLaunchKernelGGL(ln_fwd_kernel<3>, grid, block, 0, s, jp); break;
-        case 4: hipLaunchKernelGGL(ln_fwd_kernel<4>, grid, block, 0, s, jp); break;
-        default: hipLaunchKernelGGL(ln_fwd_kernel<8>, grid, block, 0, s, jp); break;
+        case 1: VK_LAUNCH(ln_fwd_kernel<1>, grid, block, 0, s, jp); break;
+        case 2: VK_LAUNCH(ln_fwd_kernel<2>, grid, block, 0, s, jp); break;
+        case 3: VK_LAUNCH(ln_fwd_kernel<3>, grid, block, 0, s, jp); break;
+        case 4: VK_LAUNCH(ln_fwd_kernel<4>, grid, block, 0, s, jp); break;
+        default: VK_LAUNCH(ln_fwd_kernel<8>, grid, block, 0, s, jp); break;
     }
     return check_launch("vk_ln_fwd");
 }
@@ -370,8 +370,8 @@
 #endif
 
 static void ln_finalize_launch(const vk_ln_bwd_args* a, hipStream_t s) {
-    hipLaunchKernelGGL(vk::ln_bwd_finalize_kernel, dim3((2 * a->H + 63) / 64), dim3(1024), 0, s, a->partial, vk_ln_bwd_partial_rows(a->M), a->H,
-                       a->dgamma, a->dbeta, a->accumulate & 1);
+    VK_LAUNCH(vk::ln_bwd_finalize_kernel, dim3((2 * a->H + 63) / 64), dim3(1024), 0, s, a->partial, vk_ln_bwd_partial_rows(a->M), a->H,
+              a->dgamma, a->dbeta, a->accumulate & 1);
 }
 
 extern "C" int vk_ln_bwd_pair(const vk_ln_bwd_args* a, const vk_ln_bwd_args* b, vk_stream_t stream) {
@@ -379,7 +379,9 @@
     if (ln_check(a->H, 2048, "vk_ln_bwd")) return -1;
     if (b && (b->H != a->H || a->dyn || b->dyn)) return set_error("vk_ln_bwd_pair: both jobs need the same H and static row counts");
     if (b && !a->partial != !b->partial) {
+        const hipEvent_t ev = take_launch_event();
         if (vk_ln_bwd_pair(a, nullptr, stream)) return -1;
+        arm_launch_event(ev);
         return vk_ln_bwd_pair(b, nullptr, stream);
     }
     const bool params = a->partial != nullptr;
@@ -393,25 +395,34 @@
     jp.job[1] = b ? *b : *a;
     jp.nb0 = nb0;
     jp.stagger = g_ln_stagger; jp.stagger_mod = g_ln_stagger_mod;
+    const bool fin_a = params && (nb0 || !(a->accumulate & 1)) && !(a->accumulate & 2);
+    const bool fin_b = params && b && (nb1 || !(b->accumulate & 1)) && !(b->accumulate & 2);
+    const hipEvent_t ev = (fin_a || fin_b) ? take_launch_event() : nullptr;
     if (nb0 + nb1 && params) switch (nch) {
-        case 1: hipLaunchKernelGGL(ln_bwd_kernel<1>, grid, block, 0, s, jp, g_ln_stamps); break;
-        case 2: hipLaunchKernelGGL(ln_bwd_kernel<2>, grid, block, 0, s, jp, g_ln_stamps); break;
-        case 3: hipLaunchKernelGGL(ln_bwd_kernel<3>, grid, block, 0, s, jp, g_ln_stamps); break;
-        case 4: hipLaunchKernelGGL(ln_bwd_kernel<4>, grid, block, 0, s, jp, g_ln_stamps); break;
-        case 5: case 6: hipLaunchKernelGGL(ln_bwd_kernel<6>, grid, block, 0, s, jp, g_ln_stamps); break;
-        default: hipLaunchKernelGGL(ln_bwd_kernel<8>, grid, block, 0, s, jp, g_ln_stamps); break;
+        case 1: VK_LAUNCH(ln_bwd_kernel<1>, grid, block, 0, s, jp, g_ln_stamps); break;
+        case 2: VK_LAUNCH(ln_bwd_kernel<2>, grid, block, 0, s, jp, g_ln_stamps); break;
+        case 3: VK_LAUNCH(ln_bwd_kernel<3>, grid, block, 0, s, jp, g_ln_stamps); break;
+        case 4: VK_LAUNCH(ln_bwd_kernel<4>, grid, block, 0, s, jp, g_ln_stamps); break;
+        case 5: case 6: VK_LAUNCH(ln_bwd_kernel<6>, grid, block, 0, s, jp, g_ln_stamps); break;
+        default: VK_LAUNCH(ln_bwd_kernel<8>, grid, block, 0, s, jp, g_ln_stamps); break;
     }
     if (nb0 + nb1 && !params) switch (nch) {
-        case 1: hipLaunchKernelGGL(ln_bwd_dx_kernel<1>, grid, block, 0, s, jp, g_ln_stamps); break;
-        case 2: hipLaunchKernelGGL(ln_bwd_dx_kernel<2>, grid, block, 0, s, jp, g_ln_stamps); break;
-        case 3: hipLaunchKernelGGL(ln_bwd_dx_kernel<3>, grid, block, 0, s, jp, g_ln_stamps); break;
-        case 4: hipLaunchKernelGGL(ln_bwd_dx_kernel<4>, grid, block, 0, s, jp, g_ln_stamps); break;
-        case 5: case 6: hipLaunchKernelGGL(ln_bwd_dx_kernel<6>, grid, block, 0, s, jp, g_ln_stamps); break;
-        default: hipLaunchKernelGGL(ln_bwd_dx_kernel<8>, grid, block, 0, s, jp, g_ln_stamps); break;
+        case 1: VK_LAUNCH(ln_bwd_dx_kernel<1>, grid, block, 0, s, jp, g_ln_stamps); break;
+        case 2: VK_LAUNCH(ln_bwd_dx_kernel<2>, grid, block, 0, s, jp, g_ln_stamps); break;
+        case 3: VK_LAUNCH(ln_bwd_dx_kernel<3>, grid, block, 0, s, jp, g_ln_stamps); break;
+        case 4: VK_LAUNCH(ln_bwd_dx_kernel<4>, grid, block, 0, s, jp, g_ln_stamps); break;
+        case 5: case 6: VK_LAUNCH(ln_bwd_dx_kernel<6>, grid, block, 0, s, jp, g_ln_stamps); break;
+        default: VK_LAUNCH(ln_bwd_dx_kernel<8>, grid, block, 0, s, jp, g_ln_stamps); break;
     }
     if (!params) return check_launch("vk_ln_bwd");
-    if ((nb0 || !(a->accumulate & 1)) && !(a->accumulate & 2)) ln_finalize_launch(a, s);
-    if (b && (nb1 || !(b->accumulate & 1)) && !(b->accumulate & 2)) ln_finalize_launch(b, s);
+    if (fin_a) {
+        if (!fin_b) arm_launch_event(ev);
+        ln_finalize_launch(a, s);
+    }
+    if (fin_b) {
+        arm_launch_event(ev);
+        ln_finalize_launch(b, s);
+    }
     return check_launch("vk_ln_bwd");
 }
 
diff --git a/volta_amd/csrc/misc.hip b/volta_amd/csrc/misc.hip
--- a/volta_amd/csrc/misc.hip
+++ b/volta_amd/csrc/misc.hip
@@ -35,13 +35,13 @@
     if (((uintptr_t)a & 15) || ((uintptr_t)b & 15) || ((uintptr_t)out & 15)) return vk::set_error("vk_mul_bf16: 16-byte alignment required");
     int64_t blocks = (n / 8 + 255) / 256;
     if (blocks > 4096) blocks = 4096;
-    hipLaunchKernelGGL(vk::mul_bf16_kernel, dim3((unsigned)blocks), dim3(256), 0, (hipStream_t)s, (const uint16_t*)a, (const uint16_t*)b,
-                       (uint16_t*)out, (size_t)n, dyn_rows, row_len);
+    VK_LAUNCH(vk::mul_bf16_kernel, dim3((unsigned)blocks), dim3(256), 0, (hipStream_t)s, (const uint16_t*)a, (const uint16_t*)b,
+              (uint16_t*)out, (size_t)n, dyn_rows, row_len);
     return vk::check_launch("vk_mul_bf16");
 }
 
 extern "C" int vk_set_seed(uint64_t* seed_dev, uint64_t seed, vk_stream_t s) {
-    hipLaunchKernelGGL(vk::set_seed_kernel, dim3(1), dim3(1), 0, (hipStream_t)s, seed_dev, seed);
+    VK_LAUNCH(vk::set_seed_kernel, dim3(1), dim3(1), 0, (hipStream_t)s, seed_dev, seed);
     return vk::check_launch("vk_set_seed");
 }
 
@@ -51,7 +51,7 @@
     int64_t blocks = (n / 8 + 255) / 256;
     if (blocks > 4096) blocks = 4096;
     if (blocks < 1) blocks = 1;
-    hipLaunchKernelGGL(vk::cast_f32_bf16_kernel, dim3((unsigned)blocks), dim3(256), 0, (hipStream_t)s, src, (uint16_t*)dst, (size_t)n);
+    VK_LAUNCH(vk::cast_f32_bf16_kernel, dim3((unsigned)blocks), dim3(256), 0, (hipStream_t)s, src, (uint16_t*)dst, (size_t)n);
     return vk::check_launch("vk_cast_f32_bf16");
 }
 
@@ -89,7 +89,7 @@
 }
 
 extern "C" int vk_mfma_peak(const uint32_t* seed64, float* out, int iters, int blocks, vk_stream_t stream) {
-    hipLaunchKernelGGL(vk::mfma_peak_kernel, dim3(blocks), dim3(512), 0, (hipStream_t)stream, seed64, out, iters);
+    VK_LAUNCH(vk::mfma_peak_kernel, dim3(blocks), dim3(512), 0, (hipStream_t)stream, seed64, out, iters);
     return vk::check_launch("vk_mfma_peak");
 }
 
@@ -109,7 +109,7 @@
     if (nwg > 256 || usec > 100000) return vk::set_error("vk_hold_cus: at most 256 workgroups for at most 0.1 s (got %d, %d us)", nwg, usec);
     constexpr int LDS = 160 * 1024;
     static const hipError_t attr = hipFuncSetAttribute((const void*)vk::hold_cus_kernel, hipFuncAttributeMaxDynamicSharedMemorySize, LDS); (void)attr;
-    hipLaunchKernelGGL(vk::hold_cus_kernel, dim3(nwg), dim3(64), whole_cu ? LDS : 64, (hipStream_t)stream, (unsigned)usec * 100u);
+    VK_LAUNCH(vk::hold_cus_kernel, dim3(nwg), dim3(64), whole_cu ? LDS : 64, (hipStream_t)stream, (unsigned)usec * 100u);
     return vk::check_launch("vk_hold_cus");
 }
 
@@ -132,8 +132,8 @@
     if (bytes <= 0 || nwg <= 0) return 0;
     if ((bytes & 15) || ((uintptr_t)src & 15) || ((uintptr_t)dst & 15)) return vk::set_error("vk_comm_standin: 16-byte granularity");
     if (nwg > 1024 || min_usec < 0 || min_usec > 100000) return vk::set_error("vk_comm_standin: at most 1024 workgroups, at most 0.1 s");
-    hipLaunchKernelGGL(vk::comm_standin_kernel, dim3(nwg), dim3(256), 0, (hipStream_t)stream, (const vk::u32x4*)src, (vk::u32x4*)dst, (size_t)(bytes / 16),
-                       (unsigned)min_usec * 100u, (unsigned long long*)stamps);
+    VK_LAUNCH(vk::comm_standin_kernel, dim3(nwg), dim3(256), 0, (hipStream_t)stream, (const vk::u32x4*)src, (vk::u32x4*)dst, (size_t)(bytes / 16),
+              (unsigned)min_usec * 100u, (unsigned long long*)stamps);
     return vk::check_launch("vk_comm_standin");
 }
 
@@ -167,26 +167,26 @@
 
 extern "C" int vk_store_u64(uint64_t* word, uint64_t value, vk_stream_t stream) {
     if (!word) return vk::set_error("vk_store_u64: NULL");
-    hipLaunchKernelGGL(vk::store_u64_kernel, dim3(1), dim3(1), 0, (hipStream_t)stream, (unsigned long long*)word, (unsigned long long)value);
+    VK_LAUNCH(vk::store_u64_kernel, dim3(1), dim3(1), 0, (hipStream_t)stream, (unsigned long long*)word, (unsigned long long)value);
     return vk::check_launch("vk_store_u64");
 }
 
 extern "C" int vk_gate_value(const uint64_t* flag, uint64_t want, int timeout_us, int32_t* err, vk_stream_t stream) {
     if (!flag || timeout_us <= 0 || timeout_us > 10000000) return vk::set_error("vk_gate_value: flag and 0 < timeout_us <= 10000000");
-    hipLaunchKernelGGL(vk::gate_value_kernel, dim3(1), dim3(64), 0, (hipStream_t)stream, (const unsigned long long*)flag, (unsigned long long)want,
-                       (unsigned)(timeout_us > 40000000 ? 4000000000u : (unsigned)timeout_us * 100u), err);
+    VK_LAUNCH(vk::gate_value_kernel, dim3(1), dim3(64), 0, (hipStream_t)stream, (const unsigned long long*)flag, (unsigned long long)want,
+              (unsigned)(timeout_us > 40000000 ? 4000000000u : (unsigned)timeout_us * 100u), err);
     return vk::check_launch("vk_gate_value");
 }
 
 extern "C" int vk_gate_wait(const uint64_t* flag, const uint64_t* stamp, int timeout_us, int32_t* err, vk_stream_t stream) {
     if (!flag || !stamp || timeout_us <= 0 || timeout_us > 1000000) return vk::set_error("vk_gate_wait: flag, stamp and 0 < timeout_us <= 1000000");
-    hipLaunchKernelGGL(vk::gate_wait_kernel, dim3(1), dim3(64), 0, (hipStream_t)stream, (const unsigned long long*)flag, (const unsigned long long*)stamp,
-                       (unsigned)timeout_us * 100u, err);
+    VK_LAUNCH(vk::gate_wait_kernel, dim3(1), dim3(64), 0, (hipStream_t)stream, (const unsigned long long*)flag, (const unsigned long long*)stamp,
+              (unsigned)timeout_us * 100u, err);
     return vk::check_launch("vk_gate_wait");
 }
 
 extern "C" int vk_bump_u64(uint64_t* word, vk_stream_t stream) {
     if (!word) return vk::set_error("vk_bump_u64: NULL");
-    hipLaunchKernelGGL(vk::bump_u64_kernel, dim3(1), dim3(1), 0, (hipStream_t)stream, (unsigned long long*)word);
+    VK_LAUNCH(vk::bump_u64_kernel, dim3(1), dim3(1), 0, (hipStream_t)stream, (unsigned long long*)word);
     return vk::check_launch("vk_bump_u64");
 }
diff --git a/volta_amd/csrc/optim.hip b/volta_amd/csrc/optim.hip
--- a/volta_amd/csrc/optim.hip
+++ b/volta_amd/csrc/optim.hip
@@ -319,7 +319,7 @@
         total += nb;
     }
     if (total == 0) return 0;
-    hipLaunchKernelGGL(side_tail_kernel, dim3((unsigned)total), dim3(256), 0, (hipStream_t)s, t);
+    VK_LAUNCH(side_tail_kernel, dim3((unsigned)total), dim3(256), 0, (hipStream_t)s, t);
     return check_launch("vk_side_tail");
 }
 
@@ -329,7 +329,7 @@
     if (((uintptr_t)src & 15) || ((uintptr_t)dst & 7)) return set_error("vk_sum_slabs_bf16: src needs 16-byte, dst 8-byte alignment");
     int64_t blocks = (n / 4 + 255) / 256;
     if (blocks > 2048) blocks = 2048;
-    hipLaunchKernelGGL(sum_slabs_bf16_kernel, dim3((unsigned)blocks), dim3(256), 0, (hipStream_t)s, (uint16_t*)dst, src, (size_t)slab_stride, nslabs, (size_t)n, dyn_rows, row_len);
+    VK_LAUNCH(sum_slabs_bf16_kernel, dim3((unsigned)blocks), dim3(256), 0, (hipStream_t)s, (uint16_t*)dst, src, (size_t)slab_stride, nslabs, (size_t)n, dyn_rows, row_len);
     return check_launch("vk_sum_slabs_bf16");
 }
 
@@ -339,7 +339,7 @@
     int64_t blocks = (n / 4 + 255) / 256;
     if (blocks > 2048) blocks = 2048;
     if (blocks < 1) blocks = 1;
-    hipLaunchKernelGGL(sum_slabs_kernel, dim3((unsigned)blocks), dim3(256), 0, (hipStream_t)s, dst, src, (size_t)slab_stride, nslabs, (size_t)n);
+    VK_LAUNCH(sum_slabs_kernel, dim3((unsigned)blocks), dim3(256), 0, (hipStream_t)s, dst, src, (size_t)slab_stride, nslabs, (size_t)n);
     return check_launch("vk_sum_slabs_f32");
 }
 
@@ -379,6 +379,46 @@
     if (a->n == 0) return 0;
     hipLaunchKernelGGL(adamw_kernel, dim3((unsigned)(a->n / 1024)), dim3(256), 0, (hipStream_t)s, *a);
     return check_launch("vk_adamw_step");
+}
+
+extern "C" void* vk_event_create(void) {
+    hipEvent_t e = nullptr;
+    if (hipEventCreateWithFlags(&e, hipEventDisableTiming) != hipSuccess) {
+        set_error("vk_event_create: hipEventCreate failed");
+        return nullptr;
+    }
+    return (void*)e;
+}
+
+extern "C" int vk_stream_wait_event(vk_stream_t s, void* event) {
+    if (!event) return set_error("vk_stream_wait_event: NULL event");
+    if (hipStreamWaitEvent((hipStream_t)s, (hipEvent_t)event, 0) != hipSuccess) return set_error("vk_stream_wait_event: hipStreamWaitEvent failed");
+    return 0;
+}
+
+extern "C" int vk_adamw_step_ranges(const vk_adamw_args* a, const int64_t* bounds, int n, void* const* events, vk_stream_t s) {
+    if (n < 0 || (n > 0 && (!bounds || !events))) return set_error("vk_adamw_step_ranges: %d ranges need bounds and events", n);
+    if (a->n % 1024) return set_error("vk_adamw_step_ranges: arena length must be a multiple of 1024 elements");
+    int64_t lo = 0;
+    for (int i = 0; i < n; ++i) {
+        const int64_t hi = bounds[i];
+        if (hi < lo || hi > a->n / 1024) return set_error("vk_adamw_step_ranges: bounds must ascend within the arena's %lld chunks (range %d ends at %lld)", (long long)(a->n / 1024), i, (long long)hi);
+        if (!events[i]) return set_error("vk_adamw_step_ranges: event %d is NULL", i);
+        if (hi > lo) {
+            vk_adamw_args r = *a;
+            const int64_t off = lo * 1024;
+            r.p += off; r.g += off; r.m += off; r.v += off;
+            if (r.shadow) r.shadow = (uint16_t*)r.shadow + off;
+            if (r.chunk_class) r.chunk_class += lo;
+            r.n = (hi - lo) * 1024;
+            hipExtLaunchKernelGGL(adamw_kernel, dim3((unsigned)(r.n / 1024)), dim3(256), 0, (hipStream_t)s, nullptr, (hipEvent_t)events[i], 0, r);
+            if (check_launch("vk_adamw_step_ranges")) return -1;
+        } else if (hipEventRecord((hipEvent_t)events[i], (hipStream_t)s) != hipSuccess) {
+            return set_error("vk_adamw_step_ranges: hipEventRecord failed");
+        }
+        lo = hi;
+    }
+    return 0;
 }
 
 extern "C" int vk_adamw_step_on(const vk_adamw_args* a, int ncus, vk_stream_t s) {
diff --git a/volta_amd/csrc/pairs.hip b/volta_amd/csrc/pairs.hip
--- a/volta_amd/csrc/pairs.hip
+++ b/volta_amd/csrc/pairs.hip
@@ -58,6 +58,6 @@
         if (a->n_items[a->side[k]] <= 0) return set_error("vk_pair_gather: segment %d reads side %d, which has no items", k, a->side[k]);
     }
     if (a->npairs == 0) return 0;
-    hipLaunchKernelGGL(pair_gather_kernel, dim3((unsigned)a->npairs, (unsigned)a->nseg), dim3(256), 0, (hipStream_t)s, *a);
+    VK_LAUNCH(pair_gather_kernel, dim3((unsigned)a->npairs, (unsigned)a->nseg), dim3(256), 0, (hipStream_t)s, *a);
     return check_launch("vk_pair_gather");
 }
diff --git a/volta_amd/csrc/util.h b/volta_amd/csrc/util.h
--- a/volta_amd/csrc/util.h
+++ b/volta_amd/csrc/util.h
@@ -1,5 +1,6 @@
 #pragma once
 #include <hip/hip_runtime.h>
+#include <hip/hip_ext.h>
 #include <cstdarg>
 #include <cstdio>
 
@@ -7,4 +8,21 @@
 char* error_buffer();
 int set_error(const char* fmt, ...);
 int check_launch(const char* what);
+
+hipEvent_t& launch_event_slot();
+inline void arm_launch_event(hipEvent_t e) { launch_event_slot() = e; }
+inline hipEvent_t take_launch_event() {
+    hipEvent_t& slot = launch_event_slot();
+    hipEvent_t e = slot;
+    slot = nullptr;
+    return e;
 }
+}
+
+#define VK_LAUNCH(kernel, grid, block, lds, stream, ...)                                                              \
+    do {                                                                                                              \
+        if (hipEvent_t vk_ev_ = vk::take_launch_event())                                                              \
+            hipExtLaunchKernelGGL(kernel, grid, block, lds, stream, nullptr, vk_ev_, 0, __VA_ARGS__);                 \
+        else                                                                                                          \
+            hipLaunchKernelGGL(kernel, grid, block, lds, stream, __VA_ARGS__);                                        \
+    } while (0)
diff --git a/volta_amd/csrc/vislosses.hip b/volta_amd/csrc/vislosses.hip
--- a/volta_amd/csrc/vislosses.hip
+++ b/volta_amd/csrc/vislosses.hip
@@ -257,10 +257,10 @@
     const dim3 grid(a->max_rows), block(256);
     hipStream_t st = (hipStream_t)s;
     switch (a->kind) {
-        case VK_VIS_MSE: hipLaunchKernelGGL(vis_reg_fwd_kernel<false>, grid, block, 0, st, *a); break;
-        case VK_VIS_HUBER: hipLaunchKernelGGL(vis_reg_fwd_kernel<true>, grid, block, 0, st, *a); break;
-        case VK_VIS_XENT: hipLaunchKernelGGL(vis_xent_fwd_kernel, grid, block, 0, st, *a); break;
-        default: hipLaunchKernelGGL(vis_nce_fwd_kernel, grid, block, 0, st, *a); break;
+        case VK_VIS_MSE: VK_LAUNCH(vis_reg_fwd_kernel<false>, grid, block, 0, st, *a); break;
+        case VK_VIS_HUBER: VK_LAUNCH(vis_reg_fwd_kernel<true>, grid, block, 0, st, *a); break;
+        case VK_VIS_XENT: VK_LAUNCH(vis_xent_fwd_kernel, grid, block, 0, st, *a); break;
+        default: VK_LAUNCH(vis_nce_fwd_kernel, grid, block, 0, st, *a); break;
     }
     return check_launch("vk_vis_loss_fwd");
 }
@@ -273,46 +273,46 @@
     hipStream_t st = (hipStream_t)s;
     uint16_t* d = (uint16_t*)dlogits;
     switch (a->kind) {
-        case VK_VIS_MSE: hipLaunchKernelGGL(vis_reg_bwd_kernel<false>, grid, block, 0, st, *a, d, ldd, gscale); break;
-        case VK_VIS_HUBER: hipLaunchKernelGGL(vis_reg_bwd_kernel<true>, grid, block, 0, st, *a, d, ldd, gscale); break;
-        case VK_VIS_XENT: hipLaunchKernelGGL(vis_xent_bwd_kernel, grid, block, 0, st, *a, d, ldd, gscale); break;
-        default: hipLaunchKernelGGL(vis_nce_bwd_kernel, grid, block, 0, st, *a, d, ldd, gscale); break;
+        case VK_VIS_MSE: VK_LAUNCH(vis_reg_bwd_kernel<false>, grid, block, 0, st, *a, d, ldd, gscale); break;
+        case VK_VIS_HUBER: VK_LAUNCH(vis_reg_bwd_kernel<true>, grid, block, 0, st, *a, d, ldd, gscale); break;
+        case VK_VIS_XENT: VK_LAUNCH(vis_xent_bwd_kernel, grid, block, 0, st, *a, d, ldd, gscale); break;
+        default: VK_LAUNCH(vis_nce_bwd_kernel, grid, block, 0, st, *a, d, ldd, gscale); break;
     }
     return check_launch("vk_vis_loss_bwd");
 }
 
 extern "C" int vk_nce_negatives(vk_dropout rng, int B, int R, int32_t* out, vk_stream_t s) {
     if (!rng.seed || B < 2 || R < 2) return set_error("vk_nce_negatives: needs a seed word, B >= 2 and R >= 2 (losses.py:50,59 draw from [0, B-1) and [0, R-1))");
-    hipLaunchKernelGGL(nce_negatives_kernel, dim3(B * R), dim3(128), 0, (hipStream_t)s, rng, B, R, out);
+    VK_LAUNCH(nce_negatives_kernel, dim3(B * R), dim3(128), 0, (hipStream_t)s, rng, B, R, out);
     return check_launch("vk_nce_negatives");
 }
 
 extern "C" int vk_pool_fuse_fwd(const void* pt, const void* pv, void* out, int B, int P, int mode, vk_dropout drop, vk_stream_t s) {
     if (mode < VK_FUSE_MUL || mode > VK_FUSE_TEXT || (mode != VK_FUSE_TEXT && !pv)) return set_error("vk_pool_fuse_fwd: mode %d (mul 0 | sum 1 | text 2; pv required unless text)", mode);
-    hipLaunchKernelGGL(pool_fuse_fwd_kernel, dim3((B * P + 255) / 256), dim3(256), 0, (hipStream_t)s, (const uint16_t*)pt, (const uint16_t*)pv, (uint16_t*)out, B, P, mode, drop);
+    VK_LAUNCH(pool_fuse_fwd_kernel, dim3((B * P + 255) / 256), dim3(256), 0, (hipStream_t)s, (const uint16_t*)pt, (const uint16_t*)pv, (uint16_t*)out, B, P, mode, drop);
     return check_launch("vk_pool_fuse_fwd");
 }
 extern "C" int vk_pool_fuse_bwd(const void* dp, int ldp, const void* pt, const void* pv, void* dyt, void* dyv, int B, int P, int mode, vk_dropout drop, vk_stream_t s) {
     if (mode < VK_FUSE_MUL || mode > VK_FUSE_TEXT || (mode != VK_FUSE_TEXT && (!pv || !dyv))) return set_error("vk_pool_fuse_bwd: mode %d (mul 0 | sum 1 | text 2; pv, dyv required unless text)", mode);
-    hipLaunchKernelGGL(pool_fuse_bwd_kernel, dim3((B * P + 255) / 256), dim3(256), 0, (hipStream_t)s, (const uint16_t*)dp, ldp, (const uint16_t*)pt,
-                       (const uint16_t*)pv, (uint16_t*)dyt, (uint16_t*)dyv, B, P, mode, drop);
+    VK_LAUNCH(pool_fuse_bwd_kernel, dim3((B * P + 255) / 256), dim3(256), 0, (hipStream_t)s, (const uint16_t*)dp, ldp, (const uint16_t*)pt,
+              (const uint16_t*)pv, (uint16_t*)dyt, (uint16_t*)dyv, B, P, mode, drop);
     return check_launch("vk_pool_fuse_bwd");
 }
 
 extern "C" int vk_text_end_rows(const int64_t* ids, int B, int T, int32_t* rows, int32_t* count, vk_stream_t s) {
     if (B <= 0 || T <= 0) return set_error("vk_text_end_rows: bad arguments");
-    hipLaunchKernelGGL(text_end_rows_kernel, dim3(B), dim3(64), 0, (hipStream_t)s, ids, B, T, rows, count);
+    VK_LAUNCH(text_end_rows_kernel, dim3(B), dim3(64), 0, (hipStream_t)s, ids, B, T, rows, count);
     return check_launch("vk_text_end_rows");
 }
 
 extern "C" int vk_vlbert_obj_ids(const int32_t* zero_flag, int64_t* ids, int M, int K, vk_stream_t s) {
     if (M <= 0 || K <= 0) return set_error("vk_vlbert_obj_ids: bad arguments");
-    hipLaunchKernelGGL(vlbert_obj_ids_kernel, dim3((M + 255) / 256), dim3(256), 0, (hipStream_t)s, zero_flag, ids, M, K);
+    VK_LAUNCH(vlbert_obj_ids_kernel, dim3((M + 255) / 256), dim3(256), 0, (hipStream_t)s, zero_flag, ids, M, K);
     return check_launch("vk_vlbert_obj_ids");
 }
 
 extern "C" int vk_vlbert_positions(const int64_t* ids, int B, int T, int K, int64_t* tpos, int64_t* opos, vk_stream_t s) {
     if (B <= 0 || T <= 0 || K <= 0 || !ids || !tpos || !opos) return set_error("vk_vlbert_positions: bad arguments");
-    hipLaunchKernelGGL(vlbert_positions_kernel, dim3(1), dim3(1024), 0, (hipStream_t)s, ids, B, T, K, tpos, opos);
+    VK_LAUNCH(vlbert_positions_kernel, dim3(1), dim3(1024), 0, (hipStream_t)s, ids, B, T, K, tpos, opos);
     return check_launch("vk_vlbert_positions");
 }
diff --git a/volta_amd/engine/arena.py b/volta_amd/engine/arena.py
--- a/volta_amd/engine/arena.py
+++ b/volta_amd/engine/arena.py
@@ -130,7 +130,6 @@
     def sync_optimizer(self):
         pend = self.opt_pending
         if pend:
-            cur = torch.cuda.current_stream()
             for ev in pend[1]:
-                cur.wait_event(ev)
+                check(L.lib.vk_stream_wait_event(L.stream_ptr(), ev))
             self.opt_pending = None
diff --git a/volta_amd/engine/builder.py b/volta_amd/engine/builder.py
--- a/volta_amd/engine/builder.py
+++ b/volta_amd/engine/builder.py
@@ -605,11 +605,10 @@
             self.fwd.run()
             return
         bounds, events = pend
-        cur = torch.cuda.current_stream()
         waited = 0
         for nd, start, end in self.fwd_segments(bounds):
             for i in range(waited, nd):
-                cur.wait_event(events[i])
+                check(L.lib.vk_stream_wait_event(L.stream_ptr(), events[i]))
             waited = max(waited, nd)
             self.fwd.run(start, end)
         self.arena.opt_pending = None
diff --git a/volta_amd/optimization.py b/volta_amd/optimization.py
--- a/volta_amd/optimization.py
+++ b/volta_amd/optimization.py
@@ -254,24 +254,15 @@
             with torch.cuda.device(arena.device):
                 f["stream"] = independent_stream(engine_streams(), device=arena.device, soft_avoid=[comm] if comm is not None else [])
             f["bounds"] = [nchunks * (i + 1) // n for i in range(n)]
-            f["events"] = [torch.cuda.Event() for _ in range(n)]
+            f["events"] = [L.lib.vk_event_create() for _ in range(n)]
+            if not all(f["events"]):
+                raise L.VoltaHipError(L.lib.vk_last_error().decode())
+            f["bounds_c"], f["events_c"] = (C.c_int64 * n)(*f["bounds"]), (C.c_void_p * n)(*f["events"])
         side, bounds, events = f["stream"], f["bounds"], f["events"]
         side.wait_stream(torch.cuda.current_stream())
         if clip is not None:
             clip.record_stream(side)
-        base = (a.p, a.g, a.m, a.v, a.shadow, a.chunk_class)
-        with torch.cuda.stream(side):
-            sp = C.c_void_p(side.cuda_stream)
-            lo = 0
-            for hi, ev in zip(bounds, events):
-                if hi > lo:
-                    off = lo * 1024
-                    a.p, a.g, a.m, a.v = base[0] + 4 * off, base[1] + 4 * off, base[2] + 4 * off, base[3] + 4 * off
-                    a.shadow, a.chunk_class = base[4] + 2 * off, base[5] + lo
-                    a.n = (hi - lo) * 1024
-                    L.check(L.lib.vk_adamw_step(C.byref(a), sp))
-                ev.record(side)
-                lo = hi
+        L.check(L.lib.vk_adamw_step_ranges(C.byref(a), f["bounds_c"], len(bounds), f["events_c"], C.c_void_p(side.cuda_stream)))
         arena.opt_pending = (bounds, events)
 
     def synchronize(self):
```

New measurement: 15680 (median of 2 runs). Within noise of the previous version (+0.0%).
